# FHE-ACCELE/Homulator

Measured on AMD Instinct MI355X. Metric: hmult+key-switch ops/sec, higher is better.
Workload: dtype u64

## Files before the change

### homulator_amd/csrc/hm_backend.hip

```cpp
#include <hip/hip_runtime.h>
#include <dlfcn.h>
#include <rccl/rccl.h>
#include <algorithm>
#include <cstdarg>
#include <cstdio>
#include <cstring>
#include <map>
#include <tuple>
#include <type_traits>
#include <memory>
#include <stdexcept>
#include <string>
#include <vector>

#include "../../include/homulator_hip.h"
#include "hm_elem_core.h"
#include "hm_modarith.h"
#include "hm_ntt_core.h"
#include "hm_params.h"
#include "hm_caps.h"


__device__ __forceinline__ bool hm_block_map(uint32_t tiles_per_limb, uint32_t n_entries, uint32_t logG, uint32_t &entry, uint32_t &tile) {
  const uint32_t b = blockIdx.x, xcd = b & 7u, slot = b >> 3;
// ... 264 lines not shown
#define HM_NIP_MAX_TERMS 4
static_assert(HM_GENERIC || HM_NIP_MAX_TERMS <= 5, "mont32 lazy key products: five terms of less than 1.5q + 2^28 stay below 8q (hm_mac_add)");
#define HM_NIP_MAX_OUT 2
#define HM_NIP_MAX_LIMBS 4096
struct HmNipLimb {
  uint16_t x[HM_NIP_MAX_TERMS];
  uint16_t y[HM_NIP_MAX_OUT][HM_NIP_MAX_TERMS];
  uint16_t out[HM_NIP_MAX_OUT];
  uint16_t mod;
  uint16_t coeff_mask;
};
#define HM_NIP_INV_OUT 0x8000u
struct HmNipArgs {
  const uint64_t *hand;
  const uint64_t *x;
  const uint64_t *y;
  uint64_t *out;
  const HmW *tw, *twist;
  const HmW *tw_inv, *twist_inv;
  const HmMod *mods;
  uint32_t logN, n_limbs, logG, n_terms;
  const HmNipLimb *limb;
  uint32_t x_galois;
};
typedef const HmNipLimb __attribute__((address_space(4))) *HmConstNipLimb;
#ifndef HM_NIP_WAVES
#define HM_NIP_WAVES 3
#endif
#ifndef HM_NIP_WIDE
#define HM_NIP_WIDE 0
#endif
#ifndef HM_NIP_PREFETCH
#define HM_NIP_PREFETCH 0
#endif
#ifndef HM_NIP_MAC_CH
#define HM_NIP_MAC_CH 2
#endif
#ifndef HM_NIP_LD_AUX
#define HM_NIP_LD_AUX 0
#endif
#ifndef HM_NIP_ST_AUX
#define HM_NIP_ST_AUX 0
#endif
template <int K> struct HmNipKey { static constexpr int value = K; };
namespace hm16 {
#include "hm_nip_body.inl"
}
#undef HM_EPT
#define HM_EPT 8
namespace hm8 {
#include "hm_nip_body.inl"
}
#undef HM_EPT
#define HM_EPT 16
template <int OUTS, int INVOUT, bool XG = false>
__global__ void __launch_bounds__((1 << HM_TL_ROW) / HM_EPT) __attribute__((amdgpu_waves_per_eu(HM_NIP_WAVES))) k_ntt_row_ip(HmNipArgs a) {
  hm16::hm_nip_body<OUTS, INVOUT, HM_TL_ROW, XG>(a);
}
template <int OUTS, int INVOUT, bool XG = false>
__global__ void __launch_bounds__((1 << HM_TL_ROW) / 8) k_ntt_row_ip8(HmNipArgs a) {
  hm8::hm_nip_body<OUTS, INVOUT, HM_TL_ROW, XG>(a);
}

#include "hm_bcol.h"
__global__ void __launch_bounds__(256) k_tensor(HmTensorArgs a) {
  const uint32_t N = 1u << a.logN;
  const uint32_t per_limb = N / 512;
  const uint32_t entry = blockIdx.x / per_limb, chunk = blockIdx.x % per_limb;
  if (entry >= a.n_limbs) return;
  const HmTensorLimb lb = a.limb[entry];
  const HmMod m = a.mods[lb.mod];
  const size_t x = (size_t)chunk * 512 + 2 * threadIdx.x;
  const ulonglong2 va = *reinterpret_cast<const ulonglong2 *>(a.a + (size_t)lb.a * N + x);
  const ulonglong2 vb = *reinterpret_cast<const ulonglong2 *>(a.b + (size_t)lb.b * N + x);
  const ulonglong2 vc = *reinterpret_cast<const ulonglong2 *>(a.c + (size_t)lb.c * N + x);
  const ulonglong2 vd = *reinterpret_cast<const ulonglong2 *>(a.d + (size_t)lb.d * N + x);
  uint64_t x0, x1, x2, y0, y1, y2;
  hm_tensor_one(va.x, vb.x, vc.x, vd.x, m, x0, x1, x2);
  hm_tensor_one(va.y, vb.y, vc.y, vd.y, m, y0, y1, y2);
  const ulonglong2 r0 = {x0, y0}, r1 = {x1, y1}, r2 = {x2, y2};
  *reinterpret_cast<ulonglong2 *>(a.o0 + (size_t)lb.o0 * N + x) = r0;
  *reinterpret_cast<ulonglong2 *>(a.o1 + (size_t)lb.o1 * N + x) = r1;
  *reinterpret_cast<ulonglong2 *>(a.o2 + (size_t)lb.o2 * N + x) = r2;
}

#ifndef HM_EWE_UNITS
#define HM_EWE_UNITS 1
#endif
template <int OP>
__global__ void __launch_bounds__(256) k_ewe(HmEweArgs a) {
  const uint32_t N = 1u << a.logN;
  const uint32_t per_limb = N / (512 * HM_EWE_UNITS);
  uint32_t entry = blockIdx.x / per_limb, chunk = blockIdx.x % per_limb;
  if (entry >= a.n_limbs) return;
  const HmEweLimb lb = a.limb[entry];
  const HmMod m = a.mods[lb.mod];
  const HmTw k = a.k[entry];
  const size_t x0 = (size_t)chunk * (512 * HM_EWE_UNITS) + 2 * threadIdx.x;
  constexpr int uses = hm_ewe_uses(OP);
  ulonglong2 va[HM_EWE_UNITS], vb[HM_EWE_UNITS], vc[HM_EWE_UNITS], vd[HM_EWE_UNITS];
#pragma unroll
  for (int u = 0; u < HM_EWE_UNITS; ++u) {
    const size_t x = x0 + 512 * u;
    va[u] = vb[u] = vc[u] = vd[u] = ulonglong2{0, 0};
    if (uses & 1) va[u] = *reinterpret_cast<const ulonglong2 *>(a.a + (size_t)lb.a * N + x);
    if (uses & 2) vb[u] = *reinterpret_cast<const ulonglong2 *>(a.b + (size_t)lb.b * N + x);
    if (uses & 4) vc[u] = *reinterpret_cast<const ulonglong2 *>(a.c + (size_t)lb.c * N + x);
    if (uses & 8) vd[u] = *reinterpret_cast<const ulonglong2 *>(a.d + (size_t)lb.d * N + x);
  }
#pragma unroll
  for (int u = 0; u < HM_EWE_UNITS; ++u) {
    ulonglong2 r;
    r.x = hm_ewe_one<OP>(va[u].x, vb[u].x, vc[u].x, vd[u].x, k, m);
    r.y = hm_ewe_one<OP>(va[u].y, vb[u].y, vc[u].y, vd[u].y, k, m);
    *reinterpret_cast<ulonglong2 *>(a.out + (size_t)lb.out * N + x0 + 512 * u) = r;
  }
}

template <int TERMS, int OUTS>
__global__ void __launch_bounds__(256) k_inner_product(HmIpArgs a) {
  const uint32_t N = 1u << a.logN;
  const uint32_t per_limb = N / 512;
  const uint32_t entry = blockIdx.x / per_limb, chunk = blockIdx.x % per_limb;
  if (entry >= a.n_limbs) return;
  const HmIpLimb &lb = a.limb[entry];
  const HmMod m = a.mods[lb.mod];
  const size_t off = (size_t)chunk * 512 + 2 * threadIdx.x;
  ulonglong2 vx[TERMS], vy[OUTS][TERMS];
  size_t offx = off;
  bool swap = false;
  if (a.x_galois > 1) {
    const uint32_t s = hm_auto_src((uint32_t)off, a.x_galois, a.logN);
    offx = s & ~1u; swap = s & 1u;
  }
#pragma unroll
  for (int j = 0; j < TERMS; ++j) {
    vx[j] = *reinterpret_cast<const ulonglong2 *>(a.x + (size_t)lb.x[j] * N + offx);
    if (swap) { const unsigned long long t = vx[j].x; vx[j].x = vx[j].y; vx[j].y = t; }
#pragma unroll
    for (int k = 0; k < OUTS; ++k) vy[k][j] = *reinterpret_cast<const ulonglong2 *>(a.y + (size_t)lb.y[k][j] * N + off);
  }
#pragma unroll
  for (int k = 0; k < OUTS; ++k) {
    hm_u128 s0 = 0, s1 = 0;
#pragma unroll
    for (int j = 0; j < TERMS; ++j) {
      s0 += (hm_u128)vx[j].x * vy[k][j].x;
      s1 += (hm_u128)vx[j].y * vy[k][j].y;
    }
    const ulonglong2 r = {hm_barrett(s0, m), hm_barrett(s1, m)};
    *reinterpret_cast<ulonglong2 *>(a.out + (size_t)lb.out[k] * N + off) = r;
  }
}

template <int N_IN>
__global__ void __launch_bounds__(HM_BCONV_THREADS) k_bconv(HmBconvArgs a) {
  const auto &p = HM_CONST_PROB(a.prob)[blockIdx.z];
  const uint32_t t0 = blockIdx.y * a.chunk;
  if (t0 >= p.n_out) return;
  const uint32_t t1 = min(t0 + a.chunk, p.n_out);
  const uint32_t x = (blockIdx.x * HM_BCONV_THREADS + threadIdx.x) * HM_BCONV_CPT;
  if (x >= (1u << a.logN)) return;
  if (p.in_packed) hm_bconv_thread<N_IN, HM_BCONV_CPT, true>(p, a.logN, x, t0, t1);
  else hm_bconv_thread<N_IN, HM_BCONV_CPT, false>(p, a.logN, x, t0, t1);
}
typedef void (*hm_bconv_kernel)(HmBconvArgs);
// ... 873 lines not shown
  f.addGalois = d->addend_galois;
  if (d->addend_galois && (d->n_conv || d->mix || !d->addend)) return fail(c, HM_ERR_UNSUPPORTED,
      "hm_ntt_mix_sub_scale: addend_galois needs an addend and combines with neither the mix prologue nor conversions inside the transform");
  if (!d->n_conv) return ntt_common(c, "hm_ntt_mix_sub_scale", d->in, d->in_limbs, d->out, d->out_limbs, d->mod_ids, d->n, 0, d->k, f);
  if (!d->conv) return fail(c, HM_ERR_ARG, "hm_ntt_mix_sub_scale: n_conv without descriptors");
  const uint32_t n = d->n;
  std::map<uint32_t, uint32_t> byOut;
  for (uint32_t i = 0; i < n; ++i)
    if (!byOut.emplace(limb_at(d->out_limbs, i), i).second) return fail(c, HM_ERR_ARG, "hm_ntt_mix_sub_scale: output limb %u appears twice",
        limb_at(d->out_limbs, i));
  std::vector<char> covered(n, 0);
  std::vector<std::vector<uint32_t>> mixLimbs(d->n_conv);
  std::vector<std::vector<uint64_t>> mixK(d->n_conv);
  std::vector<const uint32_t *> mlp(d->n_conv);
  std::vector<const uint64_t *> mkp(d->n_conv);
  for (uint32_t j = 0; j < d->n_conv; ++j) {
    const hm_bconv_desc &cv = d->conv[j];
    if (cv.out != d->out) return fail(c, HM_ERR_ARG, "hm_ntt_mix_sub_scale: conv[%u].out must be the output buffer", j);
    if (!cv.out_ids || cv.n_out == 0 || cv.n_out > HM_BCONV_MAX_OUT) return fail(c, HM_ERR_ARG, "hm_ntt_mix_sub_scale: conv[%u]: bad output basis", j);
    for (uint32_t t = 0; t < cv.n_out; ++t) {
      auto it = byOut.find(limb_at(cv.out_limbs, t));
      if (it == byOut.end()) return fail(c, HM_ERR_ARG, "hm_ntt_mix_sub_scale: conv[%u] output %u feeds no limb-poly of the call", j, t);
      const uint32_t i = it->second;
      if (covered[i]) return fail(c, HM_ERR_ARG, "hm_ntt_mix_sub_scale: limb-poly %u is fed by two conversions", i);
      if (cv.out_ids[t] != d->mod_ids[i]) return fail(c, HM_ERR_ARG,
          "hm_ntt_mix_sub_scale: conv[%u] output %u has another modulus than the limb-poly it feeds", j, t);
      covered[i] = 1;
      mixLimbs[j].push_back(d->mix ? limb_at(d->mix_limbs, i) : 0);
      mixK[j].push_back(d->mix ? d->mix_k[i] : 0);
    }
    mlp[j] = mixLimbs[j].data(); mkp[j] = mixK[j].data();
  }
  const BcolMix bm = {d->mix, mlp.data(), mkp.data()};
  hm_status st;
  if ((st = bconv_col_launch(c, d->conv, d->n_conv, d->mix ? &bm : nullptr))) return st;
  auto sub = [&](char want, bool second) -> hm_status {
    std::vector<uint32_t> il, ml, mnl, al, ol, mods;
    std::vector<uint64_t> mk, ak, kk;
    for (uint32_t i = 0; i < n; ++i) {
      if (covered[i] != want) continue;
      il.push_back(limb_at(d->in_limbs, i)); ol.push_back(limb_at(d->out_limbs, i)); mnl.push_back(limb_at(d->minuend_limbs, i));
      mods.push_back(d->mod_ids[i]); kk.push_back(d->k[i]);
      if (d->mix) { ml.push_back(limb_at(d->mix_limbs, i)); mk.push_back(d->mix_k[i]); }
      if (d->addend) al.push_back(limb_at(d->addend_limbs, i));
      if (d->addend_k) ak.push_back(d->addend_k[i]);
    }
    if (mods.empty()) return HM_OK;
    if (!second && !d->in) return fail(c, HM_ERR_ARG, "hm_ntt_mix_sub_scale: `in` is null but not every limb-poly is fed by a conversion");
    NttFused g = f;
    g.minuend_limbs = mnl.data(); g.addend_limbs = d->addend ? al.data() : nullptr; g.addend_k = d->addend_k ? ak.data() : nullptr;
    g.mix_limbs = d->mix ? ml.data() : nullptr; g.mix_k = d->mix ? mk.data() : nullptr;
    g.secondPassOnly = second;
    if (second) { g.mix = nullptr; g.mix_limbs = nullptr; g.mix_k = nullptr; }
    return ntt_common(c, "hm_ntt_mix_sub_scale", second ? d->out : d->in, second ? ol.data() : il.data(), d->out, ol.data(), mods.data(),
        (uint32_t)mods.size(), 0, kk.data(), g);
  };
  if ((st = sub(1, true))) return st;
  return sub(0, false);
}

extern "C" hm_status hm_tensor(hm_ctx *c, const uint64_t *pa, const uint32_t *la, const uint64_t *pb, const uint32_t *lb,
                               const uint64_t *pc, const uint32_t *lc, const uint64_t *pd, const uint32_t *ld, uint64_t *o0,
                               const uint32_t *l0, uint64_t *o1, const uint32_t *l1, uint64_t *o2, const uint32_t *l2,
                               const uint32_t *mod_ids, uint32_t n) {
  if (!c) return HM_ERR_ARG;
  if (!pa || !pb || !pc || !pd || !o0 || !o1 || !o2) return fail(c, HM_ERR_ARG, "hm_tensor: null buffer");
  hm_status st;
  const uint32_t *lists[7] = {la, lb, lc, ld, l0, l1, l2};
  for (auto l : lists)
    if ((st = check_limbs(c, "hm_tensor", l, n))) return st;
  if ((st = check_mods(c, "hm_tensor", mod_ids, n))) return st;
  HM_HIP(c, hipSetDevice(c->device));
  for (uint32_t base = 0; base < n; base += HM_MAX_LIMBS) {
    const uint32_t cnt = std::min<uint32_t>(HM_MAX_LIMBS, n - base);
    HmTensorArgs a;
    a.a = pa; a.b = pb; a.c = pc; a.d = pd; a.o0 = o0; a.o1 = o1; a.o2 = o2;
    a.mods = c->d_mods; a.logN = c->P.logN; a.n_limbs = cnt;
    for (uint32_t i = 0; i < cnt; ++i) {
      const uint32_t g = base + i;
      a.limb[i] = HmTensorLimb{(uint16_t)limb_at(la, g), (uint16_t)limb_at(lb, g), (uint16_t)limb_at(lc, g), (uint16_t)limb_at(ld, g),
                               (uint16_t)limb_at(l0, g), (uint16_t)limb_at(l1, g), (uint16_t)limb_at(l2, g), (uint16_t)mod_ids[g]};
    }
    hipLaunchKernelGGL(k_tensor, dim3(cnt * (c->P.N / 512)), dim3(256), 0, c->stream, a);
    HM_HIP(c, hipGetLastError());
  }
  return HM_OK;
}

extern "C" hm_status hm_automorph(hm_ctx *c, const uint64_t *in, const uint32_t *in_limbs, uint64_t *out,
                                  const uint32_t *out_limbs, uint32_t n, uint32_t galois) {
  if (!c) return HM_ERR_ARG;
  if (!in || !out) return fail(c, HM_ERR_ARG, "hm_automorph: null buffer");
  if (!(galois & 1) || galois >= 2 * c->P.N) return fail(c, HM_ERR_ARG, "hm_automorph: galois element must be odd and < 2N");
  hm_status st;
  if ((st = check_limbs(c, "hm_automorph", in_limbs, n)) || (st = check_limbs(c, "hm_automorph", out_limbs, n))) return st;
  HM_HIP(c, hipSetDevice(c->device));
  for (uint32_t base = 0; base < n; base += HM_MAX_LIMBS) {
    const uint32_t cnt = std::min<uint32_t>(HM_MAX_LIMBS, n - base);
    HmAutoArgs a;
    a.in = in; a.out = out; a.logN = c->P.logN; a.n_limbs = cnt; a.g = galois;
    for (uint32_t i = 0; i < cnt; ++i)
      a.limb[i] = HmLimb{(uint16_t)limb_at(in_limbs, base + i), (uint16_t)limb_at(out_limbs, base + i), 0, 0};
    hipLaunchKernelGGL(k_automorph, dim3(cnt * (c->P.N / 1024)), dim3(256), 0, c->stream, a);
    HM_HIP(c, hipGetLastError());
  }
  return HM_OK;
}

template <int OP>
static void launch_ewe(hm_ctx *c, const HmEweArgs &a) {
  hipLaunchKernelGGL((k_ewe<OP>), dim3(a.n_limbs * (c->P.N / (512 * HM_EWE_UNITS))), dim3(256), 0, c->stream, a);
}

extern "C" hm_status hm_ewe(hm_ctx *c, int op, const uint64_t *pa, const uint32_t *la, const uint64_t *pb,
                            const uint32_t *lb, const uint64_t *pc, const uint32_t *lc, const uint64_t *pd,
                            const uint32_t *ld, uint64_t *out, const uint32_t *lo, const uint32_t *mod_ids,
                            uint32_t n, const uint64_t *k) {
  if (!c) return HM_ERR_ARG;
  if (op < 0 || op >= HM_EWE_NOPS) return fail(c, HM_ERR_ARG, "hm_ewe: bad opcode %d", op);
  const int uses = hm_ewe_uses(op);
  if (((uses & 1) && !pa) || ((uses & 2) && !pb) || ((uses & 4) && !pc) || ((uses & 8) && !pd) || !out)
    return fail(c, HM_ERR_ARG, "hm_ewe: opcode %d is missing an operand", op);
  const bool needs_k = op == HM_EWE_MUL_CONST || op == HM_EWE_SUB_SCALE || op == HM_EWE_SUB_SCALE_ADD;
  if (needs_k && !k) return fail(c, HM_ERR_ARG, "hm_ewe: opcode %d needs constants", op);
  hm_status st;
  if ((st = check_limbs(c, "hm_ewe", la, n)) || (st = check_limbs(c, "hm_ewe", lb, n)) ||
      (st = check_limbs(c, "hm_ewe", lc, n)) || (st = check_limbs(c, "hm_ewe", ld, n)) ||
      (st = check_limbs(c, "hm_ewe", lo, n)) || (st = check_mods(c, "hm_ewe", mod_ids, n)))
    return st;
  HM_HIP(c, hipSetDevice(c->device));
  for (uint32_t base = 0; base < n; base += HM_MAX_LIMBS) {
    const uint32_t cnt = std::min<uint32_t>(HM_MAX_LIMBS, n - base);
    HmEweArgs a;
    a.a = pa; a.b = pb; a.c = pc; a.d = pd; a.out = out;
    a.mods = c->d_mods; a.logN = c->P.logN; a.n_limbs = cnt; a.op = (uint32_t)op;
    for (uint32_t i = 0; i < cnt; ++i) {
      const uint32_t g = base + i, m = mod_ids[g];
      a.limb[i] = HmEweLimb{(uint16_t)limb_at(la, g), (uint16_t)limb_at(lb, g), (uint16_t)limb_at(lc, g),
                            (uint16_t)limb_at(ld, g), (uint16_t)limb_at(lo, g), (uint16_t)m};
      a.k[i] = HmTw{0, 0};
      if (needs_k) {
        if (k[g] >= c->P.mod[m]) return fail(c, HM_ERR_ARG, "hm_ewe: k[%u] is not reduced", g);
        a.k[i] = HmTw{k[g], hm::shoup(k[g], c->P.mod[m])};
      }
    }
    switch (op) {
    case HM_EWE_MUL: launch_ewe<HM_EWE_MUL>(c, a); break;
    case HM_EWE_MAC2: launch_ewe<HM_EWE_MAC2>(c, a); break;
    case HM_EWE_MAC_ADD: launch_ewe<HM_EWE_MAC_ADD>(c, a); break;
    case HM_EWE_ADD: launch_ewe<HM_EWE_ADD>(c, a); break;
    case HM_EWE_SUB: launch_ewe<HM_EWE_SUB>(c, a); break;
    case HM_EWE_MUL_CONST: launch_ewe<HM_EWE_MUL_CONST>(c, a); break;
    case HM_EWE_SUB_SCALE: launch_ewe<HM_EWE_SUB_SCALE>(c, a); break;
    case HM_EWE_COPY: launch_ewe<HM_EWE_COPY>(c, a); break;
    case HM_EWE_SUB_SCALE_ADD: launch_ewe<HM_EWE_SUB_SCALE_ADD>(c, a); break;
    }
    HM_HIP(c, hipGetLastError());
  }
  return HM_OK;
}

template <int T, int O>
static void launch_ip(hm_ctx *c, const HmIpArgs &a) {
  hipLaunchKernelGGL((k_inner_product<T, O>), dim3(a.n_limbs * (c->P.N / 512)), dim3(256), 0, c->stream, a);
}
extern "C" hm_status hm_inner_product(hm_ctx *c, const uint64_t *x, const uint32_t *x_limbs, const uint64_t *y,
// ... 639 lines not shown
```

### homulator_amd/csrc/hm_caps.h

```cpp
#pragma once
#include <stdint.h>
#include <string.h>

#define HM_BCOL_MAX_IN 32
#define HM_BCOL_MAX_IN_MIX 15

struct HmCaps {
  uint32_t small_geometry;
  uint32_t bcol_max_in;
  uint32_t bcol_pref_in;
  uint32_t bcol_max_in_mix;
  uint32_t ip_inverse_out;
  uint32_t col_slices;
};
static inline HmCaps hm_caps(uint32_t logN) {
  switch (logN) {
  case 16: return HmCaps{1, HM_BCOL_MAX_IN, 15, HM_BCOL_MAX_IN_MIX, 1, 16};
  case 15: return HmCaps{1, HM_BCOL_MAX_IN, HM_BCOL_MAX_IN, HM_BCOL_MAX_IN_MIX, 1, 8};
  default: return HmCaps{0, 0, 0, 0, 0, 0};
  }
}
static inline int hm_cap_by_name(uint32_t logN, const char *name, uint64_t *value) {
  const HmCaps c = hm_caps(logN);
  if (!strcmp(name, "cap_small_geometry")) { *value = c.small_geometry; return 0; }
  if (!strcmp(name, "cap_bconv_col_max_in")) { *value = c.bcol_max_in; return 0; }
  if (!strcmp(name, "cap_bconv_col_max_in_mix")) { *value = c.bcol_max_in_mix; return 0; }
  if (!strcmp(name, "cap_bconv_col_pref_in")) { *value = c.bcol_pref_in; return 0; }
  if (!strcmp(name, "cap_ip_inverse_out")) { *value = c.ip_inverse_out; return 0; }
  if (!strcmp(name, "cap_col_slices")) { *value = c.col_slices; return 0; }
  return 1;
}
```

### homulator_amd/csrc/hm_dispatch_gen.inc

```

struct HmApi {
  hm_status (*create)(hm_ctx **ctx, const hm_params *params);
  void (*destroy)(hm_ctx *ctx);
  const char * (*last_error)(const hm_ctx *ctx);
  const char * (*version)(void);
  hm_status (*get_modulus)(const hm_ctx *ctx, uint32_t mod_id, uint64_t *q);
  hm_status (*get_psi)(const hm_ctx *ctx, uint32_t mod_id, uint64_t *psi);
  hm_status (*malloc)(hm_ctx *ctx, size_t bytes, void **dptr);
  hm_status (*free)(hm_ctx *ctx, void *dptr);
  hm_status (*memcpy_h2d)(hm_ctx *ctx, void *dst, const void *src, size_t bytes);
  hm_status (*memcpy_d2h)(hm_ctx *ctx, void *dst, const void *src, size_t bytes);
  hm_status (*memcpy_d2d)(hm_ctx *ctx, void *dst, const void *src, size_t bytes);
  hm_status (*sync)(hm_ctx *ctx);
  void * (*stream)(hm_ctx *ctx);
  hm_status (*wait_for)(hm_ctx *ctx, hm_ctx *producer);
  hm_status (*ntt)(hm_ctx *ctx, const uint64_t *in, const uint32_t *in_limbs, uint64_t *out, const uint32_t *out_limbs, const uint32_t *mod_ids, uint32_t n, int inverse, const uint64_t *scale);
  hm_status (*ntt_sub_scale)(hm_ctx *ctx, const uint64_t *in, const uint32_t *in_limbs, const uint64_t *minuend, const uint32_t *minuend_limbs, const uint64_t *addend, const uint32_t *addend_limbs, uint64_t *out, const uint32_t *out_limbs, const uint32_t *mod_ids, uint32_t n, const uint64_t *k);
  hm_status (*ntt_mix_sub_scale)(hm_ctx *ctx, const hm_ntt_fused_desc *desc);
  hm_status (*automorph)(hm_ctx *ctx, const uint64_t *in, const uint32_t *in_limbs, uint64_t *out, const uint32_t *out_limbs, uint32_t n, uint32_t galois);
  hm_status (*ewe)(hm_ctx *ctx, int op, const uint64_t *a, const uint32_t *a_limbs, const uint64_t *b, const uint32_t *b_limbs, const uint64_t *c, const uint32_t *c_limbs, const uint64_t *d, const uint32_t *d_limbs, uint64_t *out, const uint32_t *out_limbs, const uint32_t *mod_ids, uint32_t n, const uint64_t *k);
  hm_status (*tensor)(hm_ctx *ctx, const uint64_t *a, const uint32_t *a_limbs, const uint64_t *b, const uint32_t *b_limbs, const uint64_t *c, const uint32_t *c_limbs, const uint64_t *d, const uint32_t *d_limbs, uint64_t *o0, const uint32_t *o0_limbs, uint64_t *o1, const uint32_t *o1_limbs, uint64_t *o2, const uint32_t *o2_limbs, const uint32_t *mod_ids, uint32_t n);
  hm_status (*inner_product)(hm_ctx *ctx, const uint64_t *x, const uint32_t *x_limbs, const uint64_t *y, const uint32_t *y_limbs, uint64_t *out, const uint32_t *out_limbs, const uint32_t *mod_ids, uint32_t n, uint32_t n_terms, uint32_t n_out);
  hm_status (*inner_product_ex)(hm_ctx *ctx, const hm_ip_desc *desc);
  hm_status (*inner_product_hoisted)(hm_ctx *ctx, const hm_ip_hoisted_desc *desc);
  hm_status (*ntt_inner_product)(hm_ctx *ctx, const hm_ntt_ip_desc *desc);
  hm_status (*ntt_second_pass)(hm_ctx *ctx, uint64_t *buf, const uint32_t *limbs, const uint32_t *mod_ids, uint32_t n, int inverse, const uint64_t *scale);
  hm_status (*ntt_ex)(hm_ctx *ctx, const hm_ntt_desc *desc);
  hm_status (*bconv)(hm_ctx *ctx, const uint64_t *in, const uint32_t *in_limbs, const uint32_t *in_ids, uint32_t n_in, uint64_t *out, const uint32_t *out_limbs, const uint32_t *out_ids, uint32_t n_out);
  hm_status (*bconv_batch)(hm_ctx *ctx, const hm_bconv_desc *descs, uint32_t n_desc);
  hm_status (*bconv_col)(hm_ctx *ctx, const hm_bconv_desc *descs, uint32_t n_desc, uint32_t tile0, uint32_t n_tiles);
  hm_status (*bconv_consts)(hm_ctx *ctx, const uint32_t *in_ids, uint32_t n_in, const uint32_t *out_ids, uint32_t n_out, uint64_t *qhat_inv, uint64_t *table);
  hm_status (*comm_unique_id)(void *out128);
  hm_status (*comm_init_rccl)(hm_ctx *ctx, int rank, int world, const void *unique_id128);
  hm_status (*comm_init_external)(hm_ctx *ctx, int rank, int world, hm_exchange_fn fn, void *user);
  hm_status (*comm_info)(const hm_ctx *ctx, int *rank, int *world);
  hm_status (*slice_rows)(const uint32_t *owners, uint32_t n, uint32_t world, uint32_t *rows);
  hm_status (*limbs_to_slices)(hm_ctx *ctx, const uint64_t *buf, const uint32_t *limbs, const uint32_t *owners, uint32_t n, uint64_t *slices);
  hm_status (*slices_to_limbs)(hm_ctx *ctx, const uint64_t *slices, uint64_t *buf, const uint32_t *limbs, const uint32_t *owners, uint32_t n);
  hm_status (*limbs_to_colslices)(hm_ctx *ctx, const uint64_t *buf, const uint32_t *limbs, const uint32_t *owners, uint32_t n, uint64_t *slices);
  hm_status (*colslices_to_limbs)(hm_ctx *ctx, const uint64_t *slices, uint64_t *buf, const uint32_t *limbs, const uint32_t *owners, uint32_t n);
  hm_status (*exchange_stream)(hm_ctx *ctx, int enable);
  hm_status (*exchange_mark)(hm_ctx *ctx, uint32_t slot);
  hm_status (*exchange_wait)(hm_ctx *ctx, uint32_t slot);
  hm_status (*replicate_limbs)(hm_ctx *ctx, uint64_t *buf, const uint32_t *limbs, const uint32_t *owners, uint32_t n);
  hm_status (*fill_uniform)(hm_ctx *ctx, uint64_t *out, const uint32_t *out_limbs, const uint32_t *mod_ids, uint32_t n, uint64_t seed);
  hm_status (*capture_begin)(hm_ctx *ctx);
  hm_status (*capture_end)(hm_ctx *ctx, hm_graph **graph);
  hm_status (*graph_launch)(hm_ctx *ctx, hm_graph *graph);
  void (*graph_destroy)(hm_graph *graph);
  hm_status (*set_option)(hm_ctx *ctx, const char *name, uint64_t value);
  hm_status (*capability)(uint32_t logN, const char *name, uint64_t *value);
  hm_status (*get_counter)(hm_ctx *ctx, const char *name, uint64_t *value);
  hm_status (*timer_start)(hm_ctx *ctx);
  hm_status (*timer_stop)(hm_ctx *ctx, uint64_t *elapsed_ns);
};
static HmApi g_api[2];
static const char *hm_api_load(void *h, HmApi &a) {
  a.create = reinterpret_cast<decltype(a.create)>(dlsym(h, "hm_create")); if (!a.create) return "hm_create";
  a.destroy = reinterpret_cast<decltype(a.destroy)>(dlsym(h, "hm_destroy")); if (!a.destroy) return "hm_destroy";
  a.last_error = reinterpret_cast<decltype(a.last_error)>(dlsym(h, "hm_last_error")); if (!a.last_error) return "hm_last_error";
  a.version = reinterpret_cast<decltype(a.version)>(dlsym(h, "hm_version")); if (!a.version) return "hm_version";
  a.get_modulus = reinterpret_cast<decltype(a.get_modulus)>(dlsym(h, "hm_get_modulus")); if (!a.get_modulus) return "hm_get_modulus";
  a.get_psi = reinterpret_cast<decltype(a.get_psi)>(dlsym(h, "hm_get_psi")); if (!a.get_psi) return "hm_get_psi";
  a.malloc = reinterpret_cast<decltype(a.malloc)>(dlsym(h, "hm_malloc")); if (!a.malloc) return "hm_malloc";
  a.free = reinterpret_cast<decltype(a.free)>(dlsym(h, "hm_free")); if (!a.free) return "hm_free";
  a.memcpy_h2d = reinterpret_cast<decltype(a.memcpy_h2d)>(dlsym(h, "hm_memcpy_h2d")); if (!a.memcpy_h2d) return "hm_memcpy_h2d";
  a.memcpy_d2h = reinterpret_cast<decltype(a.memcpy_d2h)>(dlsym(h, "hm_memcpy_d2h")); if (!a.memcpy_d2h) return "hm_memcpy_d2h";
  a.memcpy_d2d = reinterpret_cast<decltype(a.memcpy_d2d)>(dlsym(h, "hm_memcpy_d2d")); if (!a.memcpy_d2d) return "hm_memcpy_d2d";
  a.sync = reinterpret_cast<decltype(a.sync)>(dlsym(h, "hm_sync")); if (!a.sync) return "hm_sync";
  a.stream = reinterpret_cast<decltype(a.stream)>(dlsym(h, "hm_stream")); if (!a.stream) return "hm_stream";
  a.wait_for = reinterpret_cast<decltype(a.wait_for)>(dlsym(h, "hm_wait_for")); if (!a.wait_for) return "hm_wait_for";
  a.ntt = reinterpret_cast<decltype(a.ntt)>(dlsym(h, "hm_ntt")); if (!a.ntt) return "hm_ntt";
  a.ntt_sub_scale = reinterpret_cast<decltype(a.ntt_sub_scale)>(dlsym(h, "hm_ntt_sub_scale")); if (!a.ntt_sub_scale) return "hm_ntt_sub_scale";
  a.ntt_mix_sub_scale = reinterpret_cast<decltype(a.ntt_mix_sub_scale)>(dlsym(h, "hm_ntt_mix_sub_scale")); if (!a.ntt_mix_sub_scale) return "hm_ntt_mix_sub_scale";
  a.automorph = reinterpret_cast<decltype(a.automorph)>(dlsym(h, "hm_automorph")); if (!a.automorph) return "hm_automorph";
  a.ewe = reinterpret_cast<decltype(a.ewe)>(dlsym(h, "hm_ewe")); if (!a.ewe) return "hm_ewe";
  a.tensor = reinterpret_cast<decltype(a.tensor)>(dlsym(h, "hm_tensor")); if (!a.tensor) return "hm_tensor";
  a.inner_product = reinterpret_cast<decltype(a.inner_product)>(dlsym(h, "hm_inner_product")); if (!a.inner_product) return "hm_inner_product";
  a.inner_product_ex = reinterpret_cast<decltype(a.inner_product_ex)>(dlsym(h, "hm_inner_product_ex")); if (!a.inner_product_ex) return "hm_inner_product_ex";
  a.inner_product_hoisted = reinterpret_cast<decltype(a.inner_product_hoisted)>(dlsym(h, "hm_inner_product_hoisted")); if (!a.inner_product_hoisted) return "hm_inner_product_hoisted";
  a.ntt_inner_product = reinterpret_cast<decltype(a.ntt_inner_product)>(dlsym(h, "hm_ntt_inner_product")); if (!a.ntt_inner_product) return "hm_ntt_inner_product";
  a.ntt_second_pass = reinterpret_cast<decltype(a.ntt_second_pass)>(dlsym(h, "hm_ntt_second_pass")); if (!a.ntt_second_pass) return "hm_ntt_second_pass";
  a.ntt_ex = reinterpret_cast<decltype(a.ntt_ex)>(dlsym(h, "hm_ntt_ex")); if (!a.ntt_ex) return "hm_ntt_ex";
  a.bconv = reinterpret_cast<decltype(a.bconv)>(dlsym(h, "hm_bconv")); if (!a.bconv) return "hm_bconv";
  a.bconv_batch = reinterpret_cast<decltype(a.bconv_batch)>(dlsym(h, "hm_bconv_batch")); if (!a.bconv_batch) return "hm_bconv_batch";
  a.bconv_col = reinterpret_cast<decltype(a.bconv_col)>(dlsym(h, "hm_bconv_col")); if (!a.bconv_col) return "hm_bconv_col";
  a.bconv_consts = reinterpret_cast<decltype(a.bconv_consts)>(dlsym(h, "hm_bconv_consts")); if (!a.bconv_consts) return "hm_bconv_consts";
  a.comm_unique_id = reinterpret_cast<decltype(a.comm_unique_id)>(dlsym(h, "hm_comm_unique_id")); if (!a.comm_unique_id) return "hm_comm_unique_id";
  a.comm_init_rccl = reinterpret_cast<decltype(a.comm_init_rccl)>(dlsym(h, "hm_comm_init_rccl")); if (!a.comm_init_rccl) return "hm_comm_init_rccl";
  a.comm_init_external = reinterpret_cast<decltype(a.comm_init_external)>(dlsym(h, "hm_comm_init_external")); if (!a.comm_init_external) return "hm_comm_init_external";
  a.comm_info = reinterpret_cast<decltype(a.comm_info)>(dlsym(h, "hm_comm_info")); if (!a.comm_info) return "hm_comm_info";
  a.slice_rows = reinterpret_cast<decltype(a.slice_rows)>(dlsym(h, "hm_slice_rows")); if (!a.slice_rows) return "hm_slice_rows";
  a.limbs_to_slices = reinterpret_cast<decltype(a.limbs_to_slices)>(dlsym(h, "hm_limbs_to_slices")); if (!a.limbs_to_slices) return "hm_limbs_to_slices";
  a.slices_to_limbs = reinterpret_cast<decltype(a.slices_to_limbs)>(dlsym(h, "hm_slices_to_limbs")); if (!a.slices_to_limbs) return "hm_slices_to_limbs";
  a.limbs_to_colslices = reinterpret_cast<decltype(a.limbs_to_colslices)>(dlsym(h, "hm_limbs_to_colslices")); if (!a.limbs_to_colslices) return "hm_limbs_to_colslices";
  a.colslices_to_limbs = reinterpret_cast<decltype(a.colslices_to_limbs)>(dlsym(h, "hm_colslices_to_limbs")); if (!a.colslices_to_limbs) return "hm_colslices_to_limbs";
  a.exchange_stream = reinterpret_cast<decltype(a.exchange_stream)>(dlsym(h, "hm_exchange_stream")); if (!a.exchange_stream) return "hm_exchange_stream";
  a.exchange_mark = reinterpret_cast<decltype(a.exchange_mark)>(dlsym(h, "hm_exchange_mark")); if (!a.exchange_mark) return "hm_exchange_mark";
  a.exchange_wait = reinterpret_cast<decltype(a.exchange_wait)>(dlsym(h, "hm_exchange_wait")); if (!a.exchange_wait) return "hm_exchange_wait";
  a.replicate_limbs = reinterpret_cast<decltype(a.replicate_limbs)>(dlsym(h, "hm_replicate_limbs")); if (!a.replicate_limbs) return "hm_replicate_limbs";
  a.fill_uniform = reinterpret_cast<decltype(a.fill_uniform)>(dlsym(h, "hm_fill_uniform")); if (!a.fill_uniform) return "hm_fill_uniform";
  a.capture_begin = reinterpret_cast<decltype(a.capture_begin)>(dlsym(h, "hm_capture_begin")); if (!a.capture_begin) return "hm_capture_begin";
  a.capture_end = reinterpret_cast<decltype(a.capture_end)>(dlsym(h, "hm_capture_end")); if (!a.capture_end) return "hm_capture_end";
  a.graph_launch = reinterpret_cast<decltype(a.graph_launch)>(dlsym(h, "hm_graph_launch")); if (!a.graph_launch) return "hm_graph_launch";
  a.graph_destroy = reinterpret_cast<decltype(a.graph_destroy)>(dlsym(h, "hm_graph_destroy")); if (!a.graph_destroy) return "hm_graph_destroy";
  a.set_option = reinterpret_cast<decltype(a.set_option)>(dlsym(h, "hm_set_option")); if (!a.set_option) return "hm_set_option";
  a.capability = reinterpret_cast<decltype(a.capability)>(dlsym(h, "hm_capability")); if (!a.capability) return "hm_capability";
  a.get_counter = reinterpret_cast<decltype(a.get_counter)>(dlsym(h, "hm_get_counter")); if (!a.get_counter) return "hm_get_counter";
  a.timer_start = reinterpret_cast<decltype(a.timer_start)>(dlsym(h, "hm_timer_start")); if (!a.timer_start) return "hm_timer_start";
  a.timer_stop = reinterpret_cast<decltype(a.timer_stop)>(dlsym(h, "hm_timer_stop")); if (!a.timer_stop) return "hm_timer_stop";
  return nullptr;
}

extern "C" hm_status hm_get_modulus(const hm_ctx *ctx, uint32_t mod_id, uint64_t *q) { if (!ctx) return HM_ERR_ARG; HM_FORWARDED(ctx); return HM_API(ctx).get_modulus(HM_IMPL(ctx), mod_id, q); }
extern "C" hm_status hm_get_psi(const hm_ctx *ctx, uint32_t mod_id, uint64_t *psi) { if (!ctx) return HM_ERR_ARG; HM_FORWARDED(ctx); return HM_API(ctx).get_psi(HM_IMPL(ctx), mod_id, psi); }
extern "C" hm_status hm_malloc(hm_ctx *ctx, size_t bytes, void **dptr) { if (!ctx) return HM_ERR_ARG; HM_FORWARDED(ctx); return HM_API(ctx).malloc(HM_IMPL(ctx), bytes, dptr); }
extern "C" hm_status hm_free(hm_ctx *ctx, void *dptr) { if (!ctx) return HM_ERR_ARG; HM_FORWARDED(ctx); return HM_API(ctx).free(HM_IMPL(ctx), dptr); }
extern "C" hm_status hm_memcpy_h2d(hm_ctx *ctx, void *dst, const void *src, size_t bytes) { if (!ctx) return HM_ERR_ARG; HM_FORWARDED(ctx); return HM_API(ctx).memcpy_h2d(HM_IMPL(ctx), dst, src, bytes); }
extern "C" hm_status hm_memcpy_d2h(hm_ctx *ctx, void *dst, const void *src, size_t bytes) { if (!ctx) return HM_ERR_ARG; HM_FORWARDED(ctx); return HM_API(ctx).memcpy_d2h(HM_IMPL(ctx), dst, src, bytes); }
extern "C" hm_status hm_memcpy_d2d(hm_ctx *ctx, void *dst, const void *src, size_t bytes) { if (!ctx) return HM_ERR_ARG; HM_FORWARDED(ctx); return HM_API(ctx).memcpy_d2d(HM_IMPL(ctx), dst, src, bytes); }
extern "C" hm_status hm_sync(hm_ctx *ctx) { if (!ctx) return HM_ERR_ARG; HM_FORWARDED(ctx); return HM_API(ctx).sync(HM_IMPL(ctx)); }
extern "C" void *hm_stream(hm_ctx *ctx) { if (!ctx) return nullptr; return HM_API(ctx).stream(HM_IMPL(ctx)); }
extern "C" hm_status hm_ntt(hm_ctx *ctx, const uint64_t *in, const uint32_t *in_limbs, uint64_t *out, const uint32_t *out_limbs, const uint32_t *mod_ids, uint32_t n, int inverse, const uint64_t *scale) { if (!ctx) return HM_ERR_ARG; HM_FORWARDED(ctx); return HM_API(ctx).ntt(HM_IMPL(ctx), in, in_limbs, out, out_limbs, mod_ids, n, inverse, scale); }
extern "C" hm_status hm_ntt_sub_scale(hm_ctx *ctx, const uint64_t *in, const uint32_t *in_limbs, const uint64_t *minuend, const uint32_t *minuend_limbs, const uint64_t *addend, const uint32_t *addend_limbs, uint64_t *out, const uint32_t *out_limbs, const uint32_t *mod_ids, uint32_t n, const uint64_t *k) { if (!ctx) return HM_ERR_ARG; HM_FORWARDED(ctx); return HM_API(ctx).ntt_sub_scale(HM_IMPL(ctx), in, in_limbs, minuend, minuend_limbs, addend, addend_limbs, out, out_limbs, mod_ids, n, k); }
extern "C" hm_status hm_ntt_mix_sub_scale(hm_ctx *ctx, const hm_ntt_fused_desc *desc) { if (!ctx) return HM_ERR_ARG; HM_FORWARDED(ctx); return HM_API(ctx).ntt_mix_sub_scale(HM_IMPL(ctx), desc); }
extern "C" hm_status hm_automorph(hm_ctx *ctx, const uint64_t *in, const uint32_t *in_limbs, uint64_t *out, const uint32_t *out_limbs, uint32_t n, uint32_t galois) { if (!ctx) return HM_ERR_ARG; HM_FORWARDED(ctx); return HM_API(ctx).automorph(HM_IMPL(ctx), in, in_limbs, out, out_limbs, n, galois); }
extern "C" hm_status hm_ewe(hm_ctx *ctx, int op, const uint64_t *a, const uint32_t *a_limbs, const uint64_t *b, const uint32_t *b_limbs, const uint64_t *c, const uint32_t *c_limbs, const uint64_t *d, const uint32_t *d_limbs, uint64_t *out, const uint32_t *out_limbs, const uint32_t *mod_ids, uint32_t n, const uint64_t *k) { if (!ctx) return HM_ERR_ARG; HM_FORWARDED(ctx); return HM_API(ctx).ewe(HM_IMPL(ctx), op, a, a_limbs, b, b_limbs, c, c_limbs, d, d_limbs, out, out_limbs, mod_ids, n, k); }
extern "C" hm_status hm_tensor(hm_ctx *ctx, const uint64_t *a, const uint32_t *a_limbs, const uint64_t *b, const uint32_t *b_limbs, const uint64_t *c, const uint32_t *c_limbs, const uint64_t *d, const uint32_t *d_limbs, uint64_t *o0, const uint32_t *o0_limbs, uint64_t *o1, const uint32_t *o1_limbs, uint64_t *o2, const uint32_t *o2_limbs, const uint32_t *mod_ids, uint32_t n) { if (!ctx) return HM_ERR_ARG; HM_FORWARDED(ctx); return HM_API(ctx).tensor(HM_IMPL(ctx), a, a_limbs, b, b_limbs, c, c_limbs, d, d_limbs, o0, o0_limbs, o1, o1_limbs, o2, o2_limbs, mod_ids, n); }
extern "C" hm_status hm_inner_product(hm_ctx *ctx, const uint64_t *x, const uint32_t *x_limbs, const uint64_t *y, const uint32_t *y_limbs, uint64_t *out, const uint32_t *out_limbs, const uint32_t *mod_ids, uint32_t n, uint32_t n_terms, uint32_t n_out) { if (!ctx) return HM_ERR_ARG; HM_FORWARDED(ctx); return HM_API(ctx).inner_product(HM_IMPL(ctx), x, x_limbs, y, y_limbs, out, out_limbs, mod_ids, n, n_terms, n_out); }
extern "C" hm_status hm_inner_product_ex(hm_ctx *ctx, const hm_ip_desc *desc) { if (!ctx) return HM_ERR_ARG; HM_FORWARDED(ctx); return HM_API(ctx).inner_product_ex(HM_IMPL(ctx), desc); }
extern "C" hm_status hm_inner_product_hoisted(hm_ctx *ctx, const hm_ip_hoisted_desc *desc) { if (!ctx) return HM_ERR_ARG; HM_FORWARDED(ctx); return HM_API(ctx).inner_product_hoisted(HM_IMPL(ctx), desc); }
extern "C" hm_status hm_ntt_inner_product(hm_ctx *ctx, const hm_ntt_ip_desc *desc) { if (!ctx) return HM_ERR_ARG; HM_FORWARDED(ctx); return HM_API(ctx).ntt_inner_product(HM_IMPL(ctx), desc); }
extern "C" hm_status hm_ntt_second_pass(hm_ctx *ctx, uint64_t *buf, const uint32_t *limbs, const uint32_t *mod_ids, uint32_t n, int inverse, const uint64_t *scale) { if (!ctx) return HM_ERR_ARG; HM_FORWARDED(ctx); return HM_API(ctx).ntt_second_pass(HM_IMPL(ctx), buf, limbs, mod_ids, n, inverse, scale); }
extern "C" hm_status hm_ntt_ex(hm_ctx *ctx, const hm_ntt_desc *desc) { if (!ctx) return HM_ERR_ARG; HM_FORWARDED(ctx); return HM_API(ctx).ntt_ex(HM_IMPL(ctx), desc); }
extern "C" hm_status hm_bconv(hm_ctx *ctx, const uint64_t *in, const uint32_t *in_limbs, const uint32_t *in_ids, uint32_t n_in, uint64_t *out, const uint32_t *out_limbs, const uint32_t *out_ids, uint32_t n_out) { if (!ctx) return HM_ERR_ARG; HM_FORWARDED(ctx); return HM_API(ctx).bconv(HM_IMPL(ctx), in, in_limbs, in_ids, n_in, out, out_limbs, out_ids, n_out); }
extern "C" hm_status hm_bconv_batch(hm_ctx *ctx, const hm_bconv_desc *descs, uint32_t n_desc) { if (!ctx) return HM_ERR_ARG; HM_FORWARDED(ctx); return HM_API(ctx).bconv_batch(HM_IMPL(ctx), descs, n_desc); }
extern "C" hm_status hm_bconv_col(hm_ctx *ctx, const hm_bconv_desc *descs, uint32_t n_desc, uint32_t tile0, uint32_t n_tiles) { if (!ctx) return HM_ERR_ARG; HM_FORWARDED(ctx); return HM_API(ctx).bconv_col(HM_IMPL(ctx), descs, n_desc, tile0, n_tiles); }
extern "C" hm_status hm_bconv_consts(hm_ctx *ctx, const uint32_t *in_ids, uint32_t n_in, const uint32_t *out_ids, uint32_t n_out, uint64_t *qhat_inv, uint64_t *table) { if (!ctx) return HM_ERR_ARG; HM_FORWARDED(ctx); return HM_API(ctx).bconv_consts(HM_IMPL(ctx), in_ids, n_in, out_ids, n_out, qhat_inv, table); }
extern "C" hm_status hm_comm_init_rccl(hm_ctx *ctx, int rank, int world, const void *unique_id128) { if (!ctx) return HM_ERR_ARG; HM_FORWARDED(ctx); return HM_API(ctx).comm_init_rccl(HM_IMPL(ctx), rank, world, unique_id128); }
extern "C" hm_status hm_comm_init_external(hm_ctx *ctx, int rank, int world, hm_exchange_fn fn, void *user) { if (!ctx) return HM_ERR_ARG; HM_FORWARDED(ctx); return HM_API(ctx).comm_init_external(HM_IMPL(ctx), rank, world, fn, user); }
extern "C" hm_status hm_comm_info(const hm_ctx *ctx, int *rank, int *world) { if (!ctx) return HM_ERR_ARG; HM_FORWARDED(ctx); return HM_API(ctx).comm_info(HM_IMPL(ctx), rank, world); }
extern "C" hm_status hm_limbs_to_slices(hm_ctx *ctx, const uint64_t *buf, const uint32_t *limbs, const uint32_t *owners, uint32_t n, uint64_t *slices) { if (!ctx) return HM_ERR_ARG; HM_FORWARDED(ctx); return HM_API(ctx).limbs_to_slices(HM_IMPL(ctx), buf, limbs, owners, n, slices); }
extern "C" hm_status hm_slices_to_limbs(hm_ctx *ctx, const uint64_t *slices, uint64_t *buf, const uint32_t *limbs, const uint32_t *owners, uint32_t n) { if (!ctx) return HM_ERR_ARG; HM_FORWARDED(ctx); return HM_API(ctx).slices_to_limbs(HM_IMPL(ctx), slices, buf, limbs, owners, n); }
extern "C" hm_status hm_limbs_to_colslices(hm_ctx *ctx, const uint64_t *buf, const uint32_t *limbs, const uint32_t *owners, uint32_t n, uint64_t *slices) { if (!ctx) return HM_ERR_ARG; HM_FORWARDED(ctx); return HM_API(ctx).limbs_to_colslices(HM_IMPL(ctx), buf, limbs, owners, n, slices); }
extern "C" hm_status hm_colslices_to_limbs(hm_ctx *ctx, const uint64_t *slices, uint64_t *buf, const uint32_t *limbs, const uint32_t *owners, uint32_t n) { if (!ctx) return HM_ERR_ARG; HM_FORWARDED(ctx); return HM_API(ctx).colslices_to_limbs(HM_IMPL(ctx), slices, buf, limbs, owners, n); }
extern "C" hm_status hm_exchange_stream(hm_ctx *ctx, int enable) { if (!ctx) return HM_ERR_ARG; HM_FORWARDED(ctx); return HM_API(ctx).exchange_stream(HM_IMPL(ctx), enable); }
extern "C" hm_status hm_exchange_mark(hm_ctx *ctx, uint32_t slot) { if (!ctx) return HM_ERR_ARG; HM_FORWARDED(ctx); return HM_API(ctx).exchange_mark(HM_IMPL(ctx), slot); }
extern "C" hm_status hm_exchange_wait(hm_ctx *ctx, uint32_t slot) { if (!ctx) return HM_ERR_ARG; HM_FORWARDED(ctx); return HM_API(ctx).exchange_wait(HM_IMPL(ctx), slot); }
extern "C" hm_status hm_replicate_limbs(hm_ctx *ctx, uint64_t *buf, const uint32_t *limbs, const uint32_t *owners, uint32_t n) { if (!ctx) return HM_ERR_ARG; HM_FORWARDED(ctx); return HM_API(ctx).replicate_limbs(HM_IMPL(ctx), buf, limbs, owners, n); }
extern "C" hm_status hm_fill_uniform(hm_ctx *ctx, uint64_t *out, const uint32_t *out_limbs, const uint32_t *mod_ids, uint32_t n, uint64_t seed) { if (!ctx) return HM_ERR_ARG; HM_FORWARDED(ctx); return HM_API(ctx).fill_uniform(HM_IMPL(ctx), out, out_limbs, mod_ids, n, seed); }
extern "C" hm_status hm_capture_begin(hm_ctx *ctx) { if (!ctx) return HM_ERR_ARG; HM_FORWARDED(ctx); return HM_API(ctx).capture_begin(HM_IMPL(ctx)); }
extern "C" hm_status hm_set_option(hm_ctx *ctx, const char *name, uint64_t value) { if (!ctx) return HM_ERR_ARG; HM_FORWARDED(ctx); return HM_API(ctx).set_option(HM_IMPL(ctx), name, value); }
extern "C" hm_status hm_get_counter(hm_ctx *ctx, const char *name, uint64_t *value) { if (!ctx) return HM_ERR_ARG; HM_FORWARDED(ctx); return HM_API(ctx).get_counter(HM_IMPL(ctx), name, value); }
extern "C" hm_status hm_timer_start(hm_ctx *ctx) { if (!ctx) return HM_ERR_ARG; HM_FORWARDED(ctx); return HM_API(ctx).timer_start(HM_IMPL(ctx)); }
extern "C" hm_status hm_timer_stop(hm_ctx *ctx, uint64_t *elapsed_ns) { if (!ctx) return HM_ERR_ARG; HM_FORWARDED(ctx); return HM_API(ctx).timer_stop(HM_IMPL(ctx), elapsed_ns); }
```

### homulator_amd/hip.py

```python
import ctypes as C
import os

import numpy as np

_HERE = os.path.dirname(os.path.abspath(__file__))
LIB_PATH = os.environ.get("HOMULATOR_HIP_LIB") or os.path.join(_HERE, "lib", "libhomulator_hip.so")
BACKEND_LIBS = ("libhm_m32.so", "libhm_gen.so")

OP_MUL, OP_MAC2, OP_MAC_ADD, OP_ADD, OP_SUB, OP_MUL_CONST, OP_SUB_SCALE, OP_COPY, OP_SUB_SCALE_ADD = range(9)

SYMBOLS = [
    "hm_create", "hm_destroy", "hm_last_error", "hm_version", "hm_get_modulus", "hm_get_psi", "hm_malloc", "hm_free",
    "hm_memcpy_h2d", "hm_memcpy_d2h", "hm_memcpy_d2d", "hm_sync", "hm_stream", "hm_wait_for", "hm_ntt", "hm_ntt_sub_scale", "hm_ntt_mix_sub_scale", "hm_tensor", "hm_inner_product", "hm_automorph", "hm_ewe",
    "hm_bconv", "hm_bconv_batch", "hm_bconv_consts", "hm_fill_uniform", "hm_timer_start", "hm_timer_stop", "hm_comm_unique_id", "hm_comm_init_rccl", "hm_comm_init_external",
    "hm_capture_begin", "hm_capture_end", "hm_graph_launch", "hm_graph_destroy", "hm_comm_info", "hm_slice_rows", "hm_limbs_to_slices", "hm_slices_to_limbs", "hm_replicate_limbs",
    "hm_set_option", "hm_get_counter", "hm_ntt_inner_product", "hm_exchange_stream", "hm_exchange_mark", "hm_exchange_wait",
    "hm_bconv_col", "hm_limbs_to_colslices", "hm_colslices_to_limbs", "hm_ntt_second_pass", "hm_ntt_ex", "hm_capability", "hm_inner_product_ex",
    "hm_inner_product_hoisted",
]


class hm_ntt_fused_desc(C.Structure):
    _fields_ = [("in_", C.c_void_p), ("in_limbs", C.c_void_p), ("mix", C.c_void_p), ("mix_limbs", C.c_void_p), ("mix_k", C.c_void_p),
                ("minuend", C.c_void_p), ("minuend_limbs", C.c_void_p), ("addend", C.c_void_p), ("addend_limbs", C.c_void_p),
                ("addend_k", C.c_void_p), ("out", C.c_void_p), ("out_limbs", C.c_void_p), ("mod_ids", C.c_void_p), ("n", C.c_uint32),
                ("k", C.c_void_p), ("conv", C.c_void_p), ("n_conv", C.c_uint32), ("addend_galois", C.c_void_p)]


class hm_ip_desc(C.Structure):
    _fields_ = [("x", C.c_void_p), ("x_limbs", C.c_void_p), ("y", C.c_void_p), ("y_limbs", C.c_void_p), ("out", C.c_void_p), ("out_limbs", C.c_void_p),
                ("mod_ids", C.c_void_p), ("n", C.c_uint32), ("n_terms", C.c_uint32), ("n_out", C.c_uint32), ("x_galois", C.c_uint32)]


class hm_ip_hoisted_desc(C.Structure):
    _fields_ = [("x", C.c_void_p), ("x_limbs", C.c_void_p), ("y", C.c_void_p), ("y_limbs", C.c_void_p), ("out", C.c_void_p), ("out_limbs", C.c_void_p),
                ("mod_ids", C.c_void_p), ("n", C.c_uint32), ("n_terms", C.c_uint32), ("n_rot", C.c_uint32), ("galois", C.c_void_p)]


class hm_ntt_ip_desc(C.Structure):
    _fields_ = [("x", C.c_void_p), ("x_limbs", C.c_void_p), ("x_is_coeff", C.c_void_p), ("hand", C.c_void_p), ("hand_limbs", C.c_void_p),
                ("y", C.c_void_p), ("y_limbs", C.c_void_p), ("out", C.c_void_p), ("out_limbs", C.c_void_p), ("mod_ids", C.c_void_p),
                ("n", C.c_uint32), ("n_terms", C.c_uint32), ("n_out", C.c_uint32), ("conv", C.c_void_p), ("n_conv", C.c_uint32),
                ("out_inverse", C.c_void_p), ("x_galois", C.c_uint32)]


class hm_bconv_desc(C.Structure):
    _fields_ = [("in_", C.c_void_p), ("in_limbs", C.c_void_p), ("in_ids", C.c_void_p), ("n_in", C.c_uint32),
                ("out", C.c_void_p), ("out_limbs", C.c_void_p), ("out_ids", C.c_void_p), ("n_out", C.c_uint32),
                ("log_len", C.c_uint32), ("sub_from", C.c_void_p), ("sub_from_limbs", C.c_void_p), ("add", C.c_void_p), ("add_limbs", C.c_void_p),
                ("sub_k", C.c_void_p), ("in_packed", C.c_uint32)]


class hm_ntt_desc(C.Structure):
    _fields_ = [("in_", C.c_void_p), ("in_limbs", C.c_void_p), ("out", C.c_void_p), ("out_limbs", C.c_void_p), ("mod_ids", C.c_void_p), ("n", C.c_uint32),
                ("inverse", C.c_int), ("scale", C.c_void_p), ("second_pass_only", C.c_int), ("out_packed", C.c_void_p),
                ("in_galois", C.c_void_p)]


class hm_params(C.Structure):
    _fields_ = [("logN", C.c_uint32), ("L", C.c_uint32), ("K", C.c_uint32), ("device", C.c_int32),
                ("q", C.c_void_p), ("p", C.c_void_p), ("psi", C.c_void_p)]


_lib = None


def load():
    global _lib
    if _lib is not None:
        return _lib
    if not os.path.exists(LIB_PATH):
        raise ImportError(f"{LIB_PATH} is missing: build it with __graft_entry__.build() "
                          "(make -C homulator_amd/csrc); homulator_amd has no CPU fallback")
    L = C.CDLL(LIB_PATH)
    vp, u32, u64, i32 = C.c_void_p, C.c_uint32, C.c_uint64, C.c_int
    L.hm_create.argtypes = [C.POINTER(vp), C.POINTER(hm_params)]
    L.hm_destroy.argtypes = [vp]
    L.hm_last_error.restype = C.c_char_p
    L.hm_last_error.argtypes = [vp]
    L.hm_version.restype = C.c_char_p
    L.hm_get_modulus.argtypes = [vp, u32, C.POINTER(u64)]
    L.hm_get_psi.argtypes = [vp, u32, C.POINTER(u64)]
    L.hm_malloc.argtypes = [vp, C.c_size_t, C.POINTER(vp)]
    L.hm_free.argtypes = [vp, vp]
    L.hm_memcpy_h2d.argtypes = [vp, vp, vp, C.c_size_t]
    L.hm_memcpy_d2h.argtypes = [vp, vp, vp, C.c_size_t]
    L.hm_memcpy_d2d.argtypes = [vp, vp, vp, C.c_size_t]
    L.hm_sync.argtypes = [vp]
    L.hm_stream.restype = vp
    L.hm_stream.argtypes = [vp]
    L.hm_wait_for.argtypes = [vp, vp]
    L.hm_ntt.argtypes = [vp, vp, vp, vp, vp, vp, u32, i32, vp]
    L.hm_ntt_second_pass.argtypes = [vp, vp, vp, vp, u32, i32, vp]
    L.hm_ntt_ex.argtypes = [vp, C.POINTER(hm_ntt_desc)]
    L.hm_inner_product_ex.argtypes = [vp, C.POINTER(hm_ip_desc)]
    L.hm_inner_product_hoisted.argtypes = [vp, C.POINTER(hm_ip_hoisted_desc)]
    L.hm_ntt_sub_scale.argtypes = [vp] + [vp] * 9 + [u32, vp]
    L.hm_ntt_mix_sub_scale.argtypes = [vp, C.POINTER(hm_ntt_fused_desc)]
    L.hm_tensor.argtypes = [vp] + [vp] * 15 + [u32]
    L.hm_inner_product.argtypes = [vp] + [vp] * 7 + [u32, u32, u32]
    L.hm_automorph.argtypes = [vp, vp, vp, vp, vp, u32, u32]
    L.hm_ewe.argtypes = [vp, i32] + [vp] * 11 + [u32, vp]
    L.hm_bconv.argtypes = [vp, vp, vp, vp, u32, vp, vp, vp, u32]
    L.hm_bconv_batch.argtypes = [vp, C.POINTER(hm_bconv_desc), u32]
    L.hm_bconv_consts.argtypes = [vp, vp, u32, vp, u32, vp, vp]
    L.hm_fill_uniform.argtypes = [vp, vp, vp, vp, u32, u64]
    L.hm_ntt_inner_product.argtypes = [vp, C.POINTER(hm_ntt_ip_desc)]
    L.hm_set_option.argtypes = [vp, C.c_char_p, u64]
    L.hm_get_counter.argtypes = [vp, C.c_char_p, C.POINTER(u64)]
    L.hm_capability.argtypes = [u32, C.c_char_p, C.POINTER(u64)]
    L.hm_comm_init_external.argtypes = [vp, i32, i32, vp, vp]
    L.hm_timer_start.argtypes = [vp]
    L.hm_timer_stop.argtypes = [vp, C.POINTER(u64)]
    _lib = L
    return L


class HmError(RuntimeError):
    pass


def capability(logN, name):
    v = C.c_uint64()
    if load().hm_capability(int(logN), name.encode(), C.byref(v)) != 0:
        raise HmError(f"hm_capability: unknown capability {name}")
    return v.value


def _u32(a):
    if a is None:
        return None, None
    arr = np.ascontiguousarray(np.asarray(a, dtype=np.uint32))
    return arr, arr.ctypes.data_as(C.c_void_p)


def _u64(a):
    if a is None:
        return None, None
    arr = np.ascontiguousarray(np.asarray([int(x) for x in a], dtype=np.uint64))
    return arr, arr.ctypes.data_as(C.c_void_p)


class DeviceBuf:

    def __init__(self, ctx, n_limbs):
        self.ctx, self.n_limbs = ctx, n_limbs
        p = C.c_void_p()
        ctx._ck(ctx.L.hm_malloc(ctx.h, 8 * ctx.N * n_limbs, C.byref(p)))
        self.ptr = p.value

    def limb_ptr(self, limb):
        return self.ptr + 8 * self.ctx.N * limb

    def upload(self, arr, limb0=0):
        a = np.ascontiguousarray(arr, dtype=np.uint64).reshape(-1, self.ctx.N)
        assert limb0 + a.shape[0] <= self.n_limbs
        self.ctx._ck(self.ctx.L.hm_memcpy_h2d(self.ctx.h, self.limb_ptr(limb0), a.ctypes.data_as(C.c_void_p), a.nbytes))
        return self

    def download(self, limb0=0, n=None):
        n = self.n_limbs - limb0 if n is None else n
        out = np.empty((n, self.ctx.N), dtype=np.uint64)
        self.ctx._ck(self.ctx.L.hm_memcpy_d2h(self.ctx.h, out.ctypes.data_as(C.c_void_p), self.limb_ptr(limb0), out.nbytes))
        return out

    def free(self):
        if self.ptr:
            self.ctx.L.hm_free(self.ctx.h, self.ptr)
            self.ptr = None


class Context:

    def __init__(self, logN, L, K, device=0, q=None, p=None):
        self.L = load()
        self.h = C.c_void_p()
        qa = None if q is None else np.ascontiguousarray(np.asarray(q, dtype=np.uint64))
        pa = None if p is None else np.ascontiguousarray(np.asarray(p, dtype=np.uint64))
        if (qa is not None and len(qa) != L) or (pa is not None and len(pa) != K):
            raise ValueError("q needs L entries and p needs K")
        prm = hm_params(logN, L, K, device, None if qa is None else qa.ctypes.data_as(C.c_void_p), None if pa is None else pa.ctypes.data_as(C.c_void_p), None)
        st = self.L.hm_create(C.byref(self.h), C.byref(prm))
        if st != 0:
            raise HmError(f"hm_create failed ({st}): {self.L.hm_last_error(None).decode()}")
        self.logN, self.N, self.nQ, self.K = logN, 1 << logN, L, K
        self.chain = None if qa is None else [int(x) for x in qa] + ([] if pa is None else [int(x) for x in pa])
        q = C.c_uint64()
        self.moduli = []
        for m in range(L + K):
            self._ck(self.L.hm_get_modulus(self.h, m, C.byref(q)))
            self.moduli.append(q.value)

    def _ck(self, st):
        if st != 0:
            raise HmError(f"hm error {st}: {self.L.hm_last_error(self.h).decode()}")

    def close(self):
        if self.h:
            self.L.hm_destroy(self.h)
            self.h = None

    def __del__(self):
        try:
            self.close()
        except Exception:
            pass

    def alloc(self, n_limbs):
        return DeviceBuf(self, n_limbs)

    def from_host(self, arr):
        a = np.ascontiguousarray(arr, dtype=np.uint64).reshape(-1, self.N)
        return self.alloc(a.shape[0]).upload(a)

    def sync(self):
        self._ck(self.L.hm_sync(self.h))

    def ext_ids(self, ell):
        return list(range(ell)) + [self.nQ + i for i in range(self.K)]

    def ntt(self, src, dst, mod_ids, inverse=False, in_limbs=None, out_limbs=None, scale=None, out_packed=None, in_galois=None):
        n = len(mod_ids)
        k1, pi = _u32(in_limbs)
        k2, po = _u32(out_limbs)
        k3, pm = _u32(mod_ids)
        k4, ps = _u64(scale)
        if out_packed is None and in_galois is None:
            self._ck(self.L.hm_ntt(self.h, src.ptr, pi, dst.ptr, po, pm, n, 1 if inverse else 0, ps))
            return
        pk = None if out_packed is None else np.ascontiguousarray(np.asarray(out_packed, dtype=np.uint8))
        k5, pg = _u32(in_galois)
        d = hm_ntt_desc(src.ptr, pi, dst.ptr, po, pm, n, 1 if inverse else 0, ps, 0, None if pk is None else pk.ctypes.data_as(C.c_void_p), pg)
        self._ck(self.L.hm_ntt_ex(self.h, C.byref(d)))

    def ntt_sub_scale(self, src, minuend, out, mod_ids, k, addend=None, in_limbs=None, minuend_limbs=None, addend_limbs=None,
                      out_limbs=None):
        keep = [_u32(x) for x in (in_limbs, minuend_limbs, addend_limbs, out_limbs, mod_ids)]
        kk, pk = _u64(k)
        self._ck(self.L.hm_ntt_sub_scale(self.h, src.ptr, keep[0][1], minuend.ptr, keep[1][1], None if addend is None else addend.ptr,
                                         keep[2][1], out.ptr, keep[3][1], keep[4][1], len(mod_ids), pk))

    def ntt_mix_sub_scale(self, src, minuend, out, mod_ids, k, mix=None, mix_k=None, addend=None, addend_k=None, in_limbs=None,
                          mix_limbs=None, minuend_limbs=None, addend_limbs=None, out_limbs=None, conv=None, addend_galois=None):
        keep = [_u32(x) for x in (in_limbs, mix_limbs, minuend_limbs, addend_limbs, out_limbs, mod_ids)]
        ks = [_u64(x) for x in (mix_k, addend_k, k)]
        kg = _u32(addend_galois)
        ptr = lambda v: None if v is None else v.ptr
        descs, keep2 = None, []
        if conv:
            descs = (hm_bconv_desc * len(conv))()
            for dd, (csrc, c_in_limbs, in_ids, c_out_limbs, out_ids, *pk) in zip(descs, conv):
                arrs = [_u32(c_in_limbs), _u32(in_ids), _u32(c_out_limbs), _u32(out_ids)]
                keep2.append(arrs)
                dd.in_packed = 1 if pk and pk[0] else 0
                dd.in_, dd.in_limbs, dd.in_ids, dd.n_in = csrc.ptr, arrs[0][1], arrs[1][1], len(in_ids)
                dd.out, dd.out_limbs, dd.out_ids, dd.n_out, dd.log_len = out.ptr, arrs[2][1], arrs[3][1], len(out_ids), 0
        d = hm_ntt_fused_desc(ptr(src) if src is not None else out.ptr, keep[0][1], ptr(mix), keep[1][1], ks[0][1], minuend.ptr, keep[2][1], ptr(addend), keep[3][1], ks[1][1],
                              out.ptr, keep[4][1], keep[5][1], len(mod_ids), ks[2][1], C.cast(descs, C.c_void_p) if conv else None, len(conv) if conv else 0,
                              kg[1])
        self._ck(self.L.hm_ntt_mix_sub_scale(self.h, C.byref(d)))

    def tensor(self, a, b, c, d, o0, o1, o2, mod_ids, limbs=None):
        ls = limbs or [None] * 7
        keep = [_u32(x) for x in ls] + [_u32(mod_ids)]
        self._ck(self.L.hm_tensor(self.h, a.ptr, keep[0][1], b.ptr, keep[1][1], c.ptr, keep[2][1], d.ptr, keep[3][1], o0.ptr, keep[4][1],
                                  o1.ptr, keep[5][1], o2.ptr, keep[6][1], keep[7][1], len(mod_ids)))

    def inner_product(self, x, x_limbs, y, y_limbs, out, out_limbs, mod_ids, n_terms, n_out, x_galois=0):
        keep = [_u32(v) for v in (x_limbs, y_limbs, out_limbs, mod_ids)]
        if x_galois:
            d = hm_ip_desc(x.ptr, keep[0][1], y.ptr, keep[1][1], out.ptr, keep[2][1], keep[3][1], len(mod_ids), n_terms, n_out, int(x_galois))
            self._ck(self.L.hm_inner_product_ex(self.h, C.byref(d)))
            return
        self._ck(self.L.hm_inner_product(self.h, x.ptr, keep[0][1], y.ptr, keep[1][1], out.ptr, keep[2][1], keep[3][1], len(mod_ids),
                                         n_terms, n_out))

    def inner_product_hoisted(self, x, x_limbs, y, y_limbs, out, out_limbs, mod_ids, n_terms, galois):
        keep = [_u32(v) for v in (x_limbs, y_limbs, out_limbs, mod_ids, galois)]
        d = hm_ip_hoisted_desc(x.ptr, keep[0][1], y.ptr, keep[1][1], out.ptr, keep[2][1], keep[3][1], len(mod_ids), n_terms, len(galois), keep[4][1])
        self._ck(self.L.hm_inner_product_hoisted(self.h, C.byref(d)))

    def ntt_second_pass(self, buf, mod_ids, inverse=False, limbs=None, scale=None):
        k1, pl = _u32(limbs)
        k2, pm = _u32(mod_ids)
        k3, ps = _u64(scale)
        self._ck(self.L.hm_ntt_second_pass(self.h, buf.ptr, pl, pm, len(mod_ids), 1 if inverse else 0, ps))

    def ntt_inner_product(self, x, x_limbs, x_is_coeff, hand, hand_limbs, y, y_limbs, out, out_limbs, mod_ids, n_terms, n_out, conv=None, out_inverse=None,
                          x_galois=0):
        keep = [_u32(v) for v in (x_limbs, hand_limbs, y_limbs, out_limbs, mod_ids)]
        flags = np.ascontiguousarray(np.asarray(x_is_coeff, dtype=np.uint8))
        descs, keep2 = None, []
        if conv:
            descs = (hm_bconv_desc * len(conv))()
            for dd, (src, in_limbs, in_ids, out_limbs_, out_ids, *pk) in zip(descs, conv):
                arrs = [_u32(in_limbs), _u32(in_ids), _u32(out_limbs_), _u32(out_ids)]
                keep2.append(arrs)
                dd.in_packed = 1 if pk and pk[0] else 0
                dd.in_, dd.in_limbs, dd.in_ids, dd.n_in = src.ptr, arrs[0][1], arrs[1][1], len(in_ids)
                dd.out, dd.out_limbs, dd.out_ids, dd.n_out, dd.log_len = hand.ptr, arrs[2][1], arrs[3][1], len(out_ids), 0
        inv = None if out_inverse is None else np.ascontiguousarray(np.asarray(out_inverse, dtype=np.uint8))
        d = hm_ntt_ip_desc(x.ptr, keep[0][1], flags.ctypes.data_as(C.c_void_p), None if hand is None else hand.ptr, keep[1][1], y.ptr, keep[2][1],
                           out.ptr, keep[3][1], keep[4][1], len(mod_ids), n_terms, n_out,
                           C.cast(descs, C.c_void_p) if conv else None, len(conv) if conv else 0,
                           None if inv is None else inv.ctypes.data_as(C.c_void_p), int(x_galois))
        self._ck(self.L.hm_ntt_inner_product(self.h, C.byref(d)))

    def automorph(self, src, dst, n, galois, in_limbs=None, out_limbs=None):
        k1, pi = _u32(in_limbs)
        k2, po = _u32(out_limbs)
        self._ck(self.L.hm_automorph(self.h, src.ptr, pi, dst.ptr, po, n, galois))

    def ewe(self, op, out, mod_ids, a=None, b=None, c=None, d=None, la=None, lb=None, lc=None, ld=None, lo=None, k=None):
        keep = [_u32(x) for x in (la, lb, lc, ld, lo, mod_ids)]
        kk, pk = _u64(k)
        ptr = lambda x: None if x is None else x.ptr
        self._ck(self.L.hm_ewe(self.h, op, ptr(a), keep[0][1], ptr(b), keep[1][1], ptr(c), keep[2][1], ptr(d), keep[3][1],
                               out.ptr, keep[4][1], keep[5][1], len(mod_ids), pk))

    def bconv(self, src, in_ids, dst, out_ids, in_limbs=None, out_limbs=None):
        k1, pil = _u32(in_limbs)
        k2, pii = _u32(in_ids)
        k3, pol = _u32(out_limbs)
        k4, poi = _u32(out_ids)
        self._ck(self.L.hm_bconv(self.h, src.ptr, pil, pii, len(in_ids), dst.ptr, pol, poi, len(out_ids)))

    def bconv_batch(self, probs, log_len=0):
        keep, descs = [], (hm_bconv_desc * len(probs))()
        for d, (src, in_limbs, in_ids, dst, out_limbs, out_ids, *pk) in zip(descs, probs):
            arrs = [_u32(in_limbs), _u32(in_ids), _u32(out_limbs), _u32(out_ids)]
            keep.append(arrs)
            d.in_packed = 1 if pk and pk[0] else 0
            d.in_, d.in_limbs, d.in_ids, d.n_in = src.ptr, arrs[0][1], arrs[1][1], len(in_ids)
            d.out, d.out_limbs, d.out_ids, d.n_out, d.log_len = dst.ptr, arrs[2][1], arrs[3][1], len(out_ids), log_len
        self._ck(self.L.hm_bconv_batch(self.h, descs, len(probs)))

    def bconv_consts(self, in_ids, out_ids):
        k1, pii = _u32(in_ids)
        k2, poi = _u32(out_ids)
        qh = np.empty(len(in_ids), dtype=np.uint64)
        tb = np.empty((len(in_ids), max(1, len(out_ids))), dtype=np.uint64)
        self._ck(self.L.hm_bconv_consts(self.h, pii, len(in_ids), poi, len(out_ids), qh.ctypes.data_as(C.c_void_p),
                                        tb.ctypes.data_as(C.c_void_p)))
        return qh, tb[:, :len(out_ids)]

    def fill_uniform(self, dst, mod_ids, seed, out_limbs=None):
        k1, pol = _u32(out_limbs)
# ... 19 lines not shown
```

### host/include/Arch.h

```cpp
#ifndef HOMULATOR_ARCH_H
#define HOMULATOR_ARCH_H
#include "Basic.h"
#include "Config.h"
#include "Instruction.h"
#include "Statistic.h"
#include "SimModel.h"

struct hm_ctx;
class DataMap;
class MemController;

struct Stage {
  std::string name;
  ins_ops kind;
  std::vector<Instruction *> ins;
  uint32_t cluster0 = 0;
};

struct InputFill {
  std::vector<AddrType> addrs;
  std::vector<uint32_t> mods;
  uint64_t seed;
  bool shared = false;
};

class Arch {
public:
  enum Backend { BACKEND_HIP = 0, BACKEND_COUNT = 1, BACKEND_SIM = 2 };

  explicit Arch(Config *cfg);
  ~Arch();

  void bindParams(uint32_t maxLevel, uint32_t curLevel, uint32_t alpha);
  uint32_t owner(uint32_t modId) const { return modId < maxLevel_ ? modId % world_ : (curLevel_ + (modId - maxLevel_)) % world_; }
  uint32_t rank() const { return rank_; }
  uint32_t world() const { return world_; }
  void commInitRccl(const void *uniqueId128);
  void commInitExternal(void *fn, void *user);
  void registerLimbs(const std::vector<AddrType> &limbStarts);
  void addInputFill(const InputFill &f) { fills.push_back(f); }
  void bindInput(const std::vector<AddrType> &dst, Arch *src, const std::vector<AddrType> &srcAddrs);
  uint64_t modulus(uint32_t modId) const;
  std::vector<uint64_t> bconvScale(const std::vector<uint32_t> &inMods);
  Backend backend() const { return backendKind; }
  void loadSim(SimProgram &&program);
  SimModel *simModel() { return sim; }
  hm_ctx *context() { return ctx; }

  void issueIns(uint32_t index, const std::string &name, std::vector<Instruction *> &insg);
  void issueIns(uint32_t index, uint32_t h, uint32_t w, std::vector<Instruction *> &insg, bool hpip);
  void setDataMap(DataMap *) {}
  std::vector<MemController *> getMemController() { return {}; }
  void issueIns(uint32_t cluster, const std::string &unit, const Stage &stage);
  void update();
  bool simulateComplete();
  unsigned long long getCycle();
  unsigned long long getcompletedIns();
  void state();
  void shownStat();

  void prepare();
  void run();
  void sync();
  double timedRun(uint32_t iters);
  bool readLimbs(const std::vector<AddrType> &addrs, uint64_t *host, uint32_t copy = 0);
  bool writeLimbs(const std::vector<AddrType> &addrs, const uint64_t *host, uint32_t copy = 0);
  void refill(const std::vector<AddrType> &addrs, uint64_t seed);
  void snapshot(const std::vector<AddrType> &addrs, uint32_t slot);
  bool readSnapshot(uint32_t slot, uint64_t *host);
  uint32_t batch() const { return batch_; }
  size_t launchCount() const { return launches.size(); }
  std::string stageTimes(uint32_t iters);
  std::string planText() const;
  unsigned long long algorithmicBytes() const { return algBytes; }
  Statistic *stats() { return stat; }
  uint32_t N() const { return n; }

private:
  struct Launch;
  Config *config;
  Backend backendKind;
  bool fuse;
  bool shardFused = false;
  bool pipelineDigits = false;
  bool shardGather = false;
  bool fuseHpip = true;
  bool fuseBconv = true;
  bool fuseIpInv = true;
  bool packBconvIn = true;
  bool fuseAuto = true;
  bool fuseModDown = true;
  bool fuseHoist = true;
  uint32_t n = 0, logN = 0, clusterCount = 1;
  uint32_t maxLevel_ = 0, curLevel_ = 0, world_ = 1, rank_ = 0;
  uint32_t batch_ = 1;
  bool commReady = false;
  bool useGraph = false;
  unsigned runCount = 0;
  void *graph = nullptr;
  std::vector<void *> sliceBuffers;
  std::map<uint32_t, std::pair<uint64_t *, size_t>> snapshots;
  hm_ctx *ctx = nullptr;
  void *hostParams = nullptr;
  uint64_t *pool = nullptr;
  std::map<AddrType, uint32_t> limbIndex;
  std::vector<Stage> stages;
  std::vector<InputFill> fills;
  struct Binding { std::vector<AddrType> dst; Arch *src; std::vector<AddrType> srcAddrs; std::vector<uint32_t> dstLimbs, srcLimbs, mods; };
  std::vector<Binding> bindings;
  std::vector<Launch *> launches;
  size_t nextLaunch = 0;
  bool prepared = false;
  unsigned long long completedIns = 0, elapsedNs = 0, algBytes = 0;
  Statistic *stat;
  SimModel *sim = nullptr;

  uint32_t limbOf(AddrType a) const;
  void buildLaunches();
  void fusePasses(std::vector<Stage> &st);
  void enqueue(Launch &l);
  void replicateForBatch();
};
#endif
```

### host/include/Instruction.h

```cpp
#ifndef HOMULATOR_INSTRUCTION_H
#define HOMULATOR_INSTRUCTION_H
#include "Basic.h"

enum ins_ops { NTT, INTT, MULT, MADD, MSUB, BCONV_STEP1, BCONV_STEP2, AUTO, DS, PRNG, IP, FETCH_RF, STORE_RF };
extern std::vector<std::string> ins_ops_name;

enum ewe_opcode {
  EWE_MUL = 0, EWE_MAC2 = 1, EWE_MAC_ADD = 2, EWE_ADD = 3, EWE_SUB = 4,
  EWE_MUL_CONST = 5, EWE_SUB_SCALE = 6, EWE_COPY = 7, EWE_SUB_SCALE_ADD = 8
};

class Instruction {
public:
  ins_ops ops;
  std::string Name;
  uint32_t level_id = 0;
  uint32_t mod_id = 0;
  std::vector<AddrType> operandList;
  AddrType OutputOperand = 0;
  ewe_opcode opcode = EWE_MUL;
  bool hasConstant = false;
  uint64_t constant = 0;
  uint32_t galois = 0;
  bool passthrough = false;
  std::vector<uint32_t> inMods;
  unsigned long long refInstructions = 0;
  unsigned long long refExtra = 0;
  bool fusedSubScale = false;
  AddrType fMinuend = 0, fAddend = 0;
  AddrType fMix = 0;
  uint64_t fMixConst = 0, fAddendConst = 0;
  std::vector<AddrType> fConvIn;
  std::vector<uint32_t> fConvMods;
  bool ipInvOut = false;
  bool secondOnly = false;
  bool packedOut = false;
  bool inPacked = false;
  std::vector<uint8_t> ipConvPacked;
  uint32_t inGalois = 0, fAddendGalois = 0;
  uint32_t ipXGalois = 0;
  bool fusedEpi = false;
  AddrType fSubFrom = 0, fAdd = 0;
  bool fusedTensor = false;
  std::vector<AddrType> extraOutputs;
  std::vector<AddrType> ipX;
  std::vector<std::vector<AddrType>> ipY;
  std::vector<AddrType> ipSrc;
  std::vector<uint8_t> ipCoeff;
  std::vector<std::vector<AddrType>> ipConvIn;
  std::vector<std::vector<uint32_t>> ipConvMods;
  std::vector<uint32_t> ipHoistG;
  std::vector<Instruction *> depsInsList;

  Instruction(std::string name, ins_ops op, uint32_t level) : ops(op), Name(std::move(name)), level_id(level) {}
  const std::string &GetOpName() const { return ins_ops_name[ops]; }
  const std::string &GetName() const { return Name; }
  uint32_t getinputCount() const { return (uint32_t)operandList.size(); }
  AddrType getOperand(uint32_t i) const { return operandList[i]; }
};

typedef std::vector<Instruction *> INSGROUP;
#endif
```

### host/src/Arch.cpp

```cpp
#include "Arch.h"

#include <algorithm>
#include <chrono>
#include <fstream>
#include <iterator>
#include <cstring>
#include <set>

#include "../../homulator_amd/csrc/hm_params.h"
#include "../../include/homulator_hip.h"

static uint32_t cap(uint32_t logN, const char *name) {
  uint64_t v = 0;
  return hm_capability(logN, name, &v) == HM_OK ? (uint32_t)v : 0u;
}

struct Arch::Launch {
  enum Kind { L_NTT, L_INTT, L_EWE, L_BCONV, L_AUTO, L_NTT_SUBSCALE, L_TENSOR, L_EXCH_IN, L_EXCH_OUT, L_REPLICATE, L_IP, L_NTT_IP,
              L_BCONV_COL, L_EXCH_IN_COL, L_EXCH_OUT_COL,
              L_IP_HOISTED } kind;
  std::vector<uint32_t> hoistG;
  Launch *xin = nullptr, *xout = nullptr;
  int recordSlot = -1;
  std::vector<int> waitSlots;
  std::vector<uint8_t> ipCoeff;
  std::vector<uint8_t> ipInv;
  bool secondOnly = false;
  std::vector<uint8_t> outPacked;
  std::vector<uint32_t> inGalois, addGalois;
  uint32_t xGalois = 0;
  uint32_t ipTerms = 0, ipOuts = 0;
  std::string name;
  std::string statKey;
  int opcode = 0;
  uint32_t galois = 0;
  std::vector<uint32_t> a, b, c, d, out, out1, out2, mods, inMods;
  struct Prob { std::vector<uint32_t> in, inMods, out, outMods, epA, epB; std::vector<uint64_t> epK; bool epi = false, epAdd = false, inPacked = false; };
  std::vector<Prob> probs;
  std::vector<uint32_t> exLimbs, exOwners;
  uint64_t *slicesIn = nullptr, *slicesOut = nullptr;
  uint32_t logLen = 0;
  std::vector<uint64_t> k, mixK, addK;
  bool hasK = false;
  unsigned long long refInstructions = 0;
  unsigned long long bytes = 0;
};

static hm::Params &hostP(void *p) { return *static_cast<hm::Params *>(p); }

Arch::Arch(Config *cfg) : config(cfg) {
  n = cfg->getValue("N");
  logN = 0;
  while ((1u << logN) < n) ++logN;
  clusterCount = cfg->getValueOr("cluster", 1);
  uint32_t b = cfg->getValueOr("backend", BACKEND_HIP);
  if (const char *e = getenv("HOMULATOR_BACKEND")) b = std::string(e) == "count" ? BACKEND_COUNT : std::string(e) == "sim" ? BACKEND_SIM : BACKEND_HIP;
  backendKind = b == BACKEND_COUNT ? BACKEND_COUNT : b == BACKEND_SIM ? BACKEND_SIM : BACKEND_HIP;
  world_ = cfg->getValueOr("world", 0);
  rank_ = cfg->getValueOr("rank", 0);
  if (world_ == 0) {
    world_ = 1;
    const char *ws = getenv("WORLD_SIZE"), *rk = getenv("RANK"), *lr = getenv("LOCAL_RANK");
    if (ws && atoi(ws) > 1 && b == BACKEND_HIP && cfg->getValueOr("launcher_env", 0)) {
      world_ = (uint32_t)atoi(ws);
      rank_ = rk ? (uint32_t)atoi(rk) : 0;
      if (lr && !getenv("HOMULATOR_DEVICE") && !cfg->hasKey("device")) cfg->setValue("device", (uint32_t)atoi(lr));
      if (cfg->getValueOr("cluster_from_argv", 0) && clusterCount != world_)
        throw std::runtime_error("[cluster] = " + std::to_string(clusterCount) + " GPUs requested, but the launcher started " + std::to_string(world_) + " ranks");
    }
  }
  if (rank_ >= world_) throw std::runtime_error("rank must be below world");
  if (world_ & (world_ - 1)) throw std::runtime_error("world must be a power of two");
  useGraph = cfg->getValueOr("graph", 0) != 0;
  if (const char *e = getenv("HOMULATOR_GRAPH")) useGraph = std::string(e) != "0";
  batch_ = std::max<uint32_t>(1, cfg->getValueOr("batch", 1));
  if (const char *e = getenv("HOMULATOR_BATCH")) batch_ = std::max(1, atoi(e));
  fuse = cfg->getValueOr("fuse", 1) != 0;
  if (const char *e = getenv("HOMULATOR_FUSE")) fuse = std::string(e) != "0";
  fuseHpip = cfg->getValueOr("fuse_hpip", 1) != 0;
  if (const char *e = getenv("HOMULATOR_FUSE_HPIP")) fuseHpip = std::string(e) != "0";
  fuseBconv = cfg->getValueOr("fuse_bconv", 1) != 0;
  if (const char *e = getenv("HOMULATOR_FUSE_BCONV")) fuseBconv = std::string(e) != "0";
  fuseIpInv = cfg->getValueOr("fuse_ip_inv", 1) != 0;
  if (const char *e = getenv("HOMULATOR_FUSE_IP_INV")) fuseIpInv = std::string(e) != "0";
  packBconvIn = cfg->getValueOr("pack_bconv_in", 1) != 0;
  if (const char *e = getenv("HOMULATOR_PACK_BCONV_IN")) packBconvIn = std::string(e) != "0";
  fuseAuto = cfg->getValueOr("fuse_auto", 1) != 0;
  if (const char *e = getenv("HOMULATOR_FUSE_AUTO")) fuseAuto = std::string(e) != "0";
  fuseModDown = cfg->getValueOr("fuse_moddown", 0) != 0;
  if (const char *e = getenv("HOMULATOR_FUSE_MODDOWN")) fuseModDown = std::string(e) != "0";
  fuseHoist = cfg->getValueOr("fuse_hoist", 1) != 0;
  pipelineDigits = world_ > 1 && cfg->getValueOr("pipeline_digits", 1) != 0;
  if (const char *e = getenv("HOMULATOR_PIPELINE_DIGITS")) pipelineDigits = world_ > 1 && std::string(e) != "0";
  shardFused = world_ > 1 && cfg->getValueOr("shard_fused", 1) != 0 && fuseHpip && fuseBconv && world_ <= cap(logN, "cap_col_slices");
  if (const char *e = getenv("HOMULATOR_SHARD_FUSED")) shardFused = shardFused && std::string(e) != "0";
  {
    uint32_t plan = cfg->getValueOr("shard_plan", 0);
    if (const char *e = getenv("HOMULATOR_SHARD_PLAN")) plan = (uint32_t)atoi(e);
    shardGather = world_ > 1 && (plan == 2 || (plan == 0 && world_ <= 4));
    if (shardGather) { shardFused = false; pipelineDigits = false; }
  }
  if (pipelineDigits && !shardFused) fuseHpip = false;
  stat = new Statistic();
}

Arch::~Arch() {
  for (Launch *l : launches) delete l;
  if (graph) hm_graph_destroy(static_cast<hm_graph *>(graph));
  if (ctx)
    for (void *p : sliceBuffers) hm_free(ctx, p);
  if (ctx)
    for (auto &kv : snapshots) hm_free(ctx, kv.second.first);
  if (ctx) {
    if (pool) hm_free(ctx, pool);
    hm_destroy(ctx);
  }
  delete static_cast<hm::Params *>(hostParams);
  delete stat;
  delete sim;
}

void Arch::loadSim(SimProgram &&program) {
  if (backendKind != BACKEND_SIM) throw std::runtime_error("loadSim: backend is not sim");
  delete sim;
  sim = nullptr;
  sim = new SimModel(config, std::move(program));
}

void Arch::commInitRccl(const void *id) {
  if (!ctx) throw std::runtime_error("commInitRccl: no HIP context");
  if (hm_comm_init_rccl(ctx, (int)rank_, (int)world_, id) != HM_OK) throw std::runtime_error(std::string("hm_comm_init_rccl: ") + hm_last_error(ctx));
  commReady = true;
}
void Arch::commInitExternal(void *fn, void *user) {
  if (!ctx) throw std::runtime_error("commInitExternal: no HIP context");
  if (hm_comm_init_external(ctx, (int)rank_, (int)world_, reinterpret_cast<hm_exchange_fn>(fn), user) != HM_OK)
    throw std::runtime_error(std::string("hm_comm_init_external: ") + hm_last_error(ctx));
  commReady = true;
}

void Arch::bindParams(uint32_t maxLevel, uint32_t curLevel, uint32_t alpha) {
  maxLevel_ = maxLevel;
  curLevel_ = curLevel;
  if (hostParams) return;
  hm::Params *hp = new hm::Params;
  const uint32_t chainBits = config->getValueOr("chain_bits", 0);
  std::vector<uint64_t> chain;
  if (chainBits) chain = hm::Params::chain_below(logN, chainBits, maxLevel + alpha);
  const uint64_t *cq = chainBits ? chain.data() : nullptr, *cp = chainBits ? chain.data() + maxLevel : nullptr;
  hp->init(logN, maxLevel, alpha, cq, cp, nullptr,  chainBits != 0);
  hostParams = hp;
  if (backendKind == BACKEND_HIP) {
    hm_params p = {logN, maxLevel, alpha, (int32_t)config->getValueOr("device", 0), cq, cp, nullptr};
    if (const char *e = getenv("HOMULATOR_DEVICE")) p.device = atoi(e);
    if (hm_create(&ctx, &p) != HM_OK)
      throw std::runtime_error(std::string("HIP backend unavailable: ") + hm_last_error(nullptr));
  }
}

uint64_t Arch::modulus(uint32_t modId) const { return hostP(hostParams).mod.at(modId); }

std::vector<uint64_t> Arch::bconvScale(const std::vector<uint32_t> &inMods) {
  std::vector<uint64_t> qh(inMods.size()), tb(inMods.size());
  hostP(hostParams).bconv_consts(inMods.data(), (uint32_t)inMods.size(), nullptr, 0, qh.data(), tb.data());
  return qh;
}

// ... 456 lines not shown
        if (dead.count(i)) continue;
        if (i->ops == IP && !i->ipX.empty()) {
          for (AddrType x : (i->ipSrc.empty() ? i->ipX : i->ipSrc)) nread[x]++;
          for (auto &cin : i->ipConvIn) for (AddrType x : cin) nread[x]++;
          for (auto &y : i->ipY) for (AddrType yy : y) nread[yy]++;
        } else {
          for (AddrType a : operands(i)) nread[a]++;
          if (i->fusedSubScale) { nread[i->fMinuend]++; if (i->fAddend) nread[i->fAddend]++; if (i->fMix) nread[i->fMix]++; }
          for (AddrType x : i->fConvIn) nread[x]++;
        }
      }
    for (auto &s : st)
      for (size_t ei = 0; ei < s.ins.size(); ++ei) {
        Instruction *e = s.ins[ei];
        if (e->ops != MULT || dead.count(e) || (e->opcode != EWE_SUB_SCALE && e->opcode != EWE_SUB_SCALE_ADD)) continue;
        auto pb = producer.find(e->operandList[2]);
        if (pb == producer.end() || pb->second->ops != BCONV_STEP2 || dead.count(pb->second) || pb->second->fusedEpi || pb->second->mod_id != e->mod_id ||
            nread[e->operandList[2]] != 1)
          continue;
        Instruction *cv = pb->second;
        cv->fusedEpi = true;
        cv->fSubFrom = e->operandList[0];
        cv->fAdd = e->opcode == EWE_SUB_SCALE_ADD ? e->operandList[3] : 0;
        cv->hasConstant = true;
        cv->constant = e->constant;
        cv->OutputOperand = e->OutputOperand;
        cv->refExtra += e->refInstructions;
        producer[cv->OutputOperand] = cv;
        for (auto &s2 : st) s2.ins.erase(std::remove(s2.ins.begin(), s2.ins.end(), cv), s2.ins.end());
        std::replace(s.ins.begin(), s.ins.end(), e, cv);
        dead.insert(e);
      }
  }
  if (packBconvIn && (world_ == 1 || shardGather)) {
    struct Conv { std::vector<AddrType> in; Instruction *ins; int digit; };
    std::vector<Conv> convs;
    std::map<AddrType, int> otherReads;
    for (auto &s : st)
      for (Instruction *i : s.ins) {
        if (dead.count(i)) continue;
        if (i->ops == IP && !i->ipX.empty()) {
          const auto &src = i->ipSrc.empty() ? i->ipX : i->ipSrc;
          for (size_t j = 0; j < src.size(); ++j) {
            const bool conv = j < i->ipConvIn.size() && !i->ipConvIn[j].empty();
            if (conv) convs.push_back(Conv{i->ipConvIn[j], i, (int)j});
            else otherReads[src[j]]++;
          }
          for (auto &y : i->ipY) for (AddrType yy : y) otherReads[yy]++;
          continue;
        }
        if (i->ops == INTT && i->secondOnly) continue;
        if (i->ops == BCONV_STEP2) convs.push_back(Conv{std::vector<AddrType>(i->operandList.begin(), i->operandList.end() - 1), i, -1});
        else if (!i->fConvIn.empty()) {
          if (i->fMix) { for (AddrType a : i->fConvIn) otherReads[a]++; }
          else convs.push_back(Conv{i->fConvIn, i, -1});
        } else for (AddrType a : operands(i)) otherReads[a]++;
        if (i->fusedSubScale) { otherReads[i->fMinuend]++; if (i->fAddend) otherReads[i->fAddend]++; if (i->fMix) otherReads[i->fMix]++; }
        if (i->fusedEpi) { otherReads[i->fSubFrom]++; if (i->fAdd) otherReads[i->fAdd]++; }
      }
    std::set<AddrType> cand;
    for (auto &s : st)
      for (Instruction *x : s.ins)
        if (x->ops == INTT && !dead.count(x) && !otherReads.count(x->OutputOperand)) cand.insert(x->OutputOperand);
    for (bool changed = true; changed;) {
      changed = false;
      for (const Conv &cv : convs) {
        bool all = true;
        for (AddrType a : cv.in) all &= cand.count(a) != 0;
        if (all) continue;
        for (AddrType a : cv.in) changed |= cand.erase(a) != 0;
      }
    }
    std::set<AddrType> read;
    for (const Conv &cv : convs) {
      if (cv.in.empty() || !cand.count(cv.in[0])) continue;
      if (cv.digit >= 0) { cv.ins->ipConvPacked.resize(cv.ins->ipConvIn.size(), 0); cv.ins->ipConvPacked[(size_t)cv.digit] = 1; }
      else cv.ins->inPacked = true;
      read.insert(cv.in.begin(), cv.in.end());
    }
    for (auto &s : st)
      for (Instruction *x : s.ins)
        if (x->ops == INTT && !dead.count(x) && read.count(x->OutputOperand)) x->packedOut = true;
  }
  if (fuseAuto) {
    struct Reader { Instruction *ins; int role; size_t digit; };
    std::map<AddrType, std::vector<Reader>> readers;
    std::vector<Reader> ownDigits;
    for (auto &s : st)
      for (Instruction *i : s.ins) {
        if (dead.count(i)) continue;
        if (i->ops == IP && !i->ipX.empty()) {
          const bool anyT = std::find(i->ipCoeff.begin(), i->ipCoeff.end(), 1) != i->ipCoeff.end(), can = !i->ipXGalois && i->ipHoistG.empty();
          const auto &src = i->ipSrc.empty() ? i->ipX : i->ipSrc;
          for (size_t j = 0; j < src.size(); ++j) {
            const bool own = can && (!anyT || (!i->ipCoeff[j] && !(j < i->ipConvIn.size() && !i->ipConvIn[j].empty())));
            readers[src[j]].push_back({i, own ? 2 : -1, j});
            if (own) ownDigits.push_back({i, 2, j});
          }
          for (auto &v : i->ipConvIn) for (AddrType a : v) readers[a].push_back({i, -1, 0});
          for (auto &y : i->ipY) for (AddrType a : y) readers[a].push_back({i, -1, 0});
          continue;
        }
        const bool plainIntt = i->ops == INTT && !i->secondOnly && i->fConvIn.empty() && !i->inGalois;
        for (AddrType a : operands(i)) readers[a].push_back({i, plainIntt && a == i->operandList[0] ? 0 : -1, 0});
        for (AddrType a : i->fConvIn) readers[a].push_back({i, -1, 0});
        if (i->fusedSubScale) {
          readers[i->fMinuend].push_back({i, -1, 0});
          if (i->fAddend) readers[i->fAddend].push_back({i, i->ops == NTT && !i->fMix && i->fConvIn.empty() && !i->fAddendGalois ? 1 : -1, 0});
          if (i->fMix) readers[i->fMix].push_back({i, -1, 0});
        }
        if (i->fusedEpi) { readers[i->fSubFrom].push_back({i, -1, 0}); if (i->fAdd) readers[i->fAdd].push_back({i, -1, 0}); }
      }
    std::map<AddrType, size_t> lastWrite;
    for (size_t si = 0; si < st.size(); ++si)
      for (Instruction *i : st[si].ins) {
        if (dead.count(i)) continue;
        lastWrite[i->OutputOperand] = si;
        for (AddrType o : i->extraOutputs) lastWrite[o] = si;
      }
    std::map<AddrType, Instruction *> cand;
    bool anyOwn = false;
    for (size_t si = 0; si < st.size(); ++si)
      for (Instruction *A : st[si].ins) {
        if (A->ops != AUTO || dead.count(A) || A->galois <= 1) continue;
        { auto w = lastWrite.find(A->operandList[0]); if (w != lastWrite.end() && w->second >= si) continue; }
        auto r = readers.find(A->OutputOperand);
        if (r == readers.end() || r->second.empty()) continue;
        bool ok = true;
        for (const Reader &x : r->second) ok &= x.role >= 0 && x.ins->mod_id == A->mod_id && x.ins->OutputOperand != A->operandList[0];
        if (!ok) continue;
        cand[A->OutputOperand] = A;
        for (const Reader &x : r->second) anyOwn |= x.role == 2;
      }
    if (anyOwn) {
      uint32_t g0 = 0;
      bool uniform = true;
      for (const Reader &x : ownDigits) {
        auto c = cand.find((x.ins->ipSrc.empty() ? x.ins->ipX : x.ins->ipSrc)[x.digit]);
        if (c == cand.end() || (g0 && c->second->galois != g0)) { uniform = false; break; }
        g0 = c->second->galois;
      }
      if (!uniform)
        for (auto it = cand.begin(); it != cand.end();) {
          bool own = false;
          for (const Reader &x : readers[it->first]) own |= x.role == 2;
          it = own ? cand.erase(it) : std::next(it);
        }
    }
    for (auto &kv : cand) {
      Instruction *A = kv.second;
      auto &rd = readers[kv.first];
      for (const Reader &x : rd) {
        if (x.role == 0) { x.ins->operandList[0] = A->operandList[0]; x.ins->inGalois = A->galois; }
        else if (x.role == 1) { x.ins->fAddend = A->operandList[0]; x.ins->fAddendGalois = A->galois; }
        else {
          x.ins->ipX[x.digit] = A->operandList[0];
          if (!x.ins->ipSrc.empty()) x.ins->ipSrc[x.digit] = A->operandList[0];
          x.ins->ipXGalois = A->galois;
        }
      }
      rd.front().ins->refInstructions += A->refInstructions;
      dead.insert(A);
    }
  }
  unsigned long long orphan = 0;
  std::vector<Stage> keep;
  for (auto &s : st) {
    Stage t = s;
    t.ins.clear();
    for (Instruction *i : s.ins) {
      if (!dead.count(i)) t.ins.push_back(i);
      else if (i->passthrough) orphan += i->refInstructions;
    }
    if (!t.ins.empty()) keep.push_back(t);
  }
  if (!keep.empty()) keep[0].ins[0]->refInstructions += orphan;
  st.swap(keep);
}

void Arch::buildLaunches() {
  std::vector<Stage> st = stages;
  if (fuse) fusePasses(st);
  const unsigned long long LP = (unsigned long long)n * 8;
  const unsigned long long bconvPorts = (unsigned long long)config->getValueOr("bconv_num_high", 1) * config->getValueOr("bconv_num_width", 1);
  const int useMask[9] = {3, 15, 7, 5, 5, 1, 5, 1, 13};

  struct Part { std::string name; int key; std::vector<Instruction *> ins; int depth = 0; };
  std::vector<Part> parts;
  for (const Stage &s : st) {
    size_t first = parts.size();
    for (Instruction *i : s.ins) {
      const bool nip = i->ops == IP && std::find(i->ipCoeff.begin(), i->ipCoeff.end(), 1) != i->ipCoeff.end();
      int key = !i->ipHoistG.empty() ? 6000 + (int)i->ipX.size() * 100 + (int)i->ipHoistG.size() : nip ? 400 +(int)i->ipX.size() * 10 + (int)i->ipY.size() : i->ops == IP && !i->ipX.empty() ? 300 + (int)i->ipX.size() * 10 + (int)i->ipY.size() : i->fusedTensor ? 200 : i->fusedSubScale ? (i->fMix ? 203 : 201) + (i->fConvIn.empty() ? 0 : 4) : i->ops == MULT ? 100 + i->opcode : (i->ops == NTT && i->passthrough) ? 100 + EWE_COPY : i->ops == AUTO ? 1000 + (int)i->galois : (int)i->ops + (i->secondOnly ? 5000 : 0);
      size_t p = first;
      for (; p < parts.size(); ++p)
        if (parts[p].key == key) break;
      if (p == parts.size()) parts.push_back(Part{s.name, key, {}, 0});
      parts[p].ins.push_back(i);
    }
  }
  auto reads = [&](Instruction *i) {
    std::vector<AddrType> v;
    if (i->ops == IP && !i->ipX.empty()) {
      v = i->ipSrc.empty() ? i->ipX : i->ipSrc;
      for (size_t j = 0; j < i->ipConvIn.size(); ++j)
        if (!i->ipConvIn[j].empty()) { v[j] = i->ipConvIn[j][0]; v.insert(v.end(), i->ipConvIn[j].begin() + 1, i->ipConvIn[j].end()); }
      for (auto &y : i->ipY) v.insert(v.end(), y.begin(), y.end());
      return v;
    }
    if (i->ops == BCONV_STEP2) v.assign(i->operandList.begin(), i->operandList.end() - 1);
    else if (i->ops == MULT) { for (int b = 0; b < 4; ++b) if (useMask[i->opcode] & (1 << b)) v.push_back(i->operandList[b]); }
    else v.push_back(i->operandList[0]);
    if (i->fusedSubScale) { v.push_back(i->fMinuend); if (i->fAddend) v.push_back(i->fAddend); if (i->fMix) v.push_back(i->fMix); }
    if (!i->fConvIn.empty()) { v[0] = i->fConvIn[0]; v.insert(v.end(), i->fConvIn.begin() + 1, i->fConvIn.end()); }
    if (i->fusedEpi) { v.push_back(i->fSubFrom); if (i->fAdd) v.push_back(i->fAdd); }
    return v;
  };
  auto writes = [&](Instruction *i) {
    std::vector<AddrType> v = {i->OutputOperand};
    v.insert(v.end(), i->extraOutputs.begin(), i->extraOutputs.end());
    for (size_t j = 0; j < i->ipCoeff.size(); ++j)
      if (i->ipCoeff[j]) v.push_back(i->ipX[j]);
    return v;
  };
  std::map<AddrType, int> writerDepth, readerDepth;
  int serial = 0;
  for (Part &p : parts) {
    int d = 0;
    for (Instruction *i : p.ins) {
      for (AddrType a : reads(i)) { auto w = writerDepth.find(a); if (w != writerDepth.end()) d = std::max(d, w->second + 1); }
      for (AddrType o : writes(i)) {
        auto w = writerDepth.find(o); if (w != writerDepth.end()) d = std::max(d, w->second + 1);
        auto r = readerDepth.find(o); if (r != readerDepth.end()) d = std::max(d, r->second + 1);
      }
    }
    if (!fuse) d = serial++;
    p.depth = d;
    for (Instruction *i : p.ins) {
      for (AddrType a : reads(i)) { int &r = readerDepth[a]; r = std::max(r, d); }
      for (AddrType o : writes(i)) writerDepth[o] = d;
    }
  }
  std::map<AddrType, uint32_t> ownerOfAddr;
  if (world_ > 1) {
    for (const InputFill &f : fills)
      for (size_t i = 0; i < f.addrs.size(); ++i) ownerOfAddr[f.addrs[i]] = owner(f.mods[i]);
    for (const Part &p : parts)
      for (Instruction *i : p.ins)
        for (AddrType o : writes(i)) ownerOfAddr[o] = owner(i->mod_id);
  }
  const uint32_t logLen = logN - (uint32_t)__builtin_ctz(world_);
  std::map<AddrType, int> slotOfAddr;
  int nextSlot = 0;
  int maxDepth = 0;
  for (const Part &p : parts) maxDepth = std::max(maxDepth, p.depth);
  for (int d = 0; d <= maxDepth; ++d) {
    std::vector<int> keysDone;
    for (size_t pi = 0; pi < parts.size(); ++pi) {
      if (parts[pi].depth != d) continue;
      const int key = parts[pi].key;
      if (std::find(keysDone.begin(), keysDone.end(), key) != keysDone.end()) continue;
      keysDone.push_back(key);
      std::vector<const Part *> group;
      for (size_t pj = pi; pj < parts.size(); ++pj)
        if (parts[pj].depth == d && parts[pj].key == key) group.push_back(&parts[pj]);
      Instruction *f = group[0]->ins[0];
      std::vector<Part> mineParts;
      bool nipSharded = false;
      if (world_ > 1 && f->ops == IP && !shardGather)
        for (const Part *g : group)
          for (Instruction *i : g->ins)
            for (auto &cin : i->ipConvIn) nipSharded |= !cin.empty();
      if (nipSharded) {
        struct Dig { std::vector<uint32_t> in, inMods, hand, handMods; };
        std::vector<Dig> digs;
        for (const Part *g : group)
          for (Instruction *i : g->ins)
            for (size_t j = 0; j < i->ipConvIn.size(); ++j) {
              if (i->ipConvIn[j].empty()) continue;
              std::vector<uint32_t> in;
              for (AddrType x : i->ipConvIn[j]) in.push_back(limbOf(x));
              Dig *dg = nullptr;
              for (auto &q : digs) if (q.in == in && q.inMods == i->ipConvMods[j]) dg = &q;
              if (!dg) { digs.push_back(Dig{in, i->ipConvMods[j], {}, {}}); dg = &digs.back(); }
              dg->hand.push_back(limbOf(i->ipX[j]));
              dg->handMods.push_back(i->mod_id);
            }
        const uint32_t per = (uint32_t)limbIndex.size();
        std::vector<Launch *> front, back;
        std::vector<int> outSlots;
        const uint32_t nTiles = cap(logN, "cap_col_slices") / world_;
        for (size_t dj = 0; dj < digs.size(); ++dj) {
          Dig &dg = digs[dj];
          Launch *XI = new Launch, *BC = new Launch, *XO = new Launch;
          XI->kind = Launch::L_EXCH_IN_COL; BC->kind = Launch::L_BCONV_COL; XO->kind = Launch::L_EXCH_OUT_COL;
          XI->statKey = XO->statKey = "XCHG"; BC->statKey = "BCONV";
          BC->name = "ModUp_BCONV_COL_(" + std::to_string(dj) + ")";
          XI->name = BC->name + ":limbs->columns"; XO->name = BC->name + ":columns->limbs";
          for (uint32_t c = 0; c < batch_; ++c) {
            for (size_t x = 0; x < dg.in.size(); ++x) { XI->exLimbs.push_back(dg.in[x] + c * per); XI->exOwners.push_back(owner(dg.inMods[x])); }
            for (size_t x = 0; x < dg.hand.size(); ++x) { XO->exLimbs.push_back(dg.hand[x] + c * per); XO->exOwners.push_back(owner(dg.handMods[x])); }
          }
          std::vector<uint32_t> inRows(XI->exLimbs.size()), outRows(XO->exLimbs.size());
// ... 110 lines not shown
      } else subgroups.push_back(group);
      std::vector<Launch *> front, back;
      for (const std::vector<const Part *> &subgroup : subgroups) {
      const std::vector<const Part *> &group = subgroup;
      f = group[0]->ins[0];
      Launch *L = new Launch;
      if (pipelineDigits)
        for (const Part *g : group) for (int sl : slotsOf(g)) if (std::find(L->waitSlots.begin(), L->waitSlots.end(), sl) == L->waitSlots.end()) L->waitSlots.push_back(sl);
      for (const Part *g : group) L->name += (L->name.empty() ? "" : "+") + g->name;
      size_t count = 0;
      for (const Part *g : group)
        for (Instruction *i : g->ins) { L->refInstructions += i->refInstructions * (i->ops == BCONV_STEP2 ? bconvPorts : 1ull) + i->refExtra; ++count; }
      if (f->ops == IP && !f->ipHoistG.empty()) {
        L->kind = Launch::L_IP_HOISTED; L->statKey = "EWE";
        L->ipTerms = (uint32_t)f->ipX.size(); L->ipOuts = 2; L->hoistG = f->ipHoistG;
        const size_t R = f->ipHoistG.size();
        std::vector<Instruction *> recs;
        for (const Part *g : group) recs.insert(recs.end(), g->ins.begin(), g->ins.end());
        for (Instruction *i : recs) {
          if (i->ipHoistG != f->ipHoistG) { delete L; throw std::runtime_error("hoisted key product: the records of one launch rotate by different elements"); }
          for (AddrType x : i->ipX) L->a.push_back(limbOf(x));
          L->mods.push_back(i->mod_id);
        }
        for (size_t r = 0; r < R; ++r)
          for (Instruction *i : recs)
            for (size_t k = 0; k < 2; ++k) {
              for (AddrType y : i->ipY[r * 2 + k]) L->b.push_back(limbOf(y));
              L->out.push_back(limbOf(r == 0 && k == 0 ? i->OutputOperand : i->extraOutputs[r * 2 + k - 1]));
            }
        L->bytes = (unsigned long long)recs.size() * (L->ipTerms + 2 * R * L->ipTerms + 2 * R) * LP;
      } else if (f->ops == IP && std::find(f->ipCoeff.begin(), f->ipCoeff.end(), 1) != f->ipCoeff.end()) {
        L->kind = Launch::L_NTT_IP; L->statKey = "NTT";
        L->ipTerms = (uint32_t)f->ipX.size(); L->ipOuts = (uint32_t)f->ipY.size();
        unsigned long long lp = 0;
        for (const Part *g : group)
          for (Instruction *i : g->ins) {
            for (size_t j = 0; j < i->ipX.size(); ++j) {
              L->a.push_back(limbOf(i->ipSrc[j])); L->c.push_back(limbOf(i->ipX[j])); L->ipCoeff.push_back(i->ipCoeff[j]);
              lp += i->ipCoeff[j] ? 3 : 1;
            }
            for (size_t j = 0; j < i->ipConvIn.size(); ++j) {
              if (i->ipConvIn[j].empty()) continue;
              std::vector<uint32_t> in;
              for (AddrType x : i->ipConvIn[j]) in.push_back(limbOf(x));
              Launch::Prob *pr = nullptr;
              const bool pk = j < i->ipConvPacked.size() && i->ipConvPacked[j];
              for (auto &q : L->probs) if (q.in == in && q.inMods == i->ipConvMods[j] && q.inPacked == pk) pr = &q;
              if (!pr) { L->probs.push_back(Launch::Prob{in, i->ipConvMods[j], {}, {}}); pr = &L->probs.back(); pr->inPacked = pk; }
              pr->out.push_back(limbOf(i->ipX[j]));
              pr->outMods.push_back(i->mod_id);
              lp -= 1;
            }
            for (auto &y : i->ipY) for (AddrType yy : y) L->b.push_back(limbOf(yy));
            L->out.push_back(limbOf(i->OutputOperand));
            for (AddrType o : i->extraOutputs) L->out.push_back(limbOf(o));
            L->mods.push_back(i->mod_id);
            L->ipInv.push_back(i->ipInvOut ? 1 : 0);
            if (i->ipXGalois) L->xGalois = i->ipXGalois;
            lp += (unsigned long long)L->ipTerms * L->ipOuts + L->ipOuts;
          }
        for (auto &q : L->probs) lp += q.in.size();
        L->bytes = lp * LP;
      } else if (f->ops == IP && !f->ipX.empty()) {
        L->kind = Launch::L_IP; L->statKey = "EWE";
        L->ipTerms = (uint32_t)f->ipX.size(); L->ipOuts = (uint32_t)f->ipY.size();
        for (const Part *g : group)
          for (Instruction *i : g->ins) {
            for (AddrType x : i->ipX) L->a.push_back(limbOf(x));
            for (auto &y : i->ipY) for (AddrType yy : y) L->b.push_back(limbOf(yy));
            L->out.push_back(limbOf(i->OutputOperand));
            for (AddrType o : i->extraOutputs) L->out.push_back(limbOf(o));
            L->mods.push_back(i->mod_id);
            if (i->ipXGalois) L->xGalois = i->ipXGalois;
          }
        L->bytes = (unsigned long long)(L->ipTerms * (1 + L->ipOuts) + L->ipOuts) * LP * count;
      } else if (f->fusedTensor) {
        L->kind = Launch::L_TENSOR; L->statKey = "EWE";
        for (const Part *g : group)
          for (Instruction *i : g->ins) {
            L->a.push_back(limbOf(i->operandList[0])); L->b.push_back(limbOf(i->operandList[3]));
            L->c.push_back(limbOf(i->operandList[2])); L->d.push_back(limbOf(i->operandList[1]));
            L->out.push_back(limbOf(i->extraOutputs[0])); L->out1.push_back(limbOf(i->OutputOperand)); L->out2.push_back(limbOf(i->extraOutputs[1]));
            L->mods.push_back(i->mod_id);
          }
        L->bytes = 7 * LP * count;
      } else if (f->fusedSubScale) {
        L->kind = Launch::L_NTT_SUBSCALE; L->statKey = "NTT";
        bool anyAddend = false;
        bool anyAddGalois = false;
        for (const Part *g : group)
          for (Instruction *i : g->ins) { anyAddend |= i->fAddend != 0; anyAddGalois |= i->fAddendGalois != 0; }
        for (const Part *g : group)
          for (Instruction *i : g->ins) {
            L->a.push_back(limbOf(i->operandList[0])); L->b.push_back(limbOf(i->fMinuend));
            if (anyAddend) L->c.push_back(i->fAddend ? limbOf(i->fAddend) : HM_NO_LIMB);
            if (anyAddGalois) L->addGalois.push_back(i->fAddendGalois);
            L->out.push_back(limbOf(i->OutputOperand)); L->mods.push_back(i->mod_id); L->k.push_back(i->constant);
            if (f->fMix) {
              L->d.push_back(limbOf(i->fMix)); L->mixK.push_back(i->fMixConst);
              if (anyAddend) L->addK.push_back(i->fAddendConst ? i->fAddendConst : 1);
            }
          }
        L->hasK = true;
        L->bytes = (anyAddend ? 4 : 3) * LP * count;
        for (const Part *g : group)
          for (Instruction *i : g->ins) {
            if (i->fConvIn.empty()) continue;
            std::vector<uint32_t> in;
            for (AddrType x : i->fConvIn) in.push_back(limbOf(x));
            Launch::Prob *pr = nullptr;
            for (auto &q : L->probs) if (q.in == in && q.inMods == i->fConvMods && q.inPacked == i->inPacked) pr = &q;
            if (!pr) { L->probs.push_back(Launch::Prob{in, i->fConvMods, {}, {}}); pr = &L->probs.back(); pr->inPacked = i->inPacked; L->bytes += LP * in.size(); }
            pr->out.push_back(limbOf(i->OutputOperand));
            pr->outMods.push_back(i->mod_id);
            L->bytes -= LP;
          }
      } else if (f->ops == NTT && f->passthrough) {
        L->kind = Launch::L_EWE; L->opcode = EWE_COPY; L->statKey = "EWE";
        for (const Part *g : group)
          for (Instruction *i : g->ins) { L->a.push_back(limbOf(i->operandList[0])); L->out.push_back(limbOf(i->OutputOperand)); L->mods.push_back(i->mod_id); }
        L->bytes = 2 * LP * count;
      } else if (f->ops == NTT || f->ops == INTT) {
        L->kind = f->ops == NTT ? Launch::L_NTT : Launch::L_INTT; L->statKey = "NTT";
        L->secondOnly = f->secondOnly;
        bool anyInGalois = false;
        for (const Part *g : group)
          for (Instruction *i : g->ins) anyInGalois |= i->inGalois != 0;
        for (const Part *g : group)
          for (Instruction *i : g->ins) {
            if (anyInGalois) L->inGalois.push_back(i->inGalois);
            L->a.push_back(limbOf(i->operandList[0])); L->out.push_back(limbOf(i->OutputOperand)); L->mods.push_back(i->mod_id);
            L->k.push_back(i->hasConstant ? i->constant : 1);
            L->hasK |= i->hasConstant;
            if (f->ops == INTT) L->outPacked.push_back(i->packedOut ? 1 : 0);
          }
        L->bytes = 2 * LP * count;
      } else if (f->ops == AUTO) {
        L->kind = Launch::L_AUTO; L->statKey = "AUTO"; L->galois = f->galois;
        for (const Part *g : group)
          for (Instruction *i : g->ins) { L->a.push_back(limbOf(i->operandList[0])); L->out.push_back(limbOf(i->OutputOperand)); }
        L->bytes = 2 * LP * count;
      } else if (f->ops == MULT) {
        L->kind = Launch::L_EWE; L->opcode = f->opcode; L->statKey = "EWE";
        const int m = useMask[f->opcode];
        int nops = 1;
        for (int b = 0; b < 4; ++b) nops += (m >> b) & 1;
        std::vector<Instruction *> recs;
        for (const Part *g : group) recs.insert(recs.end(), g->ins.begin(), g->ins.end());
        std::stable_sort(recs.begin(), recs.end(), [](const Instruction *x, const Instruction *y) { return x->mod_id < y->mod_id; });
        for (Instruction *i : recs) {
          auto get = [&](int b) { return (m & (1 << b)) ? limbOf(i->operandList[b]) : 0u; };
          L->a.push_back(get(0)); L->b.push_back(get(1)); L->c.push_back(get(2)); L->d.push_back(get(3));
          L->out.push_back(limbOf(i->OutputOperand)); L->mods.push_back(i->mod_id);
          L->k.push_back(i->hasConstant ? i->constant : 0);
          L->hasK |= i->hasConstant;
        }
        L->bytes = (unsigned long long)nops * LP * count;
      } else if (f->ops == BCONV_STEP2) {
        L->kind = Launch::L_BCONV; L->statKey = "BCONV";
        for (const Part *g : group) {
          for (Instruction *i : g->ins) {
            std::vector<uint32_t> in;
            for (size_t x = 0; x + 1 < i->operandList.size(); ++x) in.push_back(limbOf(i->operandList[x]));
            Launch::Prob *pr = nullptr;
            for (auto &q : L->probs) if (q.in == in && q.inMods == i->inMods && q.epi == i->fusedEpi && q.epAdd == (i->fAdd != 0) && q.inPacked == i->inPacked) pr = &q;
            if (!pr) { L->probs.push_back(Launch::Prob{in, i->inMods, {}, {}}); pr = &L->probs.back(); pr->epi = i->fusedEpi; pr->epAdd = i->fAdd != 0; pr->inPacked = i->inPacked; }
            pr->out.push_back(limbOf(i->OutputOperand));
            pr->outMods.push_back(i->mod_id);
            if (i->fusedEpi) {
              pr->epA.push_back(limbOf(i->fSubFrom)); pr->epK.push_back(i->constant);
              if (i->fAdd) pr->epB.push_back(limbOf(i->fAdd));
              L->bytes += LP * (i->fAdd ? 2 : 1);
            }
          }
        }
        if (world_ > 1 && batch_ > 1 && !shardGather) {
          const uint32_t per = (uint32_t)limbIndex.size();
          const size_t p0 = L->probs.size();
          for (uint32_t c = 1; c < batch_; ++c)
            for (size_t i = 0; i < p0; ++i) {
              Launch::Prob q = L->probs[i];
              for (uint32_t &x : q.in) x += c * per;
              for (uint32_t &x : q.out) x += c * per;
              L->probs.push_back(q);
            }
          L->refInstructions *= batch_;
        }
        for (auto &q : L->probs) L->bytes += LP * (q.in.size() + q.out.size());
        if (world_ > 1 && !shardGather) {
          Launch *XI = new Launch, *XO = new Launch;
          XI->kind = Launch::L_EXCH_IN; XO->kind = Launch::L_EXCH_OUT; XI->statKey = XO->statKey = "XCHG";
          XI->name = L->name + ":limbs->slices"; XO->name = L->name + ":slices->limbs";
          std::vector<uint32_t> inOwn, outOwn;
          for (auto &q : L->probs) {
            for (size_t x = 0; x < q.in.size(); ++x) {
              size_t pos = std::find(XI->exLimbs.begin(), XI->exLimbs.end(), q.in[x]) - XI->exLimbs.begin();
              if (pos == XI->exLimbs.size()) { XI->exLimbs.push_back(q.in[x]); XI->exOwners.push_back(owner(q.inMods[x])); }
            }
            for (size_t x = 0; x < q.out.size(); ++x) { XO->exLimbs.push_back(q.out[x]); XO->exOwners.push_back(owner(q.outMods[x])); }
          }
          std::vector<uint32_t> inRows(XI->exLimbs.size()), outRows(XO->exLimbs.size());
          hm_slice_rows(XI->exOwners.data(), (uint32_t)inRows.size(), world_, inRows.data());
          hm_slice_rows(XO->exOwners.data(), (uint32_t)outRows.size(), world_, outRows.data());
          size_t o = 0;
          for (auto &q : L->probs) {
            for (uint32_t &x : q.in) x = inRows[std::find(XI->exLimbs.begin(), XI->exLimbs.end(), x) - XI->exLimbs.begin()];
            for (uint32_t &x : q.out) x = outRows[o++];
          }
          L->logLen = XI->logLen = XO->logLen = logLen;
          XI->bytes = LP * XI->exLimbs.size() / world_;
          XO->bytes = LP * XO->exLimbs.size() / world_;
          L->bytes /= world_;
// ... 25 lines not shown
  }
}

static const uint64_t kBatchSeedStride = 100000;
void Arch::replicateForBatch() {
  const uint32_t per = (uint32_t)limbIndex.size();
  std::set<uint32_t> sharedLimbs;
  for (const InputFill &f : fills)
    if (f.shared)
      for (AddrType a : f.addrs) sharedLimbs.insert(limbOf(a));
  auto rep = [&](std::vector<uint32_t> &v, bool isLimb) {
    const size_t n0 = v.size();
    for (uint32_t c = 1; c < batch_; ++c)
      for (size_t i = 0; i < n0; ++i) v.push_back(isLimb && v[i] != HM_NO_LIMB && !sharedLimbs.count(v[i]) ? v[i] + c * per : v[i]);
  };
  for (Launch *l : launches) {
    if (world_ > 1 && !shardGather && (l->kind == Launch::L_BCONV || l->kind == Launch::L_EXCH_IN || l->kind == Launch::L_EXCH_OUT)) continue;
    if (l->kind == Launch::L_BCONV_COL || l->kind == Launch::L_EXCH_IN_COL || l->kind == Launch::L_EXCH_OUT_COL) continue;
    if (l->kind == Launch::L_REPLICATE) {
      const size_t n0 = l->exLimbs.size();
      for (uint32_t c = 1; c < batch_; ++c)
        for (size_t i = 0; i < n0; ++i) { l->exLimbs.push_back(l->exLimbs[i] + c * per); l->exOwners.push_back(l->exOwners[i]); }
      l->bytes *= batch_;
      continue;
    }
    if (l->kind == Launch::L_IP_HOISTED) {
      const size_t n0 = l->mods.size();
      auto inter = [&](std::vector<uint32_t> &v, size_t blocks, size_t width, bool isLimb) {
        std::vector<uint32_t> o;
        for (size_t r = 0; r < blocks; ++r)
          for (size_t e = 0; e < n0; ++e)
            for (uint32_t c = 0; c < batch_; ++c)
              for (size_t w = 0; w < width; ++w) {
                const uint32_t x = v[(r * n0 + e) * width + w];
                o.push_back(isLimb && c && !sharedLimbs.count(x) ? x + c * per : x);
              }
        v.swap(o);
      };
      const size_t R = l->hoistG.size();
      inter(l->a, 1, l->ipTerms, true); inter(l->b, R, 2 * (size_t)l->ipTerms, true); inter(l->out, R, 2, true); inter(l->mods, 1, 1, false);
      l->refInstructions *= batch_;
      l->bytes *= batch_;
      continue;
    }
    if (l->kind == Launch::L_IP || l->kind == Launch::L_NTT_IP) {
      auto inter = [&](std::vector<uint32_t> &v, size_t width, bool isLimb) {
        const size_t n0 = v.size() / width;
        std::vector<uint32_t> o;
        for (size_t e = 0; e < n0; ++e)
          for (uint32_t c = 0; c < batch_; ++c)
            for (size_t w = 0; w < width; ++w) {
              const uint32_t x = v[e * width + w];
              o.push_back(isLimb && c && !sharedLimbs.count(x) ? x + c * per : x);
            }
        v.swap(o);
      };
      inter(l->a, l->ipTerms, true); inter(l->b, (size_t)l->ipTerms * l->ipOuts, true); inter(l->out, l->ipOuts, true); inter(l->mods, 1, false);
      if (l->kind == Launch::L_NTT_IP) {
        const size_t p0 = l->probs.size();
        for (uint32_t c = 1; c < batch_; ++c)
          for (size_t i = 0; i < p0; ++i) {
            Launch::Prob q = l->probs[i];
            for (uint32_t &x : q.in) x += c * per;
            for (uint32_t &x : q.out) x += c * per;
            for (uint32_t &x : q.epA) x += c * per;
            for (uint32_t &x : q.epB) x += c * per;
            l->probs.push_back(q);
          }
        inter(l->c, l->ipTerms, true);
        std::vector<uint32_t> f(l->ipCoeff.begin(), l->ipCoeff.end());
        inter(f, l->ipTerms, false);
        l->ipCoeff.assign(f.begin(), f.end());
        std::vector<uint32_t> fi(l->ipInv.begin(), l->ipInv.end());
        inter(fi, 1, false);
        l->ipInv.assign(fi.begin(), fi.end());
      }
    } else {
      {
        const size_t n0 = l->outPacked.size();
        for (uint32_t c = 1; c < batch_; ++c)
          for (size_t i = 0; i < n0; ++i) l->outPacked.push_back(l->outPacked[i]);
      }
      rep(l->a, true); rep(l->b, true); rep(l->c, true); rep(l->d, true);
      rep(l->out, true); rep(l->out1, true); rep(l->out2, true); rep(l->mods, false);
      rep(l->inGalois, false); rep(l->addGalois, false);
      for (std::vector<uint64_t> *kv : {&l->k, &l->mixK, &l->addK}) {
        const size_t k0 = kv->size();
        for (uint32_t c = 1; c < batch_; ++c)
          for (size_t i = 0; i < k0; ++i) kv->push_back((*kv)[i]);
      }
      const size_t p0 = l->probs.size();
      for (uint32_t c = 1; c < batch_; ++c)
        for (size_t i = 0; i < p0; ++i) {
          Launch::Prob q = l->probs[i];
          for (uint32_t &x : q.in) x += c * per;
          for (uint32_t &x : q.out) x += c * per;
          for (uint32_t &x : q.epA) x += c * per;
          for (uint32_t &x : q.epB) x += c * per;
          l->probs.push_back(q);
        }
    }
    l->refInstructions *= batch_;
    l->bytes *= batch_;
  }
  algBytes *= batch_;
}

void Arch::prepare() {
  if (prepared) return;
  prepared = true;
  buildLaunches();
  if (batch_ > 1) {
    replicateForBatch();
    stat->setStat("Batch", batch_);
  }
  stat->setStat("Launches", launches.size());
  stat->setStat("LimbPolys_resident", limbIndex.size());
  stat->setStat("HBM_stage_bytes", algBytes);
  if (backendKind != BACKEND_HIP) return;
  const size_t bytes = (size_t)limbIndex.size() * batch_ * n * 8;
  void *p = nullptr;
  if (hm_malloc(ctx, bytes, &p) != HM_OK) throw std::runtime_error(std::string("hm_malloc: ") + hm_last_error(ctx));
  pool = static_cast<uint64_t *>(p);
  if (world_ > 1) {
    if (!commReady) throw std::runtime_error("world > 1 but no transport was set (commInitRccl / commInitExternal)");
    if (pipelineDigits && hm_exchange_stream(ctx, 1) != HM_OK) throw std::runtime_error(std::string("hm_exchange_stream: ") + hm_last_error(ctx));
    for (Launch *bc : launches) {
      if (bc->kind != Launch::L_BCONV_COL || !bc->xin) continue;
      Launch *xi = bc->xin, *xo = bc->xout;
      void *si = nullptr, *so = nullptr;
      if (hm_malloc(ctx, (size_t)xi->exLimbs.size() * n * 8, &si) != HM_OK || hm_malloc(ctx, (size_t)xo->exLimbs.size() * n * 8, &so) != HM_OK)
        throw std::runtime_error(std::string("hm_malloc (column slices): ") + hm_last_error(ctx));
      sliceBuffers.push_back(si); sliceBuffers.push_back(so);
      xi->slicesIn = bc->slicesIn = static_cast<uint64_t *>(si);
      bc->slicesOut = xo->slicesOut = static_cast<uint64_t *>(so);
    }
    for (Launch *bc : launches) {
      if (bc->kind != Launch::L_BCONV || !bc->xin) continue;
      Launch *xi = bc->xin, *xo = bc->xout;
      void *si = nullptr, *so = nullptr;
      if (hm_malloc(ctx, (size_t)xi->exLimbs.size() * (n / world_) * 8, &si) != HM_OK || hm_malloc(ctx, (size_t)xo->exLimbs.size() * (n / world_) * 8, &so) != HM_OK)
        throw std::runtime_error(std::string("hm_malloc (slices): ") + hm_last_error(ctx));
      sliceBuffers.push_back(si); sliceBuffers.push_back(so);
      xi->slicesIn = bc->slicesIn = static_cast<uint64_t *>(si);
      bc->slicesOut = xo->slicesOut = static_cast<uint64_t *>(so);
    }
  }
  std::set<AddrType> bound;
  for (Binding &b : bindings) {
    if (!b.src->prepared) throw std::runtime_error("bindInput: prepare the producer first");
    for (size_t i = 0; i < b.dst.size(); ++i)
      for (uint32_t c = 0; c < batch_; ++c) {
        b.dstLimbs.push_back(limbOf(b.dst[i]) + c * (uint32_t)limbIndex.size());
        b.srcLimbs.push_back(b.src->limbOf(b.srcAddrs[i]) + c * (uint32_t)b.src->limbIndex.size());
        b.mods.push_back(0);
      }
    bound.insert(b.dst.begin(), b.dst.end());
  }
  for (const InputFill &f : fills)
    for (uint32_t c = 0; c < (f.shared ? 1u : batch_); ++c) {
      if (!f.addrs.empty() && bound.count(f.addrs[0])) continue;
      std::vector<uint32_t> limbs;
      for (AddrType a : f.addrs) limbs.push_back(limbOf(a) + c * (uint32_t)limbIndex.size());
      if (hm_fill_uniform(ctx, pool, limbs.data(), f.mods.data(), (uint32_t)limbs.size(), f.seed + c * kBatchSeedStride) != HM_OK)
        throw std::runtime_error(std::string("hm_fill_uniform: ") + hm_last_error(ctx));
    }
  hm_sync(ctx);
}

static const char *const kLaunchKindNames[] = {"NTT", "INTT", "EWE", "BCONV", "AUTO", "NTT_SUBSCALE", "TENSOR", "EXCH_IN", "EXCH_OUT", "REPLICATE", "IP", "NTT_IP",
                                               "BCONV_COL", "EXCH_IN_COL", "EXCH_OUT_COL", "IP_HOISTED"};

std::string Arch::stageTimes(uint32_t iters) {
  if (!prepared) prepare();
  if (backendKind != BACKEND_HIP) return "";
  std::vector<uint64_t> total(launches.size(), 0);
  for (uint32_t it = 0; it < iters; ++it)
    for (size_t i = 0; i < launches.size(); ++i) {
      hm_timer_start(ctx);
      enqueue(*launches[i]);
      if (launches[i]->recordSlot >= 0) hm_exchange_wait(ctx, (uint32_t)launches[i]->recordSlot);
      uint64_t ns = 0;
      hm_timer_stop(ctx, &ns);
      total[i] += ns;
    }
  std::string out;
  for (size_t i = 0; i < launches.size(); ++i)
    out += std::string(kLaunchKindNames[launches[i]->kind]) + " " + launches[i]->name + " " + std::to_string(total[i] / (iters ? iters : 1)) + "\n";
  return out;
}

std::string Arch::planText() const {
  const char *const *names = kLaunchKindNames;
  std::string out;
  for (const Launch *l : launches) {
    size_t cnt = l->out.size();
    if (l->kind == Launch::L_BCONV || l->kind == Launch::L_BCONV_COL) { cnt = 0; for (auto &q : l->probs) cnt += q.out.size(); }
    if (l->kind == Launch::L_IP || l->kind == Launch::L_NTT_IP || l->kind == Launch::L_IP_HOISTED) cnt = l->mods.size();
    out += std::string(names[l->kind]) + " " + l->name + " n=" + std::to_string(cnt) + " ref=" + std::to_string(l->refInstructions);
    const size_t po = (size_t)std::count(l->outPacked.begin(), l->outPacked.end(), 1), pi = (size_t)std::count_if(l->probs.begin(), l->probs.end(), [](const Launch::Prob &q) { return q.inPacked; });
    if (po) out += " packed_out=" + std::to_string(po);
    if (pi) out += " packed_in=" + std::to_string(pi) + "/" + std::to_string(l->probs.size());
    if (l->secondOnly) out += " second_pass_only";
    for (const auto *gv : {&l->inGalois, &l->addGalois}) {
      uint32_t cnt = 0, g = 0;
      for (uint32_t x : *gv) if (x > 1) { ++cnt; g = x; }
      if (cnt) out += std::string(gv == &l->inGalois ? " auto_in=" : " auto_addend=") + std::to_string(cnt) + "/g" + std::to_string(g);
    }
    if (l->xGalois) out += " auto_x=g" + std::to_string(l->xGalois);
    if (!l->hoistG.empty()) {
      out += " rot=" + std::to_string(l->hoistG.size()) + " g=";
      for (size_t r = 0; r < l->hoistG.size(); ++r) out += (r ? "," : "") + std::to_string(l->hoistG[r]);
    }
    if (l->recordSlot >= 0) out += " mark=" + std::to_string(l->recordSlot);
    if (!l->waitSlots.empty()) { out += " wait="; for (int w : l->waitSlots) out += std::to_string(w) + ","; }
    if (!l->exLimbs.empty()) {
      out += " limbs=";
      for (size_t i = 0; i < l->exLimbs.size(); ++i) out += std::to_string(l->exLimbs[i]) + ":" + std::to_string(l->exOwners[i]) + ",";
    }
    out += "\n";
  }
  return out;
}

void Arch::enqueue(Launch &l) {
  hm_status st = HM_OK;
  for (int sl : l.waitSlots)
    if (hm_exchange_wait(ctx, (uint32_t)sl) != HM_OK) throw std::runtime_error("stage " + l.name + ": " + hm_last_error(ctx));
  const uint32_t cnt = (uint32_t)l.out.size();
  std::vector<hm_bconv_desc> descs;
  switch (l.kind) {
  case Launch::L_NTT:
    st = hm_ntt(ctx, pool, l.a.data(), pool, l.out.data(), l.mods.data(), cnt, 0, nullptr);
    break;
  case Launch::L_INTT: {
    const bool anyPacked = std::find(l.outPacked.begin(), l.outPacked.end(), 1) != l.outPacked.end();
    hm_ntt_desc d = {pool, l.a.data(), pool, l.out.data(), l.mods.data(), cnt, 1, l.hasK ? l.k.data() : nullptr, l.secondOnly ? 1 : 0,
                     anyPacked ? l.outPacked.data() : nullptr, l.inGalois.empty() ? nullptr : l.inGalois.data()};
    st = hm_ntt_ex(ctx, &d);
    break;
  }
  case Launch::L_NTT_SUBSCALE:
    if (!l.mixK.empty() || !l.probs.empty() || !l.addGalois.empty()) {
      for (auto &q : l.probs)
        descs.push_back(hm_bconv_desc{pool, q.in.data(), q.inMods.data(), (uint32_t)q.in.size(), pool, q.out.data(), q.outMods.data(), (uint32_t)q.out.size(), 0,
                                    nullptr, nullptr, nullptr, nullptr, nullptr, q.inPacked ? 1u : 0u});
      hm_ntt_fused_desc d = {pool, l.a.data(), l.mixK.empty() ? nullptr : pool, l.mixK.empty() ? nullptr : l.d.data(), l.mixK.empty() ? nullptr : l.mixK.data(), pool, l.b.data(),
                             l.c.empty() ? nullptr : pool, l.c.empty() ? nullptr : l.c.data(), l.addK.empty() ? nullptr : l.addK.data(), pool, l.out.data(), l.mods.data(), cnt,
                             l.k.data(), descs.empty() ? nullptr : descs.data(), (uint32_t)descs.size(), l.addGalois.empty() ? nullptr : l.addGalois.data()};
      st = hm_ntt_mix_sub_scale(ctx, &d);
    } else {
      st = hm_ntt_sub_scale(ctx, pool, l.a.data(), pool, l.b.data(), l.c.empty() ? nullptr : pool, l.c.empty() ? nullptr : l.c.data(), pool,
                            l.out.data(), l.mods.data(), cnt, l.k.data());
    }
    break;
  case Launch::L_IP:
    if (l.xGalois) {
      const hm_ip_desc d = {pool, l.a.data(), pool, l.b.data(), pool, l.out.data(), l.mods.data(), (uint32_t)l.mods.size(), l.ipTerms, l.ipOuts, l.xGalois};
      st = hm_inner_product_ex(ctx, &d);
    } else
    st = hm_inner_product(ctx, pool, l.a.data(), pool, l.b.data(), pool, l.out.data(), l.mods.data(), (uint32_t)l.mods.size(), l.ipTerms, l.ipOuts);
    break;
  case Launch::L_IP_HOISTED: {
    const hm_ip_hoisted_desc d = {pool, l.a.data(), pool, l.b.data(), pool, l.out.data(), l.mods.data(), (uint32_t)l.mods.size(), l.ipTerms,
                                  (uint32_t)l.hoistG.size(), l.hoistG.data()};
    st = hm_inner_product_hoisted(ctx, &d);
    break;
  }
  case Launch::L_NTT_IP: {
    for (auto &q : l.probs)
      descs.push_back(hm_bconv_desc{pool, q.in.data(), q.inMods.data(), (uint32_t)q.in.size(), pool, q.out.data(), q.outMods.data(), (uint32_t)q.out.size(), 0,
                                    nullptr, nullptr, nullptr, nullptr, nullptr, q.inPacked ? 1u : 0u});
    hm_ntt_ip_desc d = {pool, l.a.data(), l.ipCoeff.data(), pool, l.c.data(), pool, l.b.data(), pool, l.out.data(), l.mods.data(),
                        (uint32_t)l.mods.size(), l.ipTerms, l.ipOuts, descs.empty() ? nullptr : descs.data(), (uint32_t)descs.size(),
                        std::find(l.ipInv.begin(), l.ipInv.end(), 1) != l.ipInv.end() ? l.ipInv.data() : nullptr, l.xGalois};
    st = hm_ntt_inner_product(ctx, &d);
    break;
  }
  case Launch::L_TENSOR:
    st = hm_tensor(ctx, pool, l.a.data(), pool, l.b.data(), pool, l.c.data(), pool, l.d.data(), pool, l.out.data(), pool, l.out1.data(), pool,
                   l.out2.data(), l.mods.data(), cnt);
    break;
  case Launch::L_EXCH_IN:
    st = hm_limbs_to_slices(ctx, pool, l.exLimbs.data(), l.exOwners.data(), (uint32_t)l.exLimbs.size(), l.slicesIn);
    break;
  case Launch::L_EXCH_OUT:
    st = hm_slices_to_limbs(ctx, l.slicesOut, pool, l.exLimbs.data(), l.exOwners.data(), (uint32_t)l.exLimbs.size());
    break;
  case Launch::L_EXCH_IN_COL:
    st = hm_limbs_to_colslices(ctx, pool, l.exLimbs.data(), l.exOwners.data(), (uint32_t)l.exLimbs.size(), l.slicesIn);
    break;
  case Launch::L_EXCH_OUT_COL:
    st = hm_colslices_to_limbs(ctx, l.slicesOut, pool, l.exLimbs.data(), l.exOwners.data(), (uint32_t)l.exLimbs.size());
    break;
  case Launch::L_BCONV_COL:
    for (auto &q : l.probs)
      descs.push_back(hm_bconv_desc{l.slicesIn, q.in.data(), q.inMods.data(), (uint32_t)q.in.size(), l.slicesOut, q.out.data(), q.outMods.data(), (uint32_t)q.out.size(), 0});
    st = hm_bconv_col(ctx, descs.data(), (uint32_t)descs.size(), l.galois, l.logLen);
    break;
  case Launch::L_REPLICATE:
    st = hm_replicate_limbs(ctx, pool, l.exLimbs.data(), l.exOwners.data(), (uint32_t)l.exLimbs.size());
    break;
  case Launch::L_AUTO:
    st = hm_automorph(ctx, pool, l.a.data(), pool, l.out.data(), cnt, l.galois);
    break;
  case Launch::L_EWE:
    st = hm_ewe(ctx, l.opcode, pool, l.a.data(), pool, l.b.empty() ? nullptr : l.b.data(), pool, l.c.empty() ? nullptr : l.c.data(), pool,
                l.d.empty() ? nullptr : l.d.data(), pool, l.out.data(), l.mods.data(), cnt, l.hasK ? l.k.data() : nullptr);
    break;
  case Launch::L_BCONV:
    for (auto &q : l.probs)
      descs.push_back(hm_bconv_desc{l.slicesIn ? l.slicesIn : pool, q.in.data(), q.inMods.data(), (uint32_t)q.in.size(),
                                    l.slicesOut ? l.slicesOut : pool, q.out.data(), q.outMods.data(), (uint32_t)q.out.size(), l.logLen,
                                    q.epi ? pool : nullptr, q.epi ? q.epA.data() : nullptr, q.epAdd ? pool : nullptr, q.epAdd ? q.epB.data() : nullptr,
                                    q.epi ? q.epK.data() : nullptr, q.inPacked ? 1u : 0u});
    st = hm_bconv_batch(ctx, descs.data(), (uint32_t)descs.size());
    break;
  }
  if (st == HM_OK && l.recordSlot >= 0) st = hm_exchange_mark(ctx, (uint32_t)l.recordSlot);
  if (st != HM_OK) throw std::runtime_error("stage " + l.name + ": " + hm_last_error(ctx));
}

void Arch::update() {
  if (backendKind == BACKEND_SIM) {
    if (!sim) throw std::runtime_error("sim backend: no program loaded");
    sim->step();
    return;
  }
  if (!prepared) prepare();
  if (nextLaunch >= launches.size()) return;
  Launch &l = *launches[nextLaunch++];
  if (backendKind == BACKEND_HIP) {
    hm_timer_start(ctx);
    enqueue(l);
    if (l.recordSlot >= 0) hm_exchange_wait(ctx, (uint32_t)l.recordSlot);
    uint64_t ns = 0;
    hm_timer_stop(ctx, &ns);
    elapsedNs += ns;
    stat->increaseStat(l.statKey + "_(0)", ns);
  }
  stat->increaseStat(l.statKey + "_launches");
  completedIns += l.refInstructions;
}

bool Arch::simulateComplete() { return sim ? sim->complete() : prepared && nextLaunch >= launches.size(); }
unsigned long long Arch::getCycle() { return sim ? sim->cycle() : elapsedNs; }
unsigned long long Arch::getcompletedIns() { return sim ? sim->completedIns() : completedIns; }

void Arch::state() {
  if (sim) { std::cout << sim->describe(); return; }
  std::cout << "launched " << nextLaunch << " of " << launches.size() << " stages\n";
  if (nextLaunch < launches.size()) std::cout << "next: " << launches[nextLaunch]->name << "\n";
}

void Arch::shownStat() {
  if (sim) {
    std::cout << "Start outPut statistic informations:\n";
    std::cout << "=====================================\n";
    for (const auto &kv : sim->stats()) std::cout << kv.first << " :\t" << kv.second << "\n";
    return;
  }
  stat->setStat("Total_ns", elapsedNs);
// ... 109 lines not shown
```

### include/homulator_hip.h

```cpp
#ifndef HOMULATOR_HIP_H
#define HOMULATOR_HIP_H
#include <stddef.h>
#include <stdint.h>
#ifdef __cplusplus
extern "C" {
#endif

typedef struct hm_ctx hm_ctx;
typedef int hm_status;
enum { HM_OK = 0, HM_ERR_ARG = 1, HM_ERR_HIP = 2, HM_ERR_UNSUPPORTED = 3, HM_ERR_COMM = 4 };

typedef struct hm_params {
  uint32_t logN, L, K;
  int32_t device;
  const uint64_t *q, *p;
  const uint64_t *psi;
} hm_params;

hm_status hm_create(hm_ctx **ctx, const hm_params *params);
void hm_destroy(hm_ctx *ctx);
const char *hm_last_error(const hm_ctx *ctx);
const char *hm_version(void);

hm_status hm_get_modulus(const hm_ctx *ctx, uint32_t mod_id, uint64_t *q);
hm_status hm_get_psi(const hm_ctx *ctx, uint32_t mod_id, uint64_t *psi);

hm_status hm_malloc(hm_ctx *ctx, size_t bytes, void **dptr);
hm_status hm_free(hm_ctx *ctx, void *dptr);
hm_status hm_memcpy_h2d(hm_ctx *ctx, void *dst, const void *src, size_t bytes);
hm_status hm_memcpy_d2h(hm_ctx *ctx, void *dst, const void *src, size_t bytes);
hm_status hm_memcpy_d2d(hm_ctx *ctx, void *dst, const void *src, size_t bytes);
hm_status hm_sync(hm_ctx *ctx);
void *hm_stream(hm_ctx *ctx);
hm_status hm_wait_for(hm_ctx *ctx, hm_ctx *producer);


hm_status hm_ntt(hm_ctx *ctx, const uint64_t *in, const uint32_t *in_limbs, uint64_t *out,
                 const uint32_t *out_limbs, const uint32_t *mod_ids, uint32_t n, int inverse,
                 const uint64_t *scale);

hm_status hm_ntt_sub_scale(hm_ctx *ctx, const uint64_t *in, const uint32_t *in_limbs, const uint64_t *minuend,
                           const uint32_t *minuend_limbs, const uint64_t *addend, const uint32_t *addend_limbs,
                           uint64_t *out, const uint32_t *out_limbs, const uint32_t *mod_ids, uint32_t n,
                           const uint64_t *k);

#define HM_NO_LIMB 0xFFFFFFFFu
struct hm_bconv_desc;
typedef struct hm_ntt_fused_desc {
  const uint64_t *in;      const uint32_t *in_limbs;
  const uint64_t *mix;     const uint32_t *mix_limbs;     const uint64_t *mix_k;
  const uint64_t *minuend; const uint32_t *minuend_limbs;
  const uint64_t *addend;  const uint32_t *addend_limbs;  const uint64_t *addend_k;
  uint64_t *out;           const uint32_t *out_limbs;
  const uint32_t *mod_ids; uint32_t n;
  const uint64_t *k;
  const struct hm_bconv_desc *conv; uint32_t n_conv;
  const uint32_t *addend_galois;
} hm_ntt_fused_desc;
hm_status hm_ntt_mix_sub_scale(hm_ctx *ctx, const hm_ntt_fused_desc *desc);

hm_status hm_automorph(hm_ctx *ctx, const uint64_t *in, const uint32_t *in_limbs, uint64_t *out,
                       const uint32_t *out_limbs, uint32_t n, uint32_t galois);

enum hm_ewe_op {
  HM_OP_MUL = 0,
  HM_OP_MAC2 = 1,
  HM_OP_MAC_ADD = 2,
  HM_OP_ADD = 3,
  HM_OP_SUB = 4,
  HM_OP_MUL_CONST = 5,
  HM_OP_SUB_SCALE = 6,
  HM_OP_COPY = 7,
  HM_OP_SUB_SCALE_ADD = 8
};
hm_status hm_ewe(hm_ctx *ctx, int op, const uint64_t *a, const uint32_t *a_limbs, const uint64_t *b,
                 const uint32_t *b_limbs, const uint64_t *c, const uint32_t *c_limbs, const uint64_t *d,
                 const uint32_t *d_limbs, uint64_t *out, const uint32_t *out_limbs,
                 const uint32_t *mod_ids, uint32_t n, const uint64_t *k);

hm_status hm_tensor(hm_ctx *ctx, const uint64_t *a, const uint32_t *a_limbs, const uint64_t *b, const uint32_t *b_limbs,
                    const uint64_t *c, const uint32_t *c_limbs, const uint64_t *d, const uint32_t *d_limbs,
                    uint64_t *o0, const uint32_t *o0_limbs, uint64_t *o1, const uint32_t *o1_limbs, uint64_t *o2,
                    const uint32_t *o2_limbs, const uint32_t *mod_ids, uint32_t n);

hm_status hm_inner_product(hm_ctx *ctx, const uint64_t *x, const uint32_t *x_limbs, const uint64_t *y,
                           const uint32_t *y_limbs, uint64_t *out, const uint32_t *out_limbs,
                           const uint32_t *mod_ids, uint32_t n, uint32_t n_terms, uint32_t n_out);
typedef struct hm_ip_desc {
  const uint64_t *x;  const uint32_t *x_limbs;
  const uint64_t *y;  const uint32_t *y_limbs;
  uint64_t *out;      const uint32_t *out_limbs;
  const uint32_t *mod_ids;
  uint32_t n, n_terms, n_out;
  uint32_t x_galois;
} hm_ip_desc;
hm_status hm_inner_product_ex(hm_ctx *ctx, const hm_ip_desc *desc);
#define HM_IP_HOISTED_MAX_ROT 16
typedef struct hm_ip_hoisted_desc {
  const uint64_t *x;  const uint32_t *x_limbs;
  const uint64_t *y;  const uint32_t *y_limbs;
  uint64_t *out;      const uint32_t *out_limbs;
  const uint32_t *mod_ids;
  uint32_t n, n_terms, n_rot;
  const uint32_t *galois;
} hm_ip_hoisted_desc;
hm_status hm_inner_product_hoisted(hm_ctx *ctx, const hm_ip_hoisted_desc *desc);

struct hm_bconv_desc;
typedef struct hm_ntt_ip_desc {
  const uint64_t *x;    const uint32_t *x_limbs;   const uint8_t *x_is_coeff;
  uint64_t *hand;       const uint32_t *hand_limbs;
  const uint64_t *y;    const uint32_t *y_limbs;
  uint64_t *out;        const uint32_t *out_limbs;
  const uint32_t *mod_ids;
  uint32_t n, n_terms, n_out;
  const struct hm_bconv_desc *conv; uint32_t n_conv;
  const uint8_t *out_inverse;
  uint32_t x_galois;
} hm_ntt_ip_desc;
hm_status hm_ntt_inner_product(hm_ctx *ctx, const hm_ntt_ip_desc *desc);
hm_status hm_ntt_second_pass(hm_ctx *ctx, uint64_t *buf, const uint32_t *limbs, const uint32_t *mod_ids, uint32_t n, int inverse,
                             const uint64_t *scale);
typedef struct hm_ntt_desc {
  const uint64_t *in;  const uint32_t *in_limbs;
  uint64_t *out;       const uint32_t *out_limbs;
  const uint32_t *mod_ids; uint32_t n;
  int inverse;         const uint64_t *scale;
  int second_pass_only;
  const uint8_t *out_packed;
  const uint32_t *in_galois;
} hm_ntt_desc;
hm_status hm_ntt_ex(hm_ctx *ctx, const hm_ntt_desc *desc);

hm_status hm_bconv(hm_ctx *ctx, const uint64_t *in, const uint32_t *in_limbs, const uint32_t *in_ids,
                   uint32_t n_in, uint64_t *out, const uint32_t *out_limbs, const uint32_t *out_ids,
                   uint32_t n_out);
typedef struct hm_bconv_desc hm_bconv_desc;
struct hm_bconv_desc {
  const uint64_t *in; const uint32_t *in_limbs; const uint32_t *in_ids; uint32_t n_in;
  uint64_t *out; const uint32_t *out_limbs; const uint32_t *out_ids; uint32_t n_out;
  uint32_t log_len;
  const uint64_t *sub_from; const uint32_t *sub_from_limbs; const uint64_t *add; const uint32_t *add_limbs; const uint64_t *sub_k;
  uint32_t in_packed;
};
hm_status hm_bconv_batch(hm_ctx *ctx, const hm_bconv_desc *descs, uint32_t n_desc);
hm_status hm_bconv_col(hm_ctx *ctx, const hm_bconv_desc *descs, uint32_t n_desc, uint32_t tile0, uint32_t n_tiles);
hm_status hm_bconv_consts(hm_ctx *ctx, const uint32_t *in_ids, uint32_t n_in, const uint32_t *out_ids,
                          uint32_t n_out, uint64_t *qhat_inv, uint64_t *table);

typedef int (*hm_exchange_fn)(void *user, const void *send_dev, const size_t *send_off, const size_t *send_bytes,
                              void *recv_dev, const size_t *recv_off, const size_t *recv_bytes);
hm_status hm_comm_unique_id(void *out128);
hm_status hm_comm_init_rccl(hm_ctx *ctx, int rank, int world, const void *unique_id128);
hm_status hm_comm_init_external(hm_ctx *ctx, int rank, int world, hm_exchange_fn fn, void *user);
hm_status hm_comm_info(const hm_ctx *ctx, int *rank, int *world);
hm_status hm_slice_rows(const uint32_t *owners, uint32_t n, uint32_t world, uint32_t *rows);
hm_status hm_limbs_to_slices(hm_ctx *ctx, const uint64_t *buf, const uint32_t *limbs, const uint32_t *owners,
                             uint32_t n, uint64_t *slices);
hm_status hm_slices_to_limbs(hm_ctx *ctx, const uint64_t *slices, uint64_t *buf, const uint32_t *limbs,
                             const uint32_t *owners, uint32_t n);
hm_status hm_limbs_to_colslices(hm_ctx *ctx, const uint64_t *buf, const uint32_t *limbs, const uint32_t *owners,
                                uint32_t n, uint64_t *slices);
hm_status hm_colslices_to_limbs(hm_ctx *ctx, const uint64_t *slices, uint64_t *buf, const uint32_t *limbs,
                                const uint32_t *owners, uint32_t n);

hm_status hm_exchange_stream(hm_ctx *ctx, int enable);
// ... 26 lines not shown
```

Baseline: 5536.

## Fuse first inverse-NTT pass into tensor kernel for key-switch input

Adds a k_tensor_inv kernel that computes the tensor product and then runs the first inverse-NTT pass on the d2 output in registers and LDS, writing a half-transformed limb to an inverse-out buffer. The scheduler marks the following INTT as second-pass-only for those limbs and splits INTT launches into a second-only part and a full part. This removes one global round-trip and one NTT pass launch for the relinearisation input. In exchange it adds an extra output stream, higher register and LDS pressure in the tensor kernel, and more scheduler complexity.

New measurement: 5540 (median of 6 runs). No clear change (+0.1%).

```diff
diff --git a/homulator_amd/csrc/hm_backend.hip b/homulator_amd/csrc/hm_backend.hip
--- a/homulator_amd/csrc/hm_backend.hip
+++ b/homulator_amd/csrc/hm_backend.hip
@@ -370,6 +370,73 @@
   *reinterpret_cast<ulonglong2 *>(a.o0 + (size_t)lb.o0 * N + x) = r0;
   *reinterpret_cast<ulonglong2 *>(a.o1 + (size_t)lb.o1 * N + x) = r1;
   *reinterpret_cast<ulonglong2 *>(a.o2 + (size_t)lb.o2 * N + x) = r2;
+}
+
+struct HmTensorInvLimb {
+  uint16_t a, b, c, d, o0, o1, o2, inv;
+  uint16_t mod, pad;
+};
+#define HM_TENSOR_INV_MAX 192
+struct HmTensorInvArgs {
+  const uint64_t *a, *b, *c, *d;
+  uint64_t *o0, *o1, *o2, *inv;
+  const HmW *tw_inv, *twist_inv;
+  const HmMod *mods;
+  uint32_t logN, n_limbs, logG;
+  HmTensorInvLimb limb[HM_TENSOR_INV_MAX];
+};
+#ifndef HM_TENSOR_INV_CH
+#define HM_TENSOR_INV_CH 2
+#endif
+__global__ void __launch_bounds__((1 << HM_TL_ROW) / HM_EPT) __attribute__((amdgpu_waves_per_eu(HM_NTT_MIN_WAVES))) k_tensor_inv(HmTensorInvArgs a) {
+  constexpr int TL = HM_TL_ROW, LOGR = HM_ROW_LOG, R2 = hm16::HmRounds<LOGR>::n - 1, CH = HM_TENSOR_INV_CH;
+  static_assert(HM_UNITS % CH == 0, "whole steps");
+  using G = hm16::HmRound<TL, LOGR, false, R2>;
+  __shared__ __attribute__((aligned(16))) uint64_t lds[hm16::HmLds<TL, LOGR, false>::WORDS];
+  uint32_t entry, tile;
+  if (!hm_block_map(1u << (a.logN - TL), a.n_limbs, a.logG, entry, tile)) return;
+  const HmTensorInvLimb lb = a.limb[entry];
+  if (lb.mod == HM_NTT_NONE) return;
+  const size_t N = (size_t)1 << a.logN;
+  const HmMod m = HM_CONST_MODS(a.mods)[lb.mod];
+  const uint64_t *pa = a.a + (size_t)lb.a * N, *pb = a.b + (size_t)lb.b * N, *pc = a.c + (size_t)lb.c * N, *pd = a.d + (size_t)lb.d * N;
+  uint64_t *p0 = a.o0 + (size_t)lb.o0 * N, *p1 = a.o1 + (size_t)lb.o1 * N, *p2 = a.o2 + (size_t)lb.o2 * N;
+  hm16::HmNttState st;
+  const int tid = threadIdx.x;
+#pragma unroll
+  for (int u = 0; u < HM_UNITS; u += CH) {
+    uint64_t va[2 * CH], vb[2 * CH], vc[2 * CH], vd[2 * CH];
+#pragma unroll
+    for (int k = 0; k < CH; ++k) {
+      hm_gld2<G>(pa, tile, tid, u + k, va[2 * k], va[2 * k + 1]);
+      hm_gld2<G>(pb, tile, tid, u + k, vb[2 * k], vb[2 * k + 1]);
+      hm_gld2<G>(pc, tile, tid, u + k, vc[2 * k], vc[2 * k + 1]);
+      hm_gld2<G>(pd, tile, tid, u + k, vd[2 * k], vd[2 * k + 1]);
+    }
+#pragma unroll
+    for (int k = 0; k < CH; ++k) {
+      int i0, i1, x, c;
+      G::unit(tid, u + k, i0, i1, x, c);
+      uint64_t x0, x1, y0, y1;
+      hm_tensor_one(va[2 * k], vb[2 * k], vc[2 * k], vd[2 * k], m, x0, x1, st.v[i0]);
+      hm_tensor_one(va[2 * k + 1], vb[2 * k + 1], vc[2 * k + 1], vd[2 * k + 1], m, y0, y1, st.v[i1]);
+      hm_gst2<G>(p0, tile, tid, u + k, x0, y0);
+      hm_gst2<G>(p1, tile, tid, u + k, x1, y1);
+      hm_gst2<G>(p2, tile, tid, u + k, st.v[i0], st.v[i1]);
+    }
+  }
+  if (lb.inv == HM_NTT_NONE) return;
+  const HmW *twl = a.tw_inv + (size_t)lb.mod * N;
+  const uint32_t s0 = a.logN - LOGR, prefix0 = tile << (TL - LOGR);
+  const HmW *twt = a.twist_inv + ((size_t)lb.mod * (N >> LOGR) + prefix0) * 3;
+  int tid2 = threadIdx.x;
+  asm volatile("" : "+v"(tid2));
+  __builtin_assume(tid2 >= 0 && tid2 < (1 << TL) / HM_EPT);
+  const HmTw sc = {0, 0};
+  const HmEpi ep = hm_epi_none();
+  int nsync = 0;
+  hm16::hm_ntt_pass_phases<TL, LOGR, false, true, 0, 0, 0, HM_EPI_CHUNK, true>(st, tid2, lds, nullptr, a.inv + (size_t)lb.inv * N, tile, twl, twt, s0,
+      prefix0, m.q, sc, ep, [&] { hm_pass_sync<false>(nsync++); });
 }
 
 #ifndef HM_EWE_UNITS
@@ -1409,6 +1476,93 @@
                                (uint16_t)limb_at(l0, g), (uint16_t)limb_at(l1, g), (uint16_t)limb_at(l2, g), (uint16_t)mod_ids[g]};
     }
     hipLaunchKernelGGL(k_tensor, dim3(cnt * (c->P.N / 512)), dim3(256), 0, c->stream, a);
+    HM_HIP(c, hipGetLastError());
+  }
+  return HM_OK;
+}
+
+static bool limb_ranges_overlap(const uint64_t *ob, const uint32_t *ol, uint32_t no, const uint64_t *ib, const uint32_t *il, uint32_t ni, uint32_t N);
+extern "C" hm_status hm_tensor_ex(hm_ctx *c, const hm_tensor_desc *d) {
+  if (!c) return HM_ERR_ARG;
+  if (!d) return fail(c, HM_ERR_ARG, "hm_tensor_ex: null descriptor");
+  const uint32_t n = d->n, N = c->P.N;
+  std::vector<uint32_t> inv;
+  for (uint32_t i = 0; d->inv_out && i < n; ++i) {
+    const uint32_t l = limb_at(d->inv_out_limbs, i);
+    if (l == HM_NO_LIMB) continue;
+    if (l >= 0xFFFFu) return fail(c, HM_ERR_ARG, "hm_tensor_ex: inverse-out limb index %u exceeds 65534", l);
+    inv.push_back(l);
+  }
+  if (inv.empty())
+    return hm_tensor(c, d->a, d->a_limbs, d->b, d->b_limbs, d->c, d->c_limbs, d->d, d->d_limbs, d->o0, d->o0_limbs, d->o1, d->o1_limbs, d->o2,
+                     d->o2_limbs, d->mod_ids, n);
+  if (!hm_caps(c->P.logN).tensor_inverse_out) return fail(c, HM_ERR_UNSUPPORTED, "hm_tensor_ex: inv_out is not served at N = 2^%u", c->P.logN);
+  if (!d->a || !d->b || !d->c || !d->d || !d->o0 || !d->o1 || !d->o2) return fail(c, HM_ERR_ARG, "hm_tensor_ex: null buffer");
+  hm_status st;
+  const uint32_t *lists[7] = {d->a_limbs, d->b_limbs, d->c_limbs, d->d_limbs, d->o0_limbs, d->o1_limbs, d->o2_limbs};
+  for (auto l : lists)
+    if ((st = check_limbs(c, "hm_tensor_ex", l, n))) return st;
+  if ((st = check_mods(c, "hm_tensor_ex", d->mod_ids, n))) return st;
+  {
+    const uint64_t *bases[7] = {d->a, d->b, d->c, d->d, d->o0, d->o1, d->o2};
+    static const char *const names[7] = {"a", "b", "c", "d", "o0", "o1", "o2"};
+    for (int k = 0; k < 7; ++k) {
+      std::vector<uint32_t> l(n);
+      for (uint32_t i = 0; i < n; ++i) l[i] = limb_at(lists[k], i);
+      if (limb_ranges_overlap(d->inv_out, inv.data(), (uint32_t)inv.size(), bases[k], l.data(), n, N))
+        return fail(c, HM_ERR_ARG, "hm_tensor_ex: an inverse-out limb-poly overlaps a limb-poly of %s", names[k]);
+    }
+    std::vector<uint32_t> s = inv;
+    std::sort(s.begin(), s.end());
+    if (std::adjacent_find(s.begin(), s.end()) != s.end()) return fail(c, HM_ERR_ARG, "hm_tensor_ex: an inverse-out limb appears twice");
+  }
+  HM_HIP(c, hipSetDevice(c->device));
+  std::map<uint32_t, std::vector<int>> byMod;
+  for (uint32_t i = 0; i < n; ++i) byMod[d->mod_ids[i]].push_back((int)i);
+  uint32_t logG = 0;
+  for (uint32_t lg = 3; lg >= 1; --lg) {
+    size_t full = 0;
+    for (auto &kv : byMod) full += kv.second.size() >> lg << lg;
+    if (full * 8 >= (size_t)n * 7) { logG = lg; break; }
+  }
+  const uint32_t G = 1u << logG;
+  std::vector<std::vector<int>> groups;
+  {
+    std::vector<int> rest;
+    for (auto &kv : byMod) {
+      auto &v = kv.second;
+      size_t i = 0;
+      for (; i + G <= v.size(); i += G) groups.emplace_back(v.begin() + i, v.begin() + i + G);
+      rest.insert(rest.end(), v.begin() + i, v.end());
+    }
+    for (size_t i = 0; i < rest.size(); i += G) {
+      std::vector<int> g(rest.begin() + i, rest.begin() + std::min(rest.size(), i + G));
+      g.resize(G, -1);
+      groups.push_back(g);
+    }
+  }
+  const uint32_t maxGroups = HM_TENSOR_INV_MAX / G / 8 * 8;
+  const uint32_t nLaunch = ((uint32_t)groups.size() + maxGroups - 1) / maxGroups;
+  const uint32_t perLaunch = (((uint32_t)groups.size() + nLaunch - 1) / nLaunch + 7) / 8 * 8;
+  for (uint32_t base = 0; base < groups.size(); base += perLaunch) {
+    const uint32_t ng = std::min<uint32_t>(perLaunch, (uint32_t)groups.size() - base);
+    const uint32_t cnt = ((ng + 7) / 8) * 8 * G;
+    HmTensorInvArgs a;
+    for (uint32_t e = 0; e < cnt; ++e) a.limb[e] = HmTensorInvLimb{0, 0, 0, 0, 0, 0, 0, (uint16_t)HM_NTT_NONE, (uint16_t)HM_NTT_NONE, 0};
+    for (uint32_t kk = 0; kk < ng; ++kk)
+      for (uint32_t which = 0; which < G; ++which) {
+        const int gi = groups[base + kk][which];
+        if (gi < 0) continue;
+        const uint32_t g = (uint32_t)gi, e = (kk / 8) * 8 * G + which * 8 + (kk % 8);
+        const uint32_t il = limb_at(d->inv_out_limbs, g);
+        a.limb[e] = HmTensorInvLimb{(uint16_t)limb_at(d->a_limbs, g), (uint16_t)limb_at(d->b_limbs, g), (uint16_t)limb_at(d->c_limbs, g),
+                                    (uint16_t)limb_at(d->d_limbs, g), (uint16_t)limb_at(d->o0_limbs, g), (uint16_t)limb_at(d->o1_limbs, g),
+                                    (uint16_t)limb_at(d->o2_limbs, g), (uint16_t)(il == HM_NO_LIMB ? HM_NTT_NONE : il), (uint16_t)d->mod_ids[g], 0};
+      }
+    a.a = d->a; a.b = d->b; a.c = d->c; a.d = d->d; a.o0 = d->o0; a.o1 = d->o1; a.o2 = d->o2; a.inv = d->inv_out;
+    a.tw_inv = c->d_tw_inv; a.twist_inv = c->d_twist_inv; a.mods = c->d_mods;
+    a.logN = c->P.logN; a.n_limbs = cnt; a.logG = logG;
+    hipLaunchKernelGGL(k_tensor_inv, dim3(cnt * (N >> HM_TL_ROW)), dim3((1 << HM_TL_ROW) / HM_EPT), 0, c->stream, a);
     HM_HIP(c, hipGetLastError());
   }
   return HM_OK;
diff --git a/homulator_amd/csrc/hm_caps.h b/homulator_amd/csrc/hm_caps.h
--- a/homulator_amd/csrc/hm_caps.h
+++ b/homulator_amd/csrc/hm_caps.h
@@ -12,12 +12,14 @@
   uint32_t bcol_max_in_mix;
   uint32_t ip_inverse_out;
   uint32_t col_slices;
+  uint32_t tensor_inverse_out;
 };
 static inline HmCaps hm_caps(uint32_t logN) {
   switch (logN) {
-  case 16: return HmCaps{1, HM_BCOL_MAX_IN, 15, HM_BCOL_MAX_IN_MIX, 1, 16};
-  case 15: return HmCaps{1, HM_BCOL_MAX_IN, HM_BCOL_MAX_IN, HM_BCOL_MAX_IN_MIX, 1, 8};
-  default: return HmCaps{0, 0, 0, 0, 0, 0};
+  case 16: return HmCaps{1, HM_BCOL_MAX_IN, 15, HM_BCOL_MAX_IN_MIX, 1, 16, 1};
+  case 15: return HmCaps{1, HM_BCOL_MAX_IN, HM_BCOL_MAX_IN, HM_BCOL_MAX_IN_MIX, 1, 8, 1};
+  case 13: case 14: case 17: return HmCaps{0, 0, 0, 0, 0, 0, 1};
+  default: return HmCaps{0, 0, 0, 0, 0, 0, 0};
   }
 }
 static inline int hm_cap_by_name(uint32_t logN, const char *name, uint64_t *value) {
@@ -28,5 +30,6 @@
   if (!strcmp(name, "cap_bconv_col_pref_in")) { *value = c.bcol_pref_in; return 0; }
   if (!strcmp(name, "cap_ip_inverse_out")) { *value = c.ip_inverse_out; return 0; }
   if (!strcmp(name, "cap_col_slices")) { *value = c.col_slices; return 0; }
+  if (!strcmp(name, "cap_tensor_inverse_out")) { *value = c.tensor_inverse_out; return 0; }
   return 1;
 }
diff --git a/homulator_amd/csrc/hm_dispatch_gen.inc b/homulator_amd/csrc/hm_dispatch_gen.inc
--- a/homulator_amd/csrc/hm_dispatch_gen.inc
+++ b/homulator_amd/csrc/hm_dispatch_gen.inc
@@ -20,6 +20,7 @@
   hm_status (*automorph)(hm_ctx *ctx, const uint64_t *in, const uint32_t *in_limbs, uint64_t *out, const uint32_t *out_limbs, uint32_t n, uint32_t galois);
   hm_status (*ewe)(hm_ctx *ctx, int op, const uint64_t *a, const uint32_t *a_limbs, const uint64_t *b, const uint32_t *b_limbs, const uint64_t *c, const uint32_t *c_limbs, const uint64_t *d, const uint32_t *d_limbs, uint64_t *out, const uint32_t *out_limbs, const uint32_t *mod_ids, uint32_t n, const uint64_t *k);
   hm_status (*tensor)(hm_ctx *ctx, const uint64_t *a, const uint32_t *a_limbs, const uint64_t *b, const uint32_t *b_limbs, const uint64_t *c, const uint32_t *c_limbs, const uint64_t *d, const uint32_t *d_limbs, uint64_t *o0, const uint32_t *o0_limbs, uint64_t *o1, const uint32_t *o1_limbs, uint64_t *o2, const uint32_t *o2_limbs, const uint32_t *mod_ids, uint32_t n);
+  hm_status (*tensor_ex)(hm_ctx *ctx, const hm_tensor_desc *desc);
   hm_status (*inner_product)(hm_ctx *ctx, const uint64_t *x, const uint32_t *x_limbs, const uint64_t *y, const uint32_t *y_limbs, uint64_t *out, const uint32_t *out_limbs, const uint32_t *mod_ids, uint32_t n, uint32_t n_terms, uint32_t n_out);
   hm_status (*inner_product_ex)(hm_ctx *ctx, const hm_ip_desc *desc);
   hm_status (*inner_product_hoisted)(hm_ctx *ctx, const hm_ip_hoisted_desc *desc);
@@ -76,6 +77,7 @@
   a.automorph = reinterpret_cast<decltype(a.automorph)>(dlsym(h, "hm_automorph")); if (!a.automorph) return "hm_automorph";
   a.ewe = reinterpret_cast<decltype(a.ewe)>(dlsym(h, "hm_ewe")); if (!a.ewe) return "hm_ewe";
   a.tensor = reinterpret_cast<decltype(a.tensor)>(dlsym(h, "hm_tensor")); if (!a.tensor) return "hm_tensor";
+  a.tensor_ex = reinterpret_cast<decltype(a.tensor_ex)>(dlsym(h, "hm_tensor_ex")); if (!a.tensor_ex) return "hm_tensor_ex";
   a.inner_product = reinterpret_cast<decltype(a.inner_product)>(dlsym(h, "hm_inner_product")); if (!a.inner_product) return "hm_inner_product";
   a.inner_product_ex = reinterpret_cast<decltype(a.inner_product_ex)>(dlsym(h, "hm_inner_product_ex")); if (!a.inner_product_ex) return "hm_inner_product_ex";
   a.inner_product_hoisted = reinterpret_cast<decltype(a.inner_product_hoisted)>(dlsym(h, "hm_inner_product_hoisted")); if (!a.inner_product_hoisted) return "hm_inner_product_hoisted";
@@ -127,6 +129,7 @@
 extern "C" hm_status hm_automorph(hm_ctx *ctx, const uint64_t *in, const uint32_t *in_limbs, uint64_t *out, const uint32_t *out_limbs, uint32_t n, uint32_t galois) { if (!ctx) return HM_ERR_ARG; HM_FORWARDED(ctx); return HM_API(ctx).automorph(HM_IMPL(ctx), in, in_limbs, out, out_limbs, n, galois); }
 extern "C" hm_status hm_ewe(hm_ctx *ctx, int op, const uint64_t *a, const uint32_t *a_limbs, const uint64_t *b, const uint32_t *b_limbs, const uint64_t *c, const uint32_t *c_limbs, const uint64_t *d, const uint32_t *d_limbs, uint64_t *out, const uint32_t *out_limbs, const uint32_t *mod_ids, uint32_t n, const uint64_t *k) { if (!ctx) return HM_ERR_ARG; HM_FORWARDED(ctx); return HM_API(ctx).ewe(HM_IMPL(ctx), op, a, a_limbs, b, b_limbs, c, c_limbs, d, d_limbs, out, out_limbs, mod_ids, n, k); }
 extern "C" hm_status hm_tensor(hm_ctx *ctx, const uint64_t *a, const uint32_t *a_limbs, const uint64_t *b, const uint32_t *b_limbs, const uint64_t *c, const uint32_t *c_limbs, const uint64_t *d, const uint32_t *d_limbs, uint64_t *o0, const uint32_t *o0_limbs, uint64_t *o1, const uint32_t *o1_limbs, uint64_t *o2, const uint32_t *o2_limbs, const uint32_t *mod_ids, uint32_t n) { if (!ctx) return HM_ERR_ARG; HM_FORWARDED(ctx); return HM_API(ctx).tensor(HM_IMPL(ctx), a, a_limbs, b, b_limbs, c, c_limbs, d, d_limbs, o0, o0_limbs, o1, o1_limbs, o2, o2_limbs, mod_ids, n); }
+extern "C" hm_status hm_tensor_ex(hm_ctx *ctx, const hm_tensor_desc *desc) { if (!ctx) return HM_ERR_ARG; HM_FORWARDED(ctx); return HM_API(ctx).tensor_ex(HM_IMPL(ctx), desc); }
 extern "C" hm_status hm_inner_product(hm_ctx *ctx, const uint64_t *x, const uint32_t *x_limbs, const uint64_t *y, const uint32_t *y_limbs, uint64_t *out, const uint32_t *out_limbs, const uint32_t *mod_ids, uint32_t n, uint32_t n_terms, uint32_t n_out) { if (!ctx) return HM_ERR_ARG; HM_FORWARDED(ctx); return HM_API(ctx).inner_product(HM_IMPL(ctx), x, x_limbs, y, y_limbs, out, out_limbs, mod_ids, n, n_terms, n_out); }
 extern "C" hm_status hm_inner_product_ex(hm_ctx *ctx, const hm_ip_desc *desc) { if (!ctx) return HM_ERR_ARG; HM_FORWARDED(ctx); return HM_API(ctx).inner_product_ex(HM_IMPL(ctx), desc); }
 extern "C" hm_status hm_inner_product_hoisted(hm_ctx *ctx, const hm_ip_hoisted_desc *desc) { if (!ctx) return HM_ERR_ARG; HM_FORWARDED(ctx); return HM_API(ctx).inner_product_hoisted(HM_IMPL(ctx), desc); }
diff --git a/homulator_amd/hip.py b/homulator_amd/hip.py
--- a/homulator_amd/hip.py
+++ b/homulator_amd/hip.py
@@ -16,7 +16,7 @@
     "hm_capture_begin", "hm_capture_end", "hm_graph_launch", "hm_graph_destroy", "hm_comm_info", "hm_slice_rows", "hm_limbs_to_slices", "hm_slices_to_limbs", "hm_replicate_limbs",
     "hm_set_option", "hm_get_counter", "hm_ntt_inner_product", "hm_exchange_stream", "hm_exchange_mark", "hm_exchange_wait",
     "hm_bconv_col", "hm_limbs_to_colslices", "hm_colslices_to_limbs", "hm_ntt_second_pass", "hm_ntt_ex", "hm_capability", "hm_inner_product_ex",
-    "hm_inner_product_hoisted",
+    "hm_inner_product_hoisted", "hm_tensor_ex",
 ]
 
 
@@ -42,6 +42,11 @@
                 ("y", C.c_void_p), ("y_limbs", C.c_void_p), ("out", C.c_void_p), ("out_limbs", C.c_void_p), ("mod_ids", C.c_void_p),
                 ("n", C.c_uint32), ("n_terms", C.c_uint32), ("n_out", C.c_uint32), ("conv", C.c_void_p), ("n_conv", C.c_uint32),
                 ("out_inverse", C.c_void_p), ("x_galois", C.c_uint32)]
+
+
+class hm_tensor_desc(C.Structure):
+    _fields_ = [(k, C.c_void_p) for k in ("a", "a_limbs", "b", "b_limbs", "c", "c_limbs", "d", "d_limbs", "o0", "o0_limbs", "o1", "o1_limbs",
+                                          "o2", "o2_limbs", "mod_ids")] + [("n", C.c_uint32), ("inv_out", C.c_void_p), ("inv_out_limbs", C.c_void_p)]
 
 
 class hm_bconv_desc(C.Structure):
@@ -98,6 +103,7 @@
     L.hm_ntt_sub_scale.argtypes = [vp] + [vp] * 9 + [u32, vp]
     L.hm_ntt_mix_sub_scale.argtypes = [vp, C.POINTER(hm_ntt_fused_desc)]
     L.hm_tensor.argtypes = [vp] + [vp] * 15 + [u32]
+    L.hm_tensor_ex.argtypes = [vp, C.POINTER(hm_tensor_desc)]
     L.hm_inner_product.argtypes = [vp] + [vp] * 7 + [u32, u32, u32]
     L.hm_automorph.argtypes = [vp, vp, vp, vp, vp, u32, u32]
     L.hm_ewe.argtypes = [vp, i32] + [vp] * 11 + [u32, vp]
@@ -260,9 +266,15 @@
                               kg[1])
         self._ck(self.L.hm_ntt_mix_sub_scale(self.h, C.byref(d)))
 
-    def tensor(self, a, b, c, d, o0, o1, o2, mod_ids, limbs=None):
+    def tensor(self, a, b, c, d, o0, o1, o2, mod_ids, limbs=None, inv_out=None, inv_out_limbs=None):
         ls = limbs or [None] * 7
         keep = [_u32(x) for x in ls] + [_u32(mod_ids)]
+        if inv_out is not None:
+            ki = _u32(inv_out_limbs)
+            desc = hm_tensor_desc(a.ptr, keep[0][1], b.ptr, keep[1][1], c.ptr, keep[2][1], d.ptr, keep[3][1], o0.ptr, keep[4][1], o1.ptr, keep[5][1],
+                                  o2.ptr, keep[6][1], keep[7][1], len(mod_ids), inv_out.ptr, ki[1])
+            self._ck(self.L.hm_tensor_ex(self.h, C.byref(desc)))
+            return
         self._ck(self.L.hm_tensor(self.h, a.ptr, keep[0][1], b.ptr, keep[1][1], c.ptr, keep[2][1], d.ptr, keep[3][1], o0.ptr, keep[4][1],
                                   o1.ptr, keep[5][1], o2.ptr, keep[6][1], keep[7][1], len(mod_ids)))
 
diff --git a/host/include/Arch.h b/host/include/Arch.h
--- a/host/include/Arch.h
+++ b/host/include/Arch.h
@@ -87,6 +87,7 @@
   bool fuseHpip = true;
   bool fuseBconv = true;
   bool fuseIpInv = true;
+  bool fuseTensorInv = false;
   bool packBconvIn = true;
   bool fuseAuto = true;
   bool fuseModDown = true;
diff --git a/host/include/Instruction.h b/host/include/Instruction.h
--- a/host/include/Instruction.h
+++ b/host/include/Instruction.h
@@ -34,6 +34,7 @@
   std::vector<uint32_t> fConvMods;
   bool ipInvOut = false;
   bool secondOnly = false;
+  bool handFromTensor = false;
   bool packedOut = false;
   bool inPacked = false;
   std::vector<uint8_t> ipConvPacked;
@@ -42,6 +43,7 @@
   bool fusedEpi = false;
   AddrType fSubFrom = 0, fAdd = 0;
   bool fusedTensor = false;
+  AddrType tensorInvOut = 0;
   std::vector<AddrType> extraOutputs;
   std::vector<AddrType> ipX;
   std::vector<std::vector<AddrType>> ipY;
diff --git a/host/src/Arch.cpp b/host/src/Arch.cpp
--- a/host/src/Arch.cpp
+++ b/host/src/Arch.cpp
@@ -26,6 +26,7 @@
   std::vector<uint8_t> ipCoeff;
   std::vector<uint8_t> ipInv;
   bool secondOnly = false;
+  uint32_t nSecond = 0;
   std::vector<uint8_t> outPacked;
   std::vector<uint32_t> inGalois, addGalois;
   uint32_t xGalois = 0;
@@ -35,6 +36,7 @@
   int opcode = 0;
   uint32_t galois = 0;
   std::vector<uint32_t> a, b, c, d, out, out1, out2, mods, inMods;
+  std::vector<uint32_t> invOut;
   struct Prob { std::vector<uint32_t> in, inMods, out, outMods, epA, epB; std::vector<uint64_t> epK; bool epi = false, epAdd = false, inPacked = false; };
   std::vector<Prob> probs;
   std::vector<uint32_t> exLimbs, exOwners;
@@ -83,6 +85,8 @@
   if (const char *e = getenv("HOMULATOR_FUSE_BCONV")) fuseBconv = std::string(e) != "0";
   fuseIpInv = cfg->getValueOr("fuse_ip_inv", 1) != 0;
   if (const char *e = getenv("HOMULATOR_FUSE_IP_INV")) fuseIpInv = std::string(e) != "0";
+  fuseTensorInv = cfg->getValueOr("fuse_tensor_inv", 0) != 0;
+  if (const char *e = getenv("HOMULATOR_FUSE_TENSOR_INV")) fuseTensorInv = std::string(e) != "0";
   packBconvIn = cfg->getValueOr("pack_bconv_in", 1) != 0;
   if (const char *e = getenv("HOMULATOR_PACK_BCONV_IN")) packBconvIn = std::string(e) != "0";
   fuseAuto = cfg->getValueOr("fuse_auto", 1) != 0;
@@ -705,6 +709,48 @@
       for (Instruction *x : s.ins)
         if (x->ops == INTT && !dead.count(x) && read.count(x->OutputOperand)) x->packedOut = true;
   }
+  if (fuseTensorInv && (world_ == 1 || shardGather) && cap(logN, "cap_tensor_inverse_out")) {
+    std::map<AddrType, std::vector<Instruction *>> readers;
+    std::map<AddrType, std::vector<std::pair<size_t, Instruction *>>> touched;
+    for (size_t si = 0; si < st.size(); ++si)
+      for (Instruction *i : st[si].ins) {
+        if (dead.count(i)) continue;
+        std::vector<AddrType> rd;
+        if (i->ops == IP && !i->ipX.empty()) {
+          rd = i->ipSrc.empty() ? i->ipX : i->ipSrc;
+          for (auto &cin : i->ipConvIn) rd.insert(rd.end(), cin.begin(), cin.end());
+          for (auto &y : i->ipY) rd.insert(rd.end(), y.begin(), y.end());
+        } else {
+          rd = operands(i);
+          rd.insert(rd.end(), i->fConvIn.begin(), i->fConvIn.end());
+          if (i->fusedSubScale) { rd.push_back(i->fMinuend); if (i->fAddend) rd.push_back(i->fAddend); if (i->fMix) rd.push_back(i->fMix); }
+          if (i->fusedEpi) { rd.push_back(i->fSubFrom); if (i->fAdd) rd.push_back(i->fAdd); }
+        }
+        for (AddrType a : rd) { readers[a].push_back(i); touched[a].push_back({si, i}); }
+        touched[i->OutputOperand].push_back({si, i});
+        for (AddrType o : i->extraOutputs) touched[o].push_back({si, i});
+      }
+    std::map<Instruction *, size_t> stageOf;
+    for (size_t si = 0; si < st.size(); ++si)
+      for (Instruction *i : st[si].ins) stageOf[i] = si;
+    for (auto &s : st)
+      for (Instruction *t : s.ins) {
+        if (!t->fusedTensor || dead.count(t) || t->tensorInvOut || t->extraOutputs.size() != 2) continue;
+        const AddrType d2 = t->extraOutputs[1];
+        Instruction *x = nullptr;
+        int nIntt = 0;
+        for (Instruction *r : readers[d2])
+          if (r->ops == INTT) { ++nIntt; x = r; }
+        if (nIntt != 1 || x->mod_id != t->mod_id || x->secondOnly || x->inGalois || !x->fConvIn.empty() || x->operandList[0] != d2) continue;
+        bool early = false;
+        for (const auto &w : touched[x->OutputOperand]) early |= w.second != x && w.first <= stageOf[x];
+        if (early) continue;
+        t->tensorInvOut = x->OutputOperand;
+        x->operandList[0] = x->OutputOperand;
+        x->secondOnly = true;
+        x->handFromTensor = true;
+      }
+  }
   if (fuseAuto) {
     struct Reader { Instruction *ins; int role; size_t digit; };
     std::map<AddrType, std::vector<Reader>> readers;
@@ -740,6 +786,7 @@
         if (dead.count(i)) continue;
         lastWrite[i->OutputOperand] = si;
         for (AddrType o : i->extraOutputs) lastWrite[o] = si;
+        if (i->tensorInvOut) lastWrite[i->tensorInvOut] = si;
       }
     std::map<AddrType, Instruction *> cand;
     bool anyOwn = false;
@@ -814,7 +861,7 @@
     size_t first = parts.size();
     for (Instruction *i : s.ins) {
       const bool nip = i->ops == IP && std::find(i->ipCoeff.begin(), i->ipCoeff.end(), 1) != i->ipCoeff.end();
-      int key = !i->ipHoistG.empty() ? 6000 + (int)i->ipX.size() * 100 + (int)i->ipHoistG.size() : nip ? 400 +(int)i->ipX.size() * 10 + (int)i->ipY.size() : i->ops == IP && !i->ipX.empty() ? 300 + (int)i->ipX.size() * 10 + (int)i->ipY.size() : i->fusedTensor ? 200 : i->fusedSubScale ? (i->fMix ? 203 : 201) + (i->fConvIn.empty() ? 0 : 4) : i->ops == MULT ? 100 + i->opcode : (i->ops == NTT && i->passthrough) ? 100 + EWE_COPY : i->ops == AUTO ? 1000 + (int)i->galois : (int)i->ops + (i->secondOnly ? 5000 : 0);
+      int key = !i->ipHoistG.empty() ? 6000 + (int)i->ipX.size() * 100 + (int)i->ipHoistG.size() : nip ? 400 +(int)i->ipX.size() * 10 + (int)i->ipY.size() : i->ops == IP && !i->ipX.empty() ? 300 + (int)i->ipX.size() * 10 + (int)i->ipY.size() : i->fusedTensor ? 200 : i->fusedSubScale ? (i->fMix ? 203 : 201) + (i->fConvIn.empty() ? 0 : 4) : i->ops == MULT ? 100 + i->opcode : (i->ops == NTT && i->passthrough) ? 100 + EWE_COPY : i->ops == AUTO ? 1000 + (int)i->galois : (int)i->ops + (i->secondOnly && !i->handFromTensor ? 5000 : 0);
       size_t p = first;
       for (; p < parts.size(); ++p)
         if (parts[p].key == key) break;
@@ -842,6 +889,7 @@
   auto writes = [&](Instruction *i) {
     std::vector<AddrType> v = {i->OutputOperand};
     v.insert(v.end(), i->extraOutputs.begin(), i->extraOutputs.end());
+    if (i->tensorInvOut) v.push_back(i->tensorInvOut);
     for (size_t j = 0; j < i->ipCoeff.size(); ++j)
       if (i->ipCoeff[j]) v.push_back(i->ipX[j]);
     return v;
@@ -1118,8 +1166,12 @@
             L->c.push_back(limbOf(i->operandList[2])); L->d.push_back(limbOf(i->operandList[1]));
             L->out.push_back(limbOf(i->extraOutputs[0])); L->out1.push_back(limbOf(i->OutputOperand)); L->out2.push_back(limbOf(i->extraOutputs[1]));
             L->mods.push_back(i->mod_id);
+            L->invOut.push_back(i->tensorInvOut ? limbOf(i->tensorInvOut) : HM_NO_LIMB);
           }
         L->bytes = 7 * LP * count;
+        const size_t nInv = (size_t)std::count_if(L->invOut.begin(), L->invOut.end(), [](uint32_t l) { return l != HM_NO_LIMB; });
+        if (nInv) L->bytes += LP * nInv;
+        else L->invOut.clear();
       } else if (f->fusedSubScale) {
         L->kind = Launch::L_NTT_SUBSCALE; L->statKey = "NTT";
         bool anyAddend = false;
@@ -1158,12 +1210,17 @@
         L->bytes = 2 * LP * count;
       } else if (f->ops == NTT || f->ops == INTT) {
         L->kind = f->ops == NTT ? Launch::L_NTT : Launch::L_INTT; L->statKey = "NTT";
-        L->secondOnly = f->secondOnly;
+        L->secondOnly = f->secondOnly && !f->handFromTensor;
         bool anyInGalois = false;
-        for (const Part *g : group)
-          for (Instruction *i : g->ins) anyInGalois |= i->inGalois != 0;
-        for (const Part *g : group)
-          for (Instruction *i : g->ins) {
+        std::vector<Instruction *> recs;
+        for (int pass = 0; pass < 2; ++pass)
+          for (const Part *g : group)
+            for (Instruction *i : g->ins)
+              if (i->handFromTensor == (pass == 0)) recs.push_back(i);
+        for (Instruction *i : recs) anyInGalois |= i->inGalois != 0;
+        L->nSecond = (uint32_t)std::count_if(recs.begin(), recs.end(), [](Instruction *i) { return i->handFromTensor; });
+        if (L->nSecond == recs.size()) { L->secondOnly = L->nSecond != 0; L->nSecond = 0; }
+        for (Instruction *i : recs) {
             if (anyInGalois) L->inGalois.push_back(i->inGalois);
             L->a.push_back(limbOf(i->operandList[0])); L->out.push_back(limbOf(i->OutputOperand)); L->mods.push_back(i->mod_id);
             L->k.push_back(i->hasConstant ? i->constant : 1);
@@ -1355,7 +1412,7 @@
           for (size_t i = 0; i < n0; ++i) l->outPacked.push_back(l->outPacked[i]);
       }
       rep(l->a, true); rep(l->b, true); rep(l->c, true); rep(l->d, true);
-      rep(l->out, true); rep(l->out1, true); rep(l->out2, true); rep(l->mods, false);
+      rep(l->out, true); rep(l->out1, true); rep(l->out2, true); rep(l->mods, false); rep(l->invOut, true);
       rep(l->inGalois, false); rep(l->addGalois, false);
       for (std::vector<uint64_t> *kv : {&l->k, &l->mixK, &l->addK}) {
         const size_t k0 = kv->size();
@@ -1372,6 +1429,21 @@
           for (uint32_t &x : q.epB) x += c * per;
           l->probs.push_back(q);
         }
+    }
+    if (l->nSecond && batch_ > 1) {
+      const size_t n0 = l->out.size() / batch_, s0 = l->nSecond;
+      std::vector<size_t> order;
+      for (int pass = 0; pass < 2; ++pass)
+        for (uint32_t c = 0; c < batch_; ++c)
+          for (size_t i = pass ? s0 : 0; i < (pass ? n0 : s0); ++i) order.push_back(c * n0 + i);
+      auto perm = [&](auto &v) {
+        if (v.empty()) return;
+        auto o = v;
+        for (size_t j = 0; j < order.size(); ++j) o[j] = v[order[j]];
+        v.swap(o);
+      };
+      perm(l->a); perm(l->out); perm(l->mods); perm(l->k); perm(l->outPacked); perm(l->inGalois);
+      l->nSecond = (uint32_t)(s0 * batch_);
     }
     l->refInstructions *= batch_;
     l->bytes *= batch_;
@@ -1475,6 +1547,8 @@
     if (po) out += " packed_out=" + std::to_string(po);
     if (pi) out += " packed_in=" + std::to_string(pi) + "/" + std::to_string(l->probs.size());
     if (l->secondOnly) out += " second_pass_only";
+    if (l->nSecond) out += " second_pass_only=" + std::to_string(l->nSecond);
+    if (!l->invOut.empty()) out += " inverse_out=" + std::to_string(std::count_if(l->invOut.begin(), l->invOut.end(), [](uint32_t x) { return x != HM_NO_LIMB; }));
     for (const auto *gv : {&l->inGalois, &l->addGalois}) {
       uint32_t cnt = 0, g = 0;
       for (uint32_t x : *gv) if (x > 1) { ++cnt; g = x; }
@@ -1508,6 +1582,15 @@
     break;
   case Launch::L_INTT: {
     const bool anyPacked = std::find(l.outPacked.begin(), l.outPacked.end(), 1) != l.outPacked.end();
+    if (l.nSecond) {
+      const uint32_t s = l.nSecond;
+      hm_ntt_desc d2 = {pool, l.a.data(), pool, l.out.data(), l.mods.data(), s, 1, l.hasK ? l.k.data() : nullptr, 1, anyPacked ? l.outPacked.data() : nullptr, nullptr};
+      if ((st = hm_ntt_ex(ctx, &d2)) != HM_OK) break;
+      hm_ntt_desc d = {pool, l.a.data() + s, pool, l.out.data() + s, l.mods.data() + s, cnt - s, 1, l.hasK ? l.k.data() + s : nullptr, 0,
+                       anyPacked ? l.outPacked.data() + s : nullptr, l.inGalois.empty() ? nullptr : l.inGalois.data() + s};
+      st = hm_ntt_ex(ctx, &d);
+      break;
+    }
     hm_ntt_desc d = {pool, l.a.data(), pool, l.out.data(), l.mods.data(), cnt, 1, l.hasK ? l.k.data() : nullptr, l.secondOnly ? 1 : 0,
                      anyPacked ? l.outPacked.data() : nullptr, l.inGalois.empty() ? nullptr : l.inGalois.data()};
     st = hm_ntt_ex(ctx, &d);
@@ -1551,6 +1634,11 @@
     break;
   }
   case Launch::L_TENSOR:
+    if (!l.invOut.empty()) {
+      const hm_tensor_desc d = {pool, l.a.data(), pool, l.b.data(), pool, l.c.data(), pool, l.d.data(), pool, l.out.data(), pool, l.out1.data(), pool,
+                                l.out2.data(), l.mods.data(), cnt, pool, l.invOut.data()};
+      st = hm_tensor_ex(ctx, &d);
+    } else
     st = hm_tensor(ctx, pool, l.a.data(), pool, l.b.data(), pool, l.c.data(), pool, l.d.data(), pool, l.out.data(), pool, l.out1.data(), pool,
                    l.out2.data(), l.mods.data(), cnt);
     break;
diff --git a/include/homulator_hip.h b/include/homulator_hip.h
--- a/include/homulator_hip.h
+++ b/include/homulator_hip.h
@@ -82,6 +82,18 @@
                     const uint64_t *c, const uint32_t *c_limbs, const uint64_t *d, const uint32_t *d_limbs,
                     uint64_t *o0, const uint32_t *o0_limbs, uint64_t *o1, const uint32_t *o1_limbs, uint64_t *o2,
                     const uint32_t *o2_limbs, const uint32_t *mod_ids, uint32_t n);
+typedef struct hm_tensor_desc {
+  const uint64_t *a;  const uint32_t *a_limbs;
+  const uint64_t *b;  const uint32_t *b_limbs;
+  const uint64_t *c;  const uint32_t *c_limbs;
+  const uint64_t *d;  const uint32_t *d_limbs;
+  uint64_t *o0;       const uint32_t *o0_limbs;
+  uint64_t *o1;       const uint32_t *o1_limbs;
+  uint64_t *o2;       const uint32_t *o2_limbs;
+  const uint32_t *mod_ids; uint32_t n;
+  uint64_t *inv_out;  const uint32_t *inv_out_limbs;
+} hm_tensor_desc;
+hm_status hm_tensor_ex(hm_ctx *ctx, const hm_tensor_desc *desc);
 
 hm_status hm_inner_product(hm_ctx *ctx, const uint64_t *x, const uint32_t *x_limbs, const uint64_t *y,
                            const uint32_t *y_limbs, uint64_t *out, const uint32_t *out_limbs,
```
